# muelea/tuch

Measured on AMD Instinct MI355X. Metric: SMPLify-DC fit iters/sec at batch 64, higher is better.
Workload: dtype f32; 1 GPU; configs[1] extended to the full stage-2 step: batch=64/GPU SMPL forward + contact_fitting_loss (L_P/L_C push/pull, winding inside test, segment filter, r2r) + backward + Adam, V=6890 F=13776, float32; bodies_per_gpu=64, global_batch=64, launch=hipGraph replay of the whole step

## Files before the change

include/tuch_amd.h:

```cpp
#ifndef TUCH_AMD_H
#define TUCH_AMD_H

#include <stddef.h>
#include <stdint.h>

#ifdef __cplusplus
extern "C" {
#endif

const char* tuch_last_error(void);
int tuch_abi_version(void);


int tuch_batch_pairwise_dist(const float* x, const float* y, int B, int Nx, int Ny, int squared,
                             float* P, void* stream);

int tuch_batch_pairwise_dist_bwd(const float* x, const float* y, const float* grad_P, int B, int Nx, int Ny,
                                 int squared, float* grad_x, float* grad_y, void* stream);

int tuch_solid_angles_bwd(const float* points, const float* triangles, const float* grad_out, const float* grad_w,
                          int B, int Q, int F, float* grad_points, float* grad_triangles, void* stream);

int tuch_solid_angles(const float* points, const float* triangles, int B, int Q, int F, float* out,
                      void* stream);
// ... 70 lines not shown
int tuch_smplify_tail_bwd(const float* grad_out, const uint8_t* valid, const float* gj, const float* gc, const float* gp,
                          int B, int NJ, int P, float contact_scale, float r2r_scale, float* grad_contact, float* grad_r2r,
                          float* gj_out, float* gc_out, float* gp_out, void* stream);

size_t tuch_smplify_stage2_fused_scratch_floats(int B);
int tuch_smplify_stage2_fused(const float* points, const int32_t* partner, const uint8_t* exterior,
                              const uint8_t* body_valid, int B, int N, int mode, float euclthres,
                              const float* small_terms, const float* r2r, const int32_t* ij, int P, float contact_scale,
                              float r2r_scale, float* share, int* ticket, float* terms, float* out, float* grad_points,
                              const tuch_contact_model* model, const void* pair_keys, void* grad_fixed_zeroed, void* stream);
int tuch_fixed_to_float(const void* fixed, size_t n, float* out, void* stream);
void tuch_set_deterministic(int on);
int tuch_get_deterministic(void);

int tuch_region_pair_keys(const tuch_contact_model* model, const float* verts, int B, const uint8_t* select,
                          int use_geomask, void* keys_zeroed, void* stream);
int tuch_smplify_stage2_finish(const float* points, const int32_t* partner, const uint8_t* exterior,
                               const uint8_t* body_valid, int B, int N, int mode, float euclthres,
                               const float* small_terms, const float* r2r, int P, float contact_scale, float r2r_scale,
                               float* share, int* ticket, float* terms, float* out, void* stream);
int tuch_smplify_stage2_bwd(const float* grad_out, const uint8_t* body_valid, const float* points, const int32_t* partner,
                            const uint8_t* exterior, int B, int N, int mode, float euclthres, float contact_scale,
                            const int32_t* ij, int P, float r2r_scale, const float* gj, const float* gc, const float* gp,
                            int NJ, float* grad_points, float* gj_out, float* gc_out, float* gp_out, void* stream);

typedef struct tuch_contact_model tuch_contact_model;

int tuch_contact_model_create(tuch_contact_model** out, int V, int F, const int32_t* faces ,
                              const uint8_t* geomask ,
                              int num_segments, const int32_t* seg_q_off, const int32_t* seg_q_vidx,
                              const int32_t* seg_f_off, const int32_t* seg_faces,
                              int num_caps, const int32_t* cap_off, const int32_t* cap_vidx,
                              int num_regions, const int32_t* region_off, const int32_t* region_vidx,
                              int num_pairs, const int32_t* pairs);
void tuch_contact_model_destroy(tuch_contact_model* model);
int tuch_contact_model_set_option(tuch_contact_model* model, const char* name, int value);
int tuch_contact_model_get_option(const tuch_contact_model* model, const char* name, int* value);
int tuch_contact_model_canary_hits(const tuch_contact_model* model, int* hits_host, int reset);
int tuch_contact_model_canary_selftest(const tuch_contact_model* model, void* workspace, size_t workspace_bytes, void* stream);
const uint64_t* tuch_contact_model_mask_bits(const tuch_contact_model* model);
const int32_t* tuch_contact_model_faces(const tuch_contact_model* model);
int32_t* tuch_contact_model_tickets(const tuch_contact_model* model);
const uint64_t* tuch_contact_model_tree_mask_bits(const tuch_contact_model* model);
int tuch_contact_model_info(const tuch_contact_model* model, int* V, int* F, int* num_segments,
                            int* seg_q_total, int* num_pairs);
int tuch_contact_model_strips(const tuch_contact_model* model, int* stream_len, int* num_strips,
                              int32_t* vidx_host, float* sign_host);

int tuch_winding_tree_work(const tuch_contact_model* model, const float* verts, int B, void* workspace,
                           size_t workspace_bytes, unsigned long long* out_host, void* stream);

int tuch_ray_work(const tuch_contact_model* model, const float* verts, int B, void* workspace,
                  size_t workspace_bytes, unsigned long long* out_host, void* stream);
int tuch_contact_model_tree_order(const tuch_contact_model* model, int32_t* qperm_host, int32_t* face_leaf_host);

size_t tuch_v2v_model_workspace_bytes(const tuch_contact_model* model, int B);
size_t tuch_v2v_hint_bytes(const tuch_contact_model* model, int B);
int tuch_v2v_min_model(const tuch_contact_model* model, const float* verts, int B, float* min_d2,
                       int32_t* argmin, void* hint_inout, void* workspace, size_t workspace_bytes, void* stream);
int tuch_v2v_min_model_shared(const tuch_contact_model* model, const float* verts, int B, float* min_d2,
                              int32_t* argmin, void* hint_inout, void* workspace, size_t workspace_bytes, int leave_room,
                              void* stream);
int tuch_v2v_min_model_shared_zero(const tuch_contact_model* model, const float* verts, int B, float* min_d2, int32_t* argmin,
                                   void* hint_inout, void* workspace, size_t workspace_bytes, int leave_room, void* zero,
                                   size_t zero_bytes, void* stream);

int tuch_v2v_min_model_can_cap(const tuch_contact_model* model);
int tuch_v2v_min_model_capped(const tuch_contact_model* model, const float* verts, int B, float* min_d2, int32_t* argmin,
                              void* hint_inout, void* workspace, size_t workspace_bytes, int leave_room, void* zero,
                              size_t zero_bytes, const uint8_t* prev_exterior, float cap, void* stream);
int tuch_v2v_min_model_fix(const tuch_contact_model* model, int B, const uint8_t* exterior, uint8_t* prev_exterior, float cap,
                           float* min_d2, int32_t* argmin, void* hint_inout, void* workspace, size_t workspace_bytes,
                           void* stream);

typedef struct tuch_cluster_tree tuch_cluster_tree;
int tuch_cluster_tree_build(int V, int F, const int32_t* faces, int leaf_faces, tuch_cluster_tree** out);
void tuch_cluster_tree_free(tuch_cluster_tree* tree);
int tuch_cluster_tree_info(const tuch_cluster_tree* tree, int* num_nodes, int* exact_len, int* stream_len,
                           int* num_qblocks, int* num_frontiers, int* frontier_total);
int tuch_cluster_tree_export(const tuch_cluster_tree* tree, int32_t* nodes, int32_t* vidx, float* sign,
                             int32_t* qperm, int32_t* frontier_off, int32_t* frontier_nodes,
                             int32_t* launch_order, int32_t* rows, int32_t* face_leaf);

size_t tuch_exterior_workspace_bytes(const tuch_contact_model* model, int B);
int tuch_exterior_flags(const tuch_contact_model* model, const float* verts, int B, int apply_segments,
                        float thresh, float* w, uint8_t* exterior, float* seg_w, uint8_t* seg_exterior,
                        void* workspace, size_t workspace_bytes, void* stream);

size_t tuch_winding_points_workspace_bytes(const tuch_contact_model* model, int B, int Q);
int tuch_winding_points(const tuch_contact_model* model, const float* verts, const float* points,
                        const int32_t* counts, int B, int Q, float thresh, float* w, uint8_t* exterior,
                        void* workspace, size_t workspace_bytes, void* stream);

int tuch_region_pair_min(const tuch_contact_model* model, const float* verts, int B, const uint8_t* select,
                         int use_geomask, float* out_min, int32_t* out_ij, void* stream);
int tuch_region_pair_min_bwd(const tuch_contact_model* model, const float* verts, int B, const int32_t* ij,
                             const float* grad_out, float* grad_verts, void* stream);

int tuch_self_contact(const float* verts , const uint64_t* geomask_bits, int B, int V, float euclthres,
                      const int32_t* vreg_off , const int32_t* vreg , int R,
                      uint8_t* in_contact , int32_t* partner , float* min_d2 ,
                      float* sig_d2 , float* cnc_d2 , void* stream);

typedef struct tuch_smpl_model tuch_smpl_model;

int tuch_smpl_model_create(tuch_smpl_model** out, int V, const float* v_template, const float* shapedirs,
// ... 76 lines not shown
```

tuch_amd/_C.py:

```python
from __future__ import annotations

import ctypes
import os
from ctypes import POINTER, c_char_p, c_float, c_int, c_size_t, c_void_p

import torch

_HERE = os.path.dirname(os.path.abspath(__file__))
LIB_PATH = os.environ.get('TUCH_AMD_LIB') or os.path.join(_HERE, 'libtuch_amd.so')
_lib = None

_SIGNATURES = {
    'tuch_last_error': (c_char_p, []),
    'tuch_abi_version': (c_int, []),
    'tuch_batch_pairwise_dist': (c_int, [c_void_p, c_void_p, c_int, c_int, c_int, c_int, c_void_p, c_void_p]),
    'tuch_batch_pairwise_dist_bwd': (c_int, [c_void_p, c_void_p, c_void_p, c_int, c_int, c_int, c_int, c_void_p, c_void_p,
                                             c_void_p]),
    'tuch_solid_angles_bwd': (c_int, [c_void_p, c_void_p, c_void_p, c_void_p, c_int, c_int, c_int, c_void_p, c_void_p, c_void_p]),
    'tuch_solid_angles': (c_int, [c_void_p, c_void_p, c_int, c_int, c_int, c_void_p, c_void_p]),
    'tuch_gather_triangles': (c_int, [c_void_p, c_void_p, c_int, c_int, c_int, c_void_p, c_void_p]),
    'tuch_winding_workspace_bytes': (c_size_t, [c_int, c_int, c_int]),
    'tuch_winding_numbers': (c_int, [c_void_p, c_void_p, c_int, c_int, c_int, c_void_p, c_void_p, c_float,
                                     c_void_p, c_size_t, c_void_p]),
    'tuch_geomask_words': (c_int, [c_int]),
# ... 15 lines not shown
    'tuch_valid_mean_fwd': (c_int, [c_void_p, c_void_p, c_int, c_int, c_void_p, c_void_p]),
    'tuch_valid_mean_bwd': (c_int, [c_void_p, c_void_p, c_void_p, c_int, c_int, c_void_p, c_void_p]),
    'tuch_smpl_backward_split_adam': (c_int, [c_void_p, c_void_p, c_int, c_void_p, c_int, c_int, c_void_p, c_void_p, c_void_p,
                                              c_void_p, c_void_p, c_int, c_void_p, c_int, c_void_p, c_int,
                                              c_void_p, c_int, c_void_p, c_int, c_void_p, c_void_p, c_void_p, c_void_p, c_void_p,
                                              c_void_p, c_float, c_float, c_float, c_float, c_void_p, c_size_t, c_void_p, c_void_p]),
    'tuch_contact_terms_bwd_fixed': (c_int, [c_void_p, c_void_p, c_void_p, c_void_p, c_int, c_int, c_int, c_float,
                                             c_void_p, c_void_p, c_void_p]),
    'tuch_smplify_small_terms': (c_int, [c_void_p] * 9 + [c_int, c_int, c_int, c_float, c_float, c_float] + [c_void_p] * 5),
    'tuch_smplify_stage1_terms': (c_int, [c_void_p] * 7 + [c_int, c_int, c_int, c_float, c_float, c_float, c_float] + [c_void_p] * 7),
    'tuch_adam_step': (c_int, [c_int, c_void_p, c_void_p, c_void_p, c_void_p, c_void_p, c_void_p, c_void_p, c_float, c_float,
                                c_void_p]),
    'tuch_smplify_objective': (c_int, [c_void_p, c_void_p, c_void_p, c_int, c_int, c_float, c_float, c_void_p, c_void_p]),
    'tuch_smplify_objective_bwd': (c_int, [c_void_p, c_int, c_int, c_float, c_float, c_void_p, c_void_p, c_void_p,
                                           c_void_p]),
    'tuch_smplify_tail_bwd': (c_int, [c_void_p] * 5 + [c_int, c_int, c_int, c_float, c_float] + [c_void_p] * 6),
    'tuch_contact_model_create': (c_int, [POINTER(c_void_p), c_int, c_int, c_void_p, c_void_p,
                                          c_int, c_void_p, c_void_p, c_void_p, c_void_p,
                                          c_int, c_void_p, c_void_p,
                                          c_int, c_void_p, c_void_p, c_int, c_void_p]),
    'tuch_contact_model_destroy': (None, [c_void_p]),
    'tuch_contact_model_set_option': (c_int, [c_void_p, c_char_p, c_int]),
    'tuch_contact_model_get_option': (c_int, [c_void_p, c_char_p, POINTER(c_int)]),
    'tuch_contact_model_canary_hits': (c_int, [c_void_p, POINTER(c_int), c_int]),
    'tuch_contact_model_canary_selftest': (c_int, [c_void_p, c_void_p, c_size_t, c_void_p]),
    'tuch_contact_model_mask_bits': (c_void_p, [c_void_p]),
    'tuch_contact_model_faces': (c_void_p, [c_void_p]),
    'tuch_contact_model_tickets': (c_void_p, [c_void_p]),
    'tuch_contact_model_tree_mask_bits': (c_void_p, [c_void_p]),
    'tuch_contact_model_info': (c_int, [c_void_p, POINTER(c_int), POINTER(c_int), POINTER(c_int),
                                        POINTER(c_int), POINTER(c_int)]),
    'tuch_contact_model_strips': (c_int, [c_void_p, POINTER(c_int), POINTER(c_int), c_void_p, c_void_p]),
    'tuch_cluster_tree_build': (c_int, [c_int, c_int, c_void_p, c_int, POINTER(c_void_p)]),
    'tuch_cluster_tree_free': (None, [c_void_p]),
    'tuch_cluster_tree_info': (c_int, [c_void_p] + [POINTER(c_int)] * 6),
    'tuch_cluster_tree_export': (c_int, [c_void_p] * 10),
    'tuch_hd_points_fwd': (c_int, [c_void_p] * 5 + [c_int, c_int, c_void_p, c_void_p]),
    'tuch_hd_points_bwd': (c_int, [c_void_p] * 5 + [c_int, c_int, c_void_p, c_void_p]),
    'tuch_estimate_translation': (c_int, [c_void_p, c_void_p, c_void_p, c_int, c_int, c_float, c_float, c_void_p, c_void_p]),
    'tuch_rotmat_to_angle_axis': (c_int, [c_void_p, c_int, c_int, c_void_p, c_void_p]),
    'tuch_winding_tree_work': (c_int, [c_void_p, c_void_p, c_int, c_void_p, c_size_t, c_void_p, c_void_p]),
    'tuch_hd_model_create': (c_int, [POINTER(c_void_p), c_void_p, c_int, c_void_p, c_void_p, c_void_p]),
    'tuch_hd_model_create_k': (c_int, [POINTER(c_void_p), c_void_p, c_int, c_int, c_void_p, c_void_p, c_void_p]),
    'tuch_hd_model_destroy': (None, [c_void_p]),
    'tuch_hd_model_info': (c_int, [c_void_p, POINTER(c_int), c_void_p]),
    'tuch_hd_contact_saved_bytes': (c_size_t, [c_void_p, c_int]),
    'tuch_hd_contact_workspace_bytes': (c_size_t, [c_void_p, c_int]),
    'tuch_hd_contact_fwd': (c_int, [c_void_p] * 6 + [c_int, c_float, c_float, c_void_p, c_void_p, c_size_t, c_void_p, c_size_t,
                                    c_void_p]),
    'tuch_hd_contact_bwd': (c_int, [c_void_p, c_void_p, c_void_p, c_int, c_void_p, c_void_p, c_size_t, c_void_p]),
    'tuch_hd_contact_selection': (c_int, [c_void_p, c_void_p, c_int, c_void_p, c_void_p]),
    'tuch_hd_contact_details': (c_int, [c_void_p, c_void_p, c_int, c_void_p, c_void_p]),
    'tuch_ray_work': (c_int, [c_void_p, c_void_p, c_int, c_void_p, c_size_t, c_void_p, c_void_p]),
    'tuch_contact_model_tree_order': (c_int, [c_void_p, c_void_p, c_void_p]),
    'tuch_v2v_model_workspace_bytes': (c_size_t, [c_void_p, c_int]),
    'tuch_v2v_hint_bytes': (c_size_t, [c_void_p, c_int]),
    'tuch_v2v_min_model': (c_int, [c_void_p, c_void_p, c_int, c_void_p, c_void_p, c_void_p, c_void_p, c_size_t, c_void_p]),
    'tuch_v2v_min_model_shared': (c_int, [c_void_p, c_void_p, c_int, c_void_p, c_void_p, c_void_p, c_void_p, c_size_t, c_int,
                                          c_void_p]),
    'tuch_v2v_min_model_shared_zero': (c_int, [c_void_p, c_void_p, c_int, c_void_p, c_void_p, c_void_p, c_void_p, c_size_t, c_int,
                                               c_void_p, c_size_t, c_void_p]),
    'tuch_exterior_workspace_bytes': (c_size_t, [c_void_p, c_int]),
    'tuch_v2v_min_model_can_cap': (c_int, [c_void_p]),
    'tuch_v2v_min_model_capped': (c_int, [c_void_p, c_void_p, c_int, c_void_p, c_void_p, c_void_p, c_void_p, c_size_t, c_int,
                                          c_void_p, c_size_t, c_void_p, c_float, c_void_p]),
    'tuch_v2v_min_model_fix': (c_int, [c_void_p, c_int, c_void_p, c_void_p, c_float, c_void_p, c_void_p, c_void_p, c_void_p,
                                       c_size_t, c_void_p]),
    'tuch_exterior_flags': (c_int, [c_void_p, c_void_p, c_int, c_int, c_float, c_void_p, c_void_p, c_void_p,
                                    c_void_p, c_void_p, c_size_t, c_void_p]),
    'tuch_winding_points_workspace_bytes': (c_size_t, [c_void_p, c_int, c_int]),
    'tuch_winding_points': (c_int, [c_void_p, c_void_p, c_void_p, c_void_p, c_int, c_int, c_float, c_void_p, c_void_p,
                                    c_void_p, c_size_t, c_void_p]),
    'tuch_contact_terms_ragged_fwd': (c_int, [c_void_p, c_void_p, c_void_p, c_void_p, c_int, c_int, c_float, c_void_p,
                                              c_void_p]),
    'tuch_contact_terms_ragged_bwd': (c_int, [c_void_p, c_void_p, c_void_p, c_void_p, c_void_p, c_int, c_int, c_float,
                                              c_void_p, c_void_p]),
    'tuch_region_pair_min': (c_int, [c_void_p, c_void_p, c_int, c_void_p, c_int, c_void_p, c_void_p, c_void_p]),
    'tuch_smpl_model_create': (c_int, [POINTER(c_void_p), c_int] + [c_void_p] * 9),
    'tuch_smpl_model_destroy': (None, [c_void_p]),
    'tuch_smpl_model_info': (c_int, [c_void_p, POINTER(c_int)]),
    'tuch_smpl_forward_workspace_bytes': (c_size_t, [c_void_p, c_int]),
    'tuch_smpl_backward_workspace_bytes': (c_size_t, [c_void_p, c_int]),
    'tuch_smpl_forward': (c_int, [c_void_p, c_void_p, c_void_p, c_int, c_int, c_void_p, c_void_p, c_void_p,
                                  c_size_t, c_void_p]),
    'tuch_smpl_backward': (c_int, [c_void_p, c_void_p, c_int, c_int, c_void_p, c_void_p, c_void_p, c_void_p,
                                   c_void_p, c_void_p, c_size_t, c_void_p]),
    'tuch_smplify_stage2_fused_scratch_floats': (c_size_t, [c_int]),
    'tuch_smplify_stage2_fused': (c_int, [c_void_p, c_void_p, c_void_p, c_void_p, c_int, c_int, c_int, c_float, c_void_p, c_void_p,
                                           c_void_p, c_int, c_float, c_float, c_void_p, c_void_p, c_void_p, c_void_p, c_void_p,
                                           c_void_p, c_void_p, c_void_p, c_void_p]),
    'tuch_set_deterministic': (None, [c_int]),
    'tuch_get_deterministic': (c_int, []),
    'tuch_region_pair_keys': (c_int, [c_void_p, c_void_p, c_int, c_void_p, c_int, c_void_p, c_void_p]),
    'tuch_smplify_stage2_finish': (c_int, [c_void_p, c_void_p, c_void_p, c_void_p, c_int, c_int, c_int, c_float, c_void_p,
                                           c_void_p, c_int, c_float, c_float, c_void_p, c_void_p, c_void_p, c_void_p,
                                           c_void_p]),
    'tuch_smplify_stage2_bwd': (c_int, [c_void_p, c_void_p, c_void_p, c_void_p, c_void_p, c_int, c_int, c_int, c_float,
                                        c_float, c_void_p, c_int, c_float, c_void_p, c_void_p, c_void_p, c_int, c_void_p,
                                        c_void_p, c_void_p, c_void_p, c_void_p]),
    'tuch_smpl_forward_split': (c_int, [c_void_p, c_void_p, c_void_p, c_int, c_void_p, c_int, c_int, c_int, c_void_p,
                                        c_void_p, c_void_p, c_size_t, c_void_p]),
    'tuch_smpl_backward_split': (c_int, [c_void_p, c_void_p, c_int, c_void_p, c_int, c_int, c_int, c_void_p, c_void_p,
                                         c_void_p, c_void_p, c_void_p, c_int, c_void_p, c_int, c_void_p, c_size_t,
                                         c_void_p]),
    'tuch_smpl_backward_split_add': (c_int, [c_void_p, c_void_p, c_int, c_void_p, c_int, c_int, c_int, c_void_p, c_void_p,
                                             c_void_p, c_void_p, c_void_p, c_int, c_void_p, c_int, c_void_p, c_int, c_void_p,
# ... 65 lines not shown
```

tuch_amd/csrc/api.hip:

```cpp
#include "common.h"
#include <stdarg.h>
#include <stdio.h>

static thread_local char g_error[512] = "";

void tuch_set_error(const char* fmt, ...)
{
    va_list ap;
    va_start(ap, fmt);
    vsnprintf(g_error, sizeof(g_error), fmt, ap);
    va_end(ap);
}

int tuch_check_launch(const char* what)
{
    const hipError_t e = hipGetLastError();
    if (e != hipSuccess) {
        tuch_set_error("%s: %s", what, hipGetErrorString(e));
        return TUCH_ERR_HIP;
    }
    return TUCH_OK;
}

extern "C" const char* tuch_last_error(void) { return g_error; }
extern "C" int tuch_abi_version(void) { return 1; }

#include <stdlib.h>
static int g_deterministic = [] { const char* e = getenv("TUCH_DETERMINISTIC"); return e && atoi(e) == 0 ? 0 : 1; }();
int tuch_deterministic() { return g_deterministic; }
extern "C" void tuch_set_deterministic(int on) { g_deterministic = on ? 1 : 0; }
extern "C" int tuch_get_deterministic(void) { return g_deterministic; }

static int g_host_tables = [] { const char* e = getenv("TUCH_HOST_TABLES"); return e && atoi(e) != 0 ? 1 : 0; }();
int tuch_host_tables() { return g_host_tables; }
#include <string.h>
int tuch_table_upload(void** dst, const void* src, size_t bytes)
{
    *dst = nullptr;
    if (bytes == 0) return TUCH_OK;
    if (g_host_tables) {
        *dst = malloc(bytes);
        if (!*dst) { tuch_set_error("model table: malloc(%zu) failed", bytes); return TUCH_ERR_HIP; }
        memcpy(*dst, src, bytes);
        return TUCH_OK;
    }
    if (hipMalloc(dst, bytes) != hipSuccess) {
        *dst = nullptr;
        tuch_set_error("model table: hipMalloc(%zu) failed", bytes);
        return TUCH_ERR_HIP;
    }
    if (hipMemcpy(*dst, src, bytes, hipMemcpyHostToDevice) != hipSuccess) {
        tuch_set_error("model table: hipMemcpy of %zu bytes failed", bytes);
        return TUCH_ERR_HIP;
    }
    return TUCH_OK;
}
int tuch_table_download(void* dst_host, const void* src, size_t bytes)
{
    if (g_host_tables) { memcpy(dst_host, src, bytes); return TUCH_OK; }
    return hipMemcpy(dst_host, src, bytes, hipMemcpyDeviceToHost) == hipSuccess ? TUCH_OK : TUCH_ERR_HIP;
}
void tuch_table_free(void* p)
{
    if (!p) return;
    if (g_host_tables) free(p); else (void)hipFree(p);
}
```

tuch_amd/csrc/model.h:

```cpp
#pragma once
#include "common.h"
#include <vector>

struct tuch_cluster_tree {
    int V = 0, F = 0, num_nodes = 0, exact_len = 0, stream_len = 0, num_qblocks = 0, num_heights = 0;
    std::vector<int32_t> nodes;
    std::vector<int32_t> vidx;
    std::vector<float> sign;
    std::vector<int32_t> qperm;
    std::vector<int32_t> height_off, height_nodes;
    std::vector<int32_t> frontier_off, frontier_nodes;
    std::vector<int32_t> launch_order;
    std::vector<int32_t> ancestors;
    std::vector<int32_t> rows;
    std::vector<int32_t> face_leaf;
};

bool tuch_cluster_tree_build_impl(int V, int F, const int32_t* faces, int leaf_faces, tuch_cluster_tree& t);
void tuch_build_strips(const int32_t* faces, int F, std::vector<int32_t>& vidx, std::vector<float>& sign,
                       int* num_strips);

struct tuch_contact_model;

struct tuch_options {
    int winding_ray = 1;
    int winding_tree = 1;
    int winding_strips = 1;
    int tree_waves = 32768;
    int ray_pair_cap = 16;
    int ray_waves = 32768;
    int ray_fans = 0;
    int ray_cross = 0;
    int ray_cross_split = 0;
    int v2v_tree = 1;
    int v2v_waves = 0;
    int v2v_cap = 0;
    int v2v_flat = 2;
    int v2v_pairs = 24;
    int v2v_lds = -1;
    int seg_splits = 16;
    int seg_assist = 1;
    int seg_fused = 1;
    int canary = 0;
    int hd_search = 1;
    int hd_search_waves = 4;
    int hd_overlap = 1;
};
void tuch_options_from_env(tuch_options* o);

bool tuch_ray_available(const tuch_contact_model* m);
struct RayEntry { int32_t leaf, node; uint32_t mask_lo, mask_hi; };
struct RayTile { int32_t ex_off, ex_len, first, n; };
struct RayBody { int32_t tiles, overflow; };
struct TreeNode;
void tuch_ray_layout_touch(const tuch_contact_model* m, int B, int Q);
size_t tuch_ray_workspace_bytes(const tuch_contact_model* m, int B, int Q);
int tuch_ray_exterior_verts(const tuch_contact_model* m, const float* verts, int B, float thresh, uint8_t* exterior,
                            float* w, void* workspace, hipStream_t s, unsigned long long* stats_host,
                            uint8_t* exterior_copy = nullptr);
const int32_t* tuch_ray_segment_counts(const tuch_contact_model* m, int B, const void* workspace);
void tuch_ray_segment_prepare(const tuch_contact_model* m, const float* verts, const float* caps, int assisted, int B,
                              float* seg_entries, hipStream_t s);
bool tuch_ray_segment_fused_available(const tuch_contact_model* m);
int tuch_ray_segment_flags_one(const tuch_contact_model* m, const float* verts, const uint8_t* body_flags,
                               const int32_t* leaf_counts, int B, float thresh, uint8_t* exterior, hipStream_t s);
int tuch_ray_segment_flags(const tuch_contact_model* m, const float* verts, const float* caps, const int32_t* seg_count,
                           const int32_t* seg_list, const int32_t* leaf_counts, int B, int nsplit, float thresh, float* seg_tris,
                           int32_t* seg_partial, float* seg_w, uint8_t* seg_ext, uint8_t* exterior, hipStream_t s);
int tuch_ray_exterior_points(const tuch_contact_model* m, const float* verts, const float* points, const int32_t* counts,
                             int B, int Q, float thresh, uint8_t* exterior, float* w, void* workspace, hipStream_t s);

int tuch_v2v_min_indexed_seeded(const float* points, const int32_t* vertex_ids, const int32_t* offsets,
                                const int32_t* counts, const float* seed_best, const int32_t* seed_arg,
                                const int32_t* all_masked_arg, const uint64_t* geomask_bits, int B, int V,
                                int max_points_per_body, float* min_d2, int32_t* argmin, void* workspace, hipStream_t s);
extern "C" size_t tuch_v2v_min_indexed_workspace_bytes(int B, int max_points_per_body);
size_t tuch_hd_search_workspace_bytes(int B, int max_points_per_body);
int tuch_hd_search(const float* points, const int32_t* vertex_ids, const int32_t* offsets, const int32_t* counts,
                   const int32_t* all_masked_arg, const uint64_t* geomask_bits, int B, int V, int max_points_per_body,
                   float* min_d2, int32_t* argmin, void* workspace, hipStream_t s, int waves);
extern "C" size_t tuch_winding_points_workspace_bytes(const tuch_contact_model* m, int B, int Q);
extern "C" int tuch_winding_points(const tuch_contact_model* m, const float* verts, const float* points,
                                   const int32_t* counts, int B, int Q, float thresh, float* w,
                                   uint8_t* exterior, void* workspace, size_t workspace_bytes, void* stream);

struct tuch_contact_model {
    int device;
    tuch_options opt;
    int V, F;
    int32_t* faces;
    int32_t* tickets;
    int32_t* canary_hits;
    uint64_t* mask_bits;
    int strip_len, num_strips;
    int32_t* strip_vidx;
    float* strip_sign;
    int tree_nodes, tree_stream_len, tree_exact_len, tree_qblocks, tree_heights, tree_leaves;
    int32_t* tree_node;
    int32_t* tree_vidx;
    float* tree_sign;
    int32_t* tree_sign_word;
    int32_t* tree_qperm;
    int32_t* tree_height_off;
    int32_t* tree_height_nodes;
    int32_t* tree_frontier_nodes;
    int32_t* tree_launch_order;
    int32_t* tree_ancestors;
    int32_t* tree_rows;
    int32_t* tree_v2v_info;
    uint64_t* tree_mask_bits;
    uint64_t* tree_masked;
    int32_t* tree_sub_leaf;
// ... 49 lines not shown
```

tuch_amd/csrc/model.hip:

```cpp
#include "model.h"
#include <stdio.h>
#include <stdlib.h>
#include <string.h>
#include <algorithm>
#include <vector>
#include <unordered_map>

extern "C" int tuch_geomask_words(int V);

namespace {

template <typename T>
int upload(T** dst, const T* src, size_t count)
{
    return tuch_table_upload((void**)dst, src, count * sizeof(T));
}

int* host_copy(const int32_t* src, size_t n)
{
    int* p = (int*)malloc(sizeof(int) * (n ? n : 1));
    if (n) memcpy(p, src, sizeof(int) * n);
    return p;
}

// ... 375 lines not shown
        for (int r = 0; r < num_regions; ++r) {
            const int n = region_off[r + 1] - region_off[r];
            if (n > m->region_max) m->region_max = n;
        }
        rc = upload(&m->region_off, region_off, (size_t)num_regions + 1);
        if (rc == TUCH_OK) rc = upload(&m->region_vidx, region_vidx, (size_t)region_off[num_regions]);
        if (rc == TUCH_OK && num_pairs > 0) rc = upload(&m->pairs, pairs, (size_t)num_pairs * 2);
        if (rc == TUCH_OK && num_pairs > 0 && geomask) {
            std::vector<int64_t> off(num_pairs + 1, 0);
            for (int p = 0; p < num_pairs; ++p) {
                const int n1 = region_off[pairs[2 * p] + 1] - region_off[pairs[2 * p]];
                const int n2 = region_off[pairs[2 * p + 1] + 1] - region_off[pairs[2 * p + 1]];
                off[p + 1] = off[p] + (int64_t)n1 * ((n2 + 31) / 32);
            }
            std::vector<uint32_t> words((size_t)off[num_pairs], 0u);
            for (int p = 0; p < num_pairs; ++p) {
                const int32_t* r1 = region_vidx + region_off[pairs[2 * p]];
                const int32_t* r2 = region_vidx + region_off[pairs[2 * p + 1]];
                const int n1 = region_off[pairs[2 * p] + 1] - region_off[pairs[2 * p]];
                const int n2 = region_off[pairs[2 * p + 1] + 1] - region_off[pairs[2 * p + 1]];
                const int wpr = (n2 + 31) / 32;
                for (int a = 0; a < n1; ++a)
                    for (int k = 0; k < n2; ++k)
                        if (geomask[(size_t)r1[a] * V + r2[k]])
                            words[(size_t)off[p] + (size_t)a * wpr + (k >> 5)] |= 1u << (k & 31);
            }
            rc = upload(&m->pair_mask, words.data(), words.size());
            if (rc == TUCH_OK) rc = upload(&m->pair_mask_off, off.data(), off.size());
        }
    }
    if (rc == TUCH_OK && !tree_sign_host.empty()) {
        std::vector<int32_t> word(tree_sign_host.size(), 0);
        for (size_t p = 0; p < word.size(); ++p) {
            const int32_t sg = tree_sign_host[p] > 0.0f ? 1 : tree_sign_host[p] < 0.0f ? -1 : 0;
            const int32_t em = p < elem_mask_host.size() ? elem_mask_host[p] : 0;
            word[p] = (int32_t)(((uint32_t)em << 24) | ((uint32_t)sg & 0xffffffu));
        }
        rc = upload(&m->tree_sign_word, word.data(), word.size());
    }
    if (rc != TUCH_OK) {
        tuch_contact_model_destroy(m);
        *out = nullptr;
        return rc;
    }
    *out = m;
    return TUCH_OK;
}

namespace {
struct OptionName { const char* name; int tuch_options::*field; };
const OptionName kOptions[] = {
    {"winding_ray", &tuch_options::winding_ray}, {"winding_tree", &tuch_options::winding_tree},
    {"winding_strips", &tuch_options::winding_strips}, {"tree_waves", &tuch_options::tree_waves},
    {"ray_pair_cap", &tuch_options::ray_pair_cap}, {"ray_waves", &tuch_options::ray_waves}, {"ray_fans", &tuch_options::ray_fans}, {"ray_cross", &tuch_options::ray_cross}, {"v2v_cap", &tuch_options::v2v_cap}, {"ray_cross_split", &tuch_options::ray_cross_split},
    {"v2v_tree", &tuch_options::v2v_tree}, {"v2v_flat", &tuch_options::v2v_flat}, {"v2v_pairs", &tuch_options::v2v_pairs}, {"v2v_waves", &tuch_options::v2v_waves}, {"v2v_lds", &tuch_options::v2v_lds},
    {"seg_splits", &tuch_options::seg_splits}, {"seg_assist", &tuch_options::seg_assist}, {"seg_fused", &tuch_options::seg_fused},
    {"canary", &tuch_options::canary}, {"hd_search", &tuch_options::hd_search}, {"hd_search_waves", &tuch_options::hd_search_waves}, {"hd_overlap", &tuch_options::hd_overlap},
};
}

void tuch_options_from_env(tuch_options* o)
{
    for (const OptionName& k : kOptions) {
        char env[64] = "TUCH_";
        size_t n = strlen(env);
        for (const char* c = k.name; *c && n + 1 < sizeof(env); ++c) env[n++] = (char)toupper((unsigned char)*c);
        env[n] = 0;
        const char* e = getenv(env);
        if (e && *e) o->*(k.field) = atoi(e);
    }
}

extern "C" int tuch_contact_model_set_option(tuch_contact_model* m, const char* name, int value)
{
    TUCH_REQUIRE(m && name, "tuch_contact_model_set_option: null argument");
    for (const OptionName& k : kOptions)
        if (!strcmp(k.name, name)) {
            TUCH_REQUIRE(strcmp(name, "seg_assist") != 0, "tuch_contact_model_set_option: seg_assist is fixed when the model "
                         "is created (TUCH_SEG_ASSIST)");
            m->opt.*(k.field) = value;
            return TUCH_OK;
        }
    tuch_set_error("tuch_contact_model_set_option: unknown option '%s'", name);
    return TUCH_ERR_ARG;
}

extern "C" int tuch_contact_model_canary_hits(const tuch_contact_model* m, int* hits_host, int reset)
{
    TUCH_REQUIRE(m && hits_host, "tuch_contact_model_canary_hits: null argument");
    if (hipDeviceSynchronize() != hipSuccess ||
        hipMemcpy(hits_host, m->canary_hits, sizeof(int32_t), hipMemcpyDeviceToHost) != hipSuccess ||
        (reset && hipMemset(m->canary_hits, 0, sizeof(int32_t)) != hipSuccess)) {
        tuch_set_error("tuch_contact_model_canary_hits: %s", hipGetErrorString(hipGetLastError()));
        return TUCH_ERR_HIP;
    }
    return TUCH_OK;
}

extern "C" int tuch_contact_model_get_option(const tuch_contact_model* m, const char* name, int* value)
{
    TUCH_REQUIRE(m && name && value, "tuch_contact_model_get_option: null argument");
    if (!strcmp(name, "seg_fused_active")) {
        *value = tuch_ray_segment_fused_available(m) ? 1 : 0;
        return TUCH_OK;
    }
    for (const OptionName& k : kOptions)
        if (!strcmp(k.name, name)) {
            *value = m->opt.*(k.field);
            return TUCH_OK;
        }
    tuch_set_error("tuch_contact_model_get_option: unknown option '%s'", name);
    return TUCH_ERR_ARG;
}

extern "C" const uint64_t* tuch_contact_model_mask_bits(const tuch_contact_model* m)
{
    return m ? m->mask_bits : nullptr;
}

extern "C" const uint64_t* tuch_contact_model_tree_mask_bits(const tuch_contact_model* m)
{
    return m ? m->tree_mask_bits : nullptr;
}

extern "C" int32_t* tuch_contact_model_tickets(const tuch_contact_model* m)
{
    return m ? m->tickets : nullptr;
}

extern "C" const int32_t* tuch_contact_model_faces(const tuch_contact_model* m)
{
    return m ? m->faces : nullptr;
}

extern "C" int tuch_contact_model_tree_order(const tuch_contact_model* m, int32_t* qperm_host, int32_t* face_leaf_host)
{
    TUCH_REQUIRE(m, "tuch_contact_model_tree_order: null model");
    TUCH_REQUIRE(m->tree_nodes > 0 && m->tree_qperm_host && m->tree_face_leaf_host,
                 "tuch_contact_model_tree_order: the model has no cluster tree");
    if (qperm_host) memcpy(qperm_host, m->tree_qperm_host, sizeof(int32_t) * m->V);
    if (face_leaf_host) memcpy(face_leaf_host, m->tree_face_leaf_host, sizeof(int32_t) * m->F);
    return TUCH_OK;
}

extern "C" int tuch_contact_model_strips(const tuch_contact_model* m, int* stream_len, int* num_strips,
                                         int32_t* vidx_host, float* sign_host)
{
    TUCH_REQUIRE(m, "tuch_contact_model_strips: null model");
    if (stream_len) *stream_len = m->strip_len;
    if (num_strips) *num_strips = m->num_strips;
    if (vidx_host && tuch_table_download(vidx_host, m->strip_vidx, sizeof(int32_t) * m->strip_len) != TUCH_OK)
        return TUCH_ERR_HIP;
    if (sign_host && tuch_table_download(sign_host, m->strip_sign, sizeof(float) * m->strip_len) != TUCH_OK)
        return TUCH_ERR_HIP;
    return TUCH_OK;
}
// ... 13 lines not shown
```

tuch_amd/csrc/ray_winding.hip:

```cpp
#include "common.h"
#include "model.h"
#include "workspace.h"
#include "tree_device.h"
#include <stdlib.h>

#pragma clang fp contract(off)

namespace {

constexpr float kPi = 3.14159265358979323846f;
constexpr int kBlock = 256;
constexpr int kRayQueries = 64;
constexpr float kShearX = 0.3217f, kShearY = 0.4331f;
constexpr float kFanX = 0.8191f, kFanY = 0.3467f, kFanZ = 0.4571f;
constexpr int kSlabs = 9;
constexpr int kSlabStride = 10;
constexpr int kNearSlabs = 13;

struct RayElem { float x, y, z, sign; };

__device__ __forceinline__ float shear_x(float x, float z) { return __builtin_fmaf(-kShearX, z, x); }
__device__ __forceinline__ float shear_y(float y, float z) { return __builtin_fmaf(-kShearY, z, y); }

__global__ __launch_bounds__(kBlock) void ray_stream_kernel(
// ... 32 lines not shown
    v = fminf(v, dpp_move<0x141>(v));
    v = fminf(v, dpp_move<0x140>(v));
    return v;
}

__device__ __forceinline__ uint32_t half_below(float x)
{
    const _Float16 h = (_Float16)x;
    uint32_t u = __builtin_bit_cast(uint16_t, h);
    if ((float)h > x) u = (u & 0x8000u) ? u + 1 : (u == 0 ? 0x8001u : u - 1);
    return u;
}
__device__ __forceinline__ uint32_t half_above(float x)
{
    const _Float16 h = (_Float16)x;
    uint32_t u = __builtin_bit_cast(uint16_t, h);
    if ((float)h < x) u = (u & 0x8000u) ? (u == 0x8000u ? 0x0001u : u - 1) : u + 1;
    return u;
}
__device__ __host__ __forceinline__ size_t near_records_at(int B, int L) { return (size_t)B * kNearSlabs * L; }
__device__ __host__ __forceinline__ size_t near_centres_at(int B, int L) { return near_records_at(B, L) + (size_t)B * L * 8; }

struct QRec { float x, y, z; int32_t tag; };
constexpr int kNoSlot = 0xffffff;
struct RayPre { int blocks, qblocks; QRec* qrec; float4* ranges; const int32_t* vmask; };

__device__ __forceinline__ void ray_block_prepass(const float* __restrict__ vb, int first_vertex,
                                                  const int32_t* __restrict__ qperm, const int32_t* __restrict__ vmask,
                                                  int Q, int qb, int lane, QRec* __restrict__ qrec, float4* __restrict__ ranges)
{
    const int slot = qb * kRayQueries + lane;
    const float* q3 = vb + 3 * (size_t)qperm[slot];
    const float* c0 = vb + 3 * (size_t)first_vertex;
    const float qz = q3[2], qx = shear_x(q3[0], qz), qy = shear_y(q3[1], qz);
    const float cz = c0[2], cx = shear_x(c0[0], cz), cy = shear_y(c0[1], cz);
    QRec r;
    r.x = qx; r.y = qy; r.z = qz;
    r.tag = slot < Q ? (slot | (vmask ? vmask[slot] << 24 : 0)) : kNoSlot;
    qrec[slot] = r;
    const float rx = qx - cx, ry = qy - cy, rz = qz - cz;
    const float r4 = rx + ry, r5 = rx - ry, r6 = rx + rz, r7 = rx - rz, r8 = ry + rz, r9 = ry - rz;
    const float bx0 = wave_min_uniform(rx), bx1 = wave_max_uniform(rx), by0 = wave_min_uniform(ry), by1 = wave_max_uniform(ry);
    const float b40 = wave_min_uniform(r4), b41 = wave_max_uniform(r4), b50 = wave_min_uniform(r5), b51 = wave_max_uniform(r5);
    const float bz0 = wave_min_uniform(rz), b60 = wave_min_uniform(r6), b71 = wave_max_uniform(r7);
    const float b80 = wave_min_uniform(r8), b91 = wave_max_uniform(r9);
    if (lane == 0) {
        ranges[0] = make_float4(bx0, bx1, by0, by1);
        ranges[1] = make_float4(b40, b41, b50, b51);
        ranges[2] = make_float4(bz0, b60, b71, b80);
        ranges[3] = make_float4(b91, 0.f, 0.f, 0.f);
    }
}

__device__ __forceinline__ float fan_terms(const float* __restrict__ vb, int v, bool real, int& n,
                                           const int32_t* __restrict__ ring_off, const int32_t* __restrict__ ring_vidx);
template <bool kPose>
__global__ __launch_bounds__(kBoundsBlock) void ray_leaf_bounds_kernel(
    const RayElem* __restrict__ stream, int T, const TreeNode* __restrict__ nodes, int N,
    const int32_t* __restrict__ height_off, const int32_t* __restrict__ height_nodes, float* __restrict__ bounds,
    const float* __restrict__ verts, const int32_t* __restrict__ vidx, const float* __restrict__ sign, int V, int Lexact,
    RayElem* __restrict__ stream_out, uint4* __restrict__ zeroed, size_t zeroed_n,
    int leaf_blocks = 0, const int32_t* __restrict__ qperm = nullptr, const int32_t* __restrict__ ring_off = nullptr,
    const int32_t* __restrict__ ring_vidx = nullptr, float2* __restrict__ fans = nullptr, int fan_stride = 0,
    RayPre pre = RayPre{0, 0, nullptr, nullptr, nullptr})
{
    if (kPose && pre.blocks > 0 && (int)blockIdx.x >= (int)gridDim.x - pre.blocks) {
        for (size_t g = ((size_t)blockIdx.y * gridDim.x + blockIdx.x) * kBoundsBlock + threadIdx.x; g < zeroed_n;
             g += (size_t)gridDim.x * gridDim.y * kBoundsBlock)
            zeroed[g] = make_uint4(0u, 0u, 0u, 0u);
        const int qb = ((int)blockIdx.x - ((int)gridDim.x - pre.blocks)) * (kBoundsBlock / 64) + (int)(threadIdx.x >> 6);
        if (qb < pre.qblocks)
            ray_block_prepass(verts + (size_t)blockIdx.y * V * 3, vidx[0], qperm, pre.vmask, V, qb, threadIdx.x & 63,
                              pre.qrec + (size_t)blockIdx.y * pre.qblocks * kRayQueries,
                              pre.ranges + ((size_t)blockIdx.y * pre.qblocks + qb) * 4);
        return;
    }
    if (kPose && leaf_blocks > 0 && (int)blockIdx.x >= leaf_blocks) {
        for (size_t g = ((size_t)blockIdx.y * gridDim.x + blockIdx.x) * kBoundsBlock + threadIdx.x; g < zeroed_n;
             g += (size_t)gridDim.x * gridDim.y * kBoundsBlock)
            zeroed[g] = make_uint4(0u, 0u, 0u, 0u);
        const int i = ((int)blockIdx.x - leaf_blocks) * kBoundsBlock + (int)threadIdx.x;
        const bool real = i < V;
        const int v = qperm[real ? i : V - 1];
        int cr = 0;
        const float half = fan_terms(verts + (size_t)blockIdx.y * V * 3, v, real, cr, ring_off, ring_vidx);
        if (i < fan_stride) fans[(size_t)blockIdx.y * fan_stride + i] = make_float2(__int_as_float(cr), half);
        return;
    }
    const int b = blockIdx.y;
    const RayElem* st = stream + (size_t)b * T;
    const int group = threadIdx.x >> 4, sub = threadIdx.x & 15;
    const int i = height_off[0] + blockIdx.x * (kBoundsBlock / 16) + group;
    const bool real = i < height_off[1];
    const int node = height_nodes[real ? i : height_off[0]];
    const int off = nodes[node].ex_off, len = real ? nodes[node].ex_len : 0;
    if (kPose) {
        for (size_t g = ((size_t)b * gridDim.x + blockIdx.x) * kBoundsBlock + threadIdx.x; g < zeroed_n;
             g += (size_t)gridDim.x * gridDim.y * kBoundsBlock)
            zeroed[g] = make_uint4(0u, 0u, 0u, 0u);
        if (blockIdx.x == 0)
            for (int p = Lexact + (int)threadIdx.x; p < T; p += kBoundsBlock) stream_out[(size_t)b * T + p] = RayElem{0.f, 0.f, 0.f, 0.f};
    }
    float lo[kSlabs], nhi[kSlabs];
#pragma unroll
    for (int k = 0; k < kSlabs; ++k) { lo[k] = 3.0e38f; nhi[k] = 3.0e38f; }
    for (int p = sub; p < len; p += 16) {
        RayElem e;
        if (kPose) {
            const float* c = verts + ((size_t)b * V + vidx[off + p]) * 3;
            e.x = shear_x(c[0], c[2]); e.y = shear_y(c[1], c[2]); e.z = c[2]; e.sign = sign[off + p];
            stream_out[(size_t)b * T + off + p] = e;
        } else {
            e = st[off + p];
        }
        float pr[kSlabs];
        slab_project(e.x, e.y, e.z, pr);
#pragma unroll
        for (int k = 0; k < kSlabs; ++k) { lo[k] = fminf(lo[k], pr[k]); nhi[k] = fminf(nhi[k], -pr[k]); }
    }
#pragma unroll
    for (int k = 0; k < kSlabs; ++k) { lo[k] = row_min(lo[k]); nhi[k] = row_min(nhi[k]); }
    if (real && sub == 0) {
        const int L = height_off[1] - height_off[0], leaf = i - height_off[0];
        float lo_p[kSlabs], hi_p[kSlabs];
#pragma unroll
        for (int k = 0; k < kSlabs; ++k) {
            const float hi = -nhi[k];
            const float pad = 4e-7f * fmaxf(fabsf(lo[k]), fabsf(hi)) + 1e-9f;
            lo_p[k] = lo[k] - pad;
            hi_p[k] = hi + pad;
        }
        float c[3];
        if (kPose) {
            const float* c0 = verts + ((size_t)b * V + vidx[0]) * 3;
            c[0] = shear_x(c0[0], c0[2]); c[1] = shear_y(c0[1], c0[2]); c[2] = c0[2];
        } else {
            const RayElem e0 = st[0];
            c[0] = e0.x; c[1] = e0.y; c[2] = e0.z;
        }
        float pc[kSlabs];
        slab_project(c[0], c[1], c[2], pc);
        uint32_t lo_h[kSlabs], hi_h[kSlabs];
#pragma unroll
        for (int k = 0; k < kSlabs; ++k) {
            const float pad = 4e-6f * (fabsf(lo_p[k]) + fabsf(hi_p[k]) + fabsf(pc[k])) + 1e-7f;
            lo_h[k] = half_below(lo_p[k] - pc[k] - pad);
            hi_h[k] = half_above(hi_p[k] - pc[k] + pad);
        }
        uint4* r = reinterpret_cast<uint4*>(bounds + near_records_at(gridDim.y, L)) + ((size_t)b * L + leaf) * 2;
        r[0] = make_uint4(lo_h[0] | lo_h[1] << 16, lo_h[3] | lo_h[4] << 16, lo_h[6] | lo_h[8] << 16, hi_h[0] | hi_h[1] << 16);
        r[1] = make_uint4(hi_h[2] | hi_h[3] << 16, hi_h[4] | hi_h[5] << 16, hi_h[7] | (uint32_t)leaf << 16, (uint32_t)node);
        if (leaf == 0) *reinterpret_cast<float4*>(bounds + near_centres_at(gridDim.y, L) + (size_t)b * 4) = make_float4(c[0], c[1], c[2], 0.f);
    }
}

__global__ __launch_bounds__(kBoundsBlock) void ray_prepass_kernel(
    const float* __restrict__ verts, const int32_t* __restrict__ vidx, const int32_t* __restrict__ qperm, int V, RayPre pre)
{
    const int qb = (int)blockIdx.x * (kBoundsBlock / 64) + (int)(threadIdx.x >> 6);
    if (qb < pre.qblocks)
        ray_block_prepass(verts + (size_t)blockIdx.y * V * 3, vidx[0], qperm, pre.vmask, V, qb, threadIdx.x & 63,
                          pre.qrec + (size_t)blockIdx.y * pre.qblocks * kRayQueries,
                          pre.ranges + ((size_t)blockIdx.y * pre.qblocks + qb) * 4);
}

struct P3 { float x, y, z; };

__device__ __forceinline__ float edge_fn(const P3& p, const P3& q) { return p.x * q.y - p.y * q.x; }

__device__ __forceinline__ bool left_of(float e, const P3& p, const P3& q)
{
    return e > 0.0f || (e == 0.0f && (p.x < q.x || (p.x == q.x && p.y < q.y)));
}

__device__ __forceinline__ int crossing(const P3& a, const P3& b, const P3& c, float ea, float eb, float ec)
{
    const bool la = left_of(ea, b, c), lb = left_of(eb, c, a), lc = left_of(ec, a, b);
    const bool pos = la && lb && lc, neg = !la && !lb && !lc;
    if (!(pos || neg)) return 0;
    const float numz = ea * a.z + eb * b.z + ec * c.z;
    if (pos) return numz > 0.0f ? 1 : 0;
    return numz < 0.0f ? -1 : 0;
}

__device__ __forceinline__ int crossing_mostly_generic(const P3& a, const P3& b, const P3& c, float ea, float eb, float ec)
{
    const float numz = ea * a.z + eb * b.z + ec * c.z;
    const float mn = __builtin_fminf(__builtin_fminf(ea, eb), ec), mx = __builtin_fmaxf(__builtin_fmaxf(ea, eb), ec);
    int n = (int)(__builtin_fminf(mn, numz) > 0.0f) - (int)(__builtin_fmaxf(mx, numz) < 0.0f);
    const bool tie = (mn * mx == 0.0f) & (numz != 0.0f);
    if (__builtin_amdgcn_ballot_w64(tie)) {
        if (tie) n = crossing(a, b, c, ea, eb, ec);
    }
    return n;
}

template <bool kSkipIncident>
__device__ __forceinline__ int crossing_with_ties(const P3 a, const P3 b, const P3 c, float ea, float eb, float ec)
{
    if (kSkipIncident) {
        const bool za = (a.x == 0.0f) & (a.y == 0.0f) & (a.z == 0.0f);
        const bool zb = (b.x == 0.0f) & (b.y == 0.0f) & (b.z == 0.0f);
        const bool zc = (c.x == 0.0f) & (c.y == 0.0f) & (c.z == 0.0f);
        if (za | zb | zc) return 0;
    }
    return crossing(a, b, c, ea, eb, ec);
}

constexpr uint32_t kSegBias = 0x80808080u;
struct S3 { v2f xy; float z; };
__device__ __forceinline__ float edge_fn(const S3& p, const S3& q)
{
    v2f r;
    asm("v_pk_mul_f32 %0, %1, %2 op_sel:[0,1] op_sel_hi:[1,0]" : "=v"(r) : "v"(p.xy), "v"(q.xy));
    float d;
    asm("v_sub_f32 %0, %1, %2" : "=v"(d) : "v"(r.x), "v"(r.y));
    return d;
}
__device__ __forceinline__ P3 p3(const S3& a) { return P3{a.xy.x, a.xy.y, a.z}; }

template <int A, bool kSkipIncident, bool kSeg>
__device__ __forceinline__ void ray_step(const RayElem el, S3 (&s)[3], float (&e)[3], v2f qxy, float qz, int& count,
                                         int qmask, uint32_t& pa, uint32_t& pb)
{
    constexpr int Bq = (A + 1) % 3, Cq = (A + 2) % 3;
    s[A].xy = (v2f){el.x, el.y} - qxy;
    s[A].z = el.z - qz;
    e[Bq] = edge_fn(s[Cq], s[A]);
    e[Cq] = edge_fn(s[A], s[Bq]);
    const int word = __float_as_int(el.sign);
    if ((word & 0xffffff) != 0) {
        const float numz = __builtin_fmaf(e[A], s[A].z, __builtin_fmaf(e[Cq], s[Cq].z, e[Bq] * s[Bq].z));
        const float mn = __builtin_fminf(__builtin_fminf(e[0], e[1]), e[2]);
        const float mx = __builtin_fmaxf(__builtin_fmaxf(e[0], e[1]), e[2]);
        int c = (int)(__builtin_fminf(mn, numz) > 0.0f) - (int)(__builtin_fmaxf(mx, numz) < 0.0f);
        const bool edge_zero = mn * mx == 0.0f;
        if (__builtin_amdgcn_ballot_w64(edge_zero)) {
            const bool tie = edge_zero & (numz != 0.0f);
            if (__builtin_amdgcn_ballot_w64(tie)) {
                if (tie) c = crossing_with_ties<kSkipIncident>(p3(s[Bq]), p3(s[Cq]), p3(s[A]), e[Bq], e[Cq], e[A]);
            }
        }
        asm("v_mad_i32_i24 %0, %1, %2, %0" : "+v"(count) : "v"(c), "s"(word));
        if (kSeg && ((uint32_t)word >> 24) != 0) {
            const uint32_t t = ((uint32_t)word >> 24) & (uint32_t)qmask;
            if (__builtin_amdgcn_ballot_w64((t != 0) & (c != 0))) {
                uint32_t cs;
                asm("v_mul_i32_i24 %0, %1, %2" : "=v"(cs) : "v"(c), "s"(word));
                pa += cs * (((t & 15u) * 0x00204081u) & 0x01010101u);
                pb += cs * ((((t >> 4) & 15u) * 0x00204081u) & 0x01010101u);
            }
        }
    }
}

template <bool kSkipIncident, bool kSeg>
__device__ __forceinline__ void ray_run(const RayElem* __restrict__ st, int off, int len,
                                        S3 (&s)[3], float (&e)[3], v2f qxy, float qz, int& count,
                                        int qmask, uint32_t& pa, uint32_t& pb)
{
    const RayElem* p = st + off;
    RayElem n0 = p[0], n1 = p[1], n2 = p[2];
    for (int left = len; left > 0; left -= 3, p += 3) {
        asm("" : "+s"(left));
        const RayElem e0 = n0, e1 = n1, e2 = n2;
        n0 = p[3]; n1 = p[4]; n2 = p[5];
        ray_step<0, kSkipIncident, kSeg>(e0, s, e, qxy, qz, count, qmask, pa, pb);
        ray_step<1, kSkipIncident, kSeg>(e1, s, e, qxy, qz, count, qmask, pa, pb);
        ray_step<2, kSkipIncident, kSeg>(e2, s, e, qxy, qz, count, qmask, pa, pb);
    }
}

constexpr int kFallbackChunks = 8;

__device__ __forceinline__ float wave_min(float v) { return wave_min_uniform(v); }
__device__ __forceinline__ float wave_max(float v) { return wave_max_uniform(v); }


__device__ __forceinline__ float lo_minus(uint32_t s, float q)
{
    float d;
    asm("v_fma_mix_f32 %0, %1, 1.0, -%2 op_sel_hi:[1,0,0]" : "=v"(d) : "v"(s), "v"(q));
    return d;
}
__device__ __forceinline__ float hi_minus(uint32_t s, float q)
{
    float d;
    asm("v_fma_mix_f32 %0, %1, 1.0, -%2 op_sel:[1,0,0] op_sel_hi:[1,0,0]" : "=v"(d) : "v"(s), "v"(q));
    return d;
}
__device__ __forceinline__ float minus_lo(float q, uint32_t s)
{
    float d;
    asm("v_fma_mix_f32 %0, -%1, 1.0, %2 op_sel_hi:[1,0,0]" : "=v"(d) : "v"(s), "v"(q));
    return d;
}
__device__ __forceinline__ float minus_hi(float q, uint32_t s)
{
    float d;
    asm("v_fma_mix_f32 %0, -%1, 1.0, %2 op_sel:[1,0,0] op_sel_hi:[1,0,0]" : "=v"(d) : "v"(s), "v"(q));
    return d;
}
__device__ __forceinline__ float max3(float a, float b, float c)
{
    float d;
    asm("v_max3_f32 %0, %1, %2, %3" : "=v"(d) : "v"(a), "v"(b), "v"(c));
    return d;
}

template <bool kVerts, int kWaves>
__global__ __launch_bounds__(64 * kWaves) void ray_near_kernel(
    const float* __restrict__ pts, const TreeNode* __restrict__ nodes, const float* __restrict__ bounds, int N,
    int num_leaves, const int32_t* __restrict__ qperm,
    const int32_t* __restrict__ counts, int Q, int qblocks, RayEntry* __restrict__ lists, int32_t* __restrict__ list_len,
    int32_t* __restrict__ leaf_cnt,
    unsigned long long* __restrict__ stats,
    const int32_t* __restrict__ ring_off = nullptr, const int32_t* __restrict__ ring_vidx = nullptr,
    float2* __restrict__ fans = nullptr)
{
    if (kVerts && (int)blockIdx.x >= qblocks) {
        const int i = ((int)blockIdx.x - qblocks) * (64 * kWaves) + (int)threadIdx.x;
        const bool real = i < Q;
        const int v = qperm[real ? i : Q - 1];
        int cr = 0;
        const float half = fan_terms(pts + (size_t)blockIdx.y * Q * 3, v, real, cr, ring_off, ring_vidx);
        if (i < qblocks * kRayQueries) fans[(size_t)blockIdx.y * qblocks * kRayQueries + i] = make_float2(__int_as_float(cr), half);
        return;
    }
    __builtin_amdgcn_s_setprio(3);
    const int qb = blockIdx.x, b = blockIdx.y, lane = threadIdx.x & 63;
    const int wave = kWaves > 1 ? __builtin_amdgcn_readfirstlane(threadIdx.x >> 6) : 0;
    __shared__ uint4 queue[64 * kWaves][2];
    __shared__ float range[16];
    __shared__ int queued[2], slots;
    int i0;
    bool real;
    if (kVerts) {
        i0 = qperm[qb * kRayQueries + lane];
        real = qb * kRayQueries + lane < Q;
    } else {
        const int n = counts ? counts[b] : Q;
        if (qb * kRayQueries >= n) {
            if (threadIdx.x == 0) list_len[(size_t)b * qblocks + qb] = 0;
            return;
        }
        i0 = min(qb * kRayQueries + lane, n - 1);
        real = qb * kRayQueries + lane < n;
    }
    if (threadIdx.x == 0) { queued[0] = 0; queued[1] = 0; slots = 0; }
    const float4 ctr = *reinterpret_cast<const float4*>(bounds + near_centres_at(gridDim.y, num_leaves) + (size_t)b * 4);
    const uint4* recs = reinterpret_cast<const uint4*>(bounds + near_records_at(gridDim.y, num_leaves)) + (size_t)b * num_leaves * 2;
    struct Chunk { uint4 r0, r1; };
    auto load_chunk = [&](int base) {
        Chunk c;
        const int lc = min(base + lane, num_leaves - 1);
        c.r0 = recs[lc * 2];
        c.r1 = recs[lc * 2 + 1];
        return c;
    };
    Chunk nxt = load_chunk(wave * 64);
    const float* q3 = pts + ((size_t)b * Q + i0) * 3;
    const float qz = q3[2];
    const float qx = shear_x(q3[0], qz), qy = shear_y(q3[1], qz);
    const float rx = qx - ctr.x, ry = qy - ctr.y, rz = qz - ctr.z;
    const float r4 = rx + ry, r5 = rx - ry, r6 = rx + rz, r7 = rx - rz, r8 = ry + rz, r9 = ry - rz;
    float bx0, bx1, by0, by1, b40, b41, b50, b51, bz0, b60, b71, b80, b91;
    if (kWaves == 4) {
        if (wave == 0) {
            const float a = wave_min(rx), c = wave_max(rx), d = wave_min(ry), e = wave_max(ry);
            if (lane == 0) { range[0] = a; range[1] = c; range[2] = d; range[3] = e; }
        } else if (wave == 1) {
            const float a = wave_min(r4), c = wave_max(r4), d = wave_min(r5), e = wave_max(r5);
            if (lane == 0) { range[4] = a; range[5] = c; range[6] = d; range[7] = e; }
        } else if (wave == 2) {
            const float a = wave_min(rz), c = wave_min(r6), d = wave_max(r7);
            if (lane == 0) { range[8] = a; range[9] = c; range[10] = d; }
        } else {
            const float a = wave_min(r8), c = wave_max(r9);
            if (lane == 0) { range[11] = a; range[12] = c; }
        }
        __syncthreads();
        bx0 = range[0]; bx1 = range[1]; by0 = range[2]; by1 = range[3]; b40 = range[4]; b41 = range[5]; b50 = range[6];
        b51 = range[7]; bz0 = range[8]; b60 = range[9]; b71 = range[10]; b80 = range[11]; b91 = range[12];
    } else {
        bx0 = wave_min(rx); bx1 = wave_max(rx); by0 = wave_min(ry); by1 = wave_max(ry);
        b40 = wave_min(r4); b41 = wave_max(r4); b50 = wave_min(r5); b51 = wave_max(r5);
        bz0 = wave_min(rz); b60 = wave_min(r6); b71 = wave_max(r7); b80 = wave_min(r8); b91 = wave_max(r9);
    }
    RayEntry* list = lists + ((size_t)b * qblocks + qb) * num_leaves;
    unsigned long long useful = 0, listed = 0;
    auto outside13 = [&](const uint4& s0, const uint4& s1, float x1, float x0, float y1, float y0, float p1, float p0,
                         float m1, float m0, float z0, float xz0, float xz1, float yz0, float yz1) {
        float out = max3(lo_minus(s0.x, x1), minus_lo(x0, s0.w), hi_minus(s0.x, y1));
        out = max3(out, minus_hi(y0, s0.w), lo_minus(s0.y, p1));
        out = max3(out, minus_hi(p0, s1.x), hi_minus(s0.y, m1));
        out = max3(out, minus_lo(m0, s1.y), minus_lo(z0, s1.x));
        out = max3(out, minus_hi(xz0, s1.y), lo_minus(s0.z, xz1));
        return max3(out, minus_lo(yz0, s1.z), hi_minus(s0.z, yz1));
    };
    auto outside = [&](const uint4& s0, const uint4& s1) {
        return outside13(s0, s1, rx, rx, ry, ry, r4, r4, r5, r5, rz, r6, r7, r8, r9);
    };
    int nslots = 0;
    auto emit = [&](const uint4& s1, unsigned long long hit) {
        if (!hit) return;
        const int leaf = (int)(s1.z >> 16), nd = (int)s1.w;
        if (kWaves == 1) ++nslots;
        if (lane == 0) {
            const int slot = kWaves == 1 ? nslots - 1 : atomicAdd(&slots, 1);
            list[slot] = RayEntry{leaf, nd, (uint32_t)hit, (uint32_t)(hit >> 32)};
            atomicAdd(&leaf_cnt[(size_t)b * num_leaves + leaf], __builtin_popcountll(hit));
        }
        if (stats) {
            const int len = nodes[nd].ex_len;
            useful += (unsigned long long)__builtin_popcountll(hit) * len;
            listed += 64ull * len;
        }
    };
    auto sync = [&] { if (kWaves > 1) __syncthreads(); else __builtin_amdgcn_wave_barrier(); };
    for (int round = 0; round * 64 * kWaves < num_leaves; ++round) {
        const int base = (round * kWaves + wave) * 64;
        const Chunk c = nxt;
        if (base + 64 * kWaves < num_leaves) nxt = load_chunk(base + 64 * kWaves);
        const bool pass = (base + lane < num_leaves) &
                          !(outside13(c.r0, c.r1, bx1, bx0, by1, by0, b41, b40, b51, b50, bz0, b60, b71, b80, b91) > 0.0f);
        const unsigned long long mask = __builtin_amdgcn_ballot_w64(pass);
        if (mask) {
            int at = 0;
            if (kWaves > 1) {
                if (lane == 0) at = atomicAdd(&queued[round & 1], __builtin_popcountll(mask));
                at = __builtin_amdgcn_readfirstlane(at);
            }
            at += __builtin_amdgcn_mbcnt_hi((uint32_t)(mask >> 32), __builtin_amdgcn_mbcnt_lo((uint32_t)mask, 0));
            if (pass) { queue[at][0] = c.r0; queue[at][1] = c.r1; }
        }
        sync();
        const int n = kWaves > 1 ? queued[round & 1] : __builtin_popcountll(mask);
        if (kWaves > 1 && threadIdx.x == 0) queued[(round + 1) & 1] = 0;
        if (kWaves == 1) {
            for (int i = 0; i < n; i += 4) {
                const int k1 = min(i + 1, n - 1), k2 = min(i + 2, n - 1), k3 = min(i + 3, n - 1);
                const uint4 a0 = queue[i][0], a1 = queue[i][1], c0 = queue[k1][0], c1 = queue[k1][1];
                const uint4 d0 = queue[k2][0], d1 = queue[k2][1], f0 = queue[k3][0], f1 = queue[k3][1];
                const float out_a = outside(a0, a1), out_c = outside(c0, c1), out_d = outside(d0, d1), out_f = outside(f0, f1);
                const unsigned long long hit_a = __builtin_amdgcn_ballot_w64(real && !(out_a > 0.0f));
                const unsigned long long hit_c = __builtin_amdgcn_ballot_w64(real && !(out_c > 0.0f) && i + 1 < n);
                const unsigned long long hit_d = __builtin_amdgcn_ballot_w64(real && !(out_d > 0.0f) && i + 2 < n);
                const unsigned long long hit_f = __builtin_amdgcn_ballot_w64(real && !(out_f > 0.0f) && i + 3 < n);
                emit(a1, hit_a);
                emit(c1, hit_c);
                emit(d1, hit_d);
                emit(f1, hit_f);
// ... 123 lines not shown
        for (int l = l0; l < l1; ++l) {
            const int c = cnt[l];
            off_s[l] = off;
            tile_s[l] = tile;
            off += c;
            tile += (c + 63) >> 6;
        }
        int ent = sq - nent;
        for (int q = q0; q < q1; ++q) { blk[q] = ent; ent += len[q]; }
        if (lane == 0) blk[qblocks] = total;
    }
    __syncthreads();
    for (int l = (int)blockIdx.y + (int)gridDim.y * lane; l < num_leaves; l += (int)gridDim.y * 64) {
        const TreeNode nd = nodes[leaf_nodes[l]];
        const int ex_off = nd.ex_off, ex_len = nd.ex_len;
        const int c = cnt[l], off = off_s[l];
        RayTile* out = tiles + (size_t)b * max_tiles + tile_s[l];
        for (int k = 0; k < c; k += 64) *out++ = RayTile{ex_off, ex_len, off + k, min(64, c - k)};
    }
    int32_t* fill = leaf_fill + (size_t)b * num_leaves;
    int32_t* out = pairs + (size_t)b * cap;
    for (int base = (int)blockIdx.y * 64; base < total; base += (int)gridDim.y * 64) {
        const int g = base + lane;
        RayEntry e = RayEntry{0, 0, 0u, 0u};
        int dst = 0, qb = 0;
        if (g < total) {
            int lo = 0, hi = qblocks;
            while (hi - lo > 1) {
                const int mid = (lo + hi) >> 1;
                if (blk[mid] <= g) lo = mid; else hi = mid;
            }
            qb = lo;
            e = lists[((size_t)b * qblocks + qb) * list_stride + (g - blk[qb])];
            dst = off_s[e.leaf] + atomicAdd(&fill[e.leaf], __builtin_popcount(e.mask_lo) + __builtin_popcount(e.mask_hi));
        }
        const int m = min(64, total - base);
        for (int k = 0; k < m; ++k) {
            const uint32_t lo = __builtin_amdgcn_readlane(e.mask_lo, k), hi = __builtin_amdgcn_readlane(e.mask_hi, k);
            const int d = __builtin_amdgcn_readlane(dst, k), q = __builtin_amdgcn_readlane(qb, k);
            const unsigned long long mask = ((unsigned long long)hi << 32) | lo;
            if ((mask >> lane) & 1ull)
                out[d + __builtin_popcountll(mask & ((1ull << lane) - 1ull))] = q * kRayQueries + lane;
        }
    }
}

template <bool kVerts, bool kCount, bool kSeg>
__global__ __launch_bounds__(64) void ray_leaf_kernel(
    const float* __restrict__ pts, const RayElem* __restrict__ stream, const RayTile* __restrict__ tiles,
    const RayBody* __restrict__ body, const int32_t* __restrict__ pairs, const RayEntry* __restrict__ lists,
    const int32_t* __restrict__ list_len, const TreeNode* __restrict__ nodes, int num_leaves,
    const int32_t* __restrict__ qperm, const int32_t* __restrict__ counts, int Q, int T, int qblocks, int num_bodies,
    int cap, int max_tiles, int32_t* __restrict__ count, unsigned long long* __restrict__ stats,
    const int32_t* __restrict__ vmask, int32_t* __restrict__ seg_count)
{
    const int lane = threadIdx.x;
    struct Work { int b, off, len, slot, qmask; bool active; float qx, qy, qz; };
    int b_cur = blockIdx.x, base = 0, g = blockIdx.y;
    auto fetch = [&]() {
        Work w;
        w.b = -1; w.off = w.len = w.slot = 0; w.qmask = 0; w.active = false; w.qx = w.qy = w.qz = 0.0f;
        while (b_cur < num_bodies) {
            const int b = b_cur;
            const int nt = __builtin_amdgcn_readfirstlane(body[b].tiles);
            if (g >= base + nt) { base += nt; b_cur += gridDim.x; continue; }
            const int t = g - base;
            g += gridDim.y;
            const float* pb = pts + (size_t)b * Q * 3;
            w.b = b;
            int i0;
            if (!__builtin_amdgcn_readfirstlane(body[b].overflow)) {
                const RayTile tile = tiles[(size_t)b * max_tiles + t];
                const int n = __builtin_amdgcn_readfirstlane(tile.n), first = __builtin_amdgcn_readfirstlane(tile.first);
                w.active = lane < n;
                w.slot = pairs[(size_t)b * cap + first + (w.active ? lane : 0)];
                i0 = kVerts ? qperm[w.slot] : w.slot;
                w.off = __builtin_amdgcn_readfirstlane(tile.ex_off);
                w.len = __builtin_amdgcn_readfirstlane(tile.ex_len);
            } else {
                const int nq = kVerts ? Q : (counts ? counts[b] : Q);
                w.slot = (t / kFallbackChunks) * kRayQueries + lane;
                w.active = w.slot < nq;
                i0 = kVerts ? qperm[w.slot] : min(w.slot, nq - 1);
                w.off = t;
                w.len = -1;
            }
            w.qz = pb[3 * i0 + 2];
            w.qx = shear_x(pb[3 * i0], w.qz);
            w.qy = shear_y(pb[3 * i0 + 1], w.qz);
            if (kSeg) w.qmask = vmask[w.slot];
            break;
        }
        return w;
    };
    int walked = 0;
    Work next = fetch();
    while (next.b >= 0) {
        const Work w = next;
        next = fetch();
        S3 s[3];
        float e[3];
#pragma unroll
        for (int k = 0; k < 3; ++k) { s[k].xy = (v2f){0.0f, 0.0f}; s[k].z = 0.0f; e[k] = 0.0f; }
        const v2f qxy = {w.qx, w.qy};
        int crossings = 0;
        uint32_t pa = kSegBias, pb = kSegBias;
        const RayElem* st = stream + (size_t)w.b * T;
        if (w.len >= 0) {
            ray_run<kVerts, kSeg>(st, w.off, w.len, s, e, qxy, w.qz, crossings, w.qmask, pa, pb);
            if (kCount) walked += w.len;
        } else {
            const int qb = w.off / kFallbackChunks, c = w.off % kFallbackChunks;
            const int cnt = __builtin_amdgcn_readfirstlane(list_len[(size_t)w.b * qblocks + qb]);
            const RayEntry* list = lists + ((size_t)w.b * qblocks + qb) * num_leaves;
            for (int j = c; j < cnt; j += kFallbackChunks) {
                const TreeNode nd = nodes[__builtin_amdgcn_readfirstlane(list[j].node)];
                ray_run<kVerts, kSeg>(st, nd.ex_off, nd.ex_len, s, e, qxy, w.qz, crossings, w.qmask, pa, pb);
                if (kCount) walked += nd.ex_len;
            }
        }
        if (w.active && crossings != 0) atomicAdd(&count[((size_t)w.b * qblocks) * kRayQueries + w.slot], crossings);
        if (kSeg && w.active && (pa != kSegBias || pb != kSegBias)) {
            int32_t* sc = seg_count + 2 * (((size_t)w.b * qblocks) * kRayQueries + w.slot);
            if (pa != kSegBias) atomicAdd(sc, (int32_t)(pa - kSegBias));
            if (pb != kSegBias) atomicAdd(sc + 1, (int32_t)(pb - kSegBias));
        }
    }
    if (kCount && lane == 0) atomicAdd(stats, (unsigned long long)walked);
}

constexpr int kCrossRing = 256, kCrossTrip = 3;
template <bool kSeg>
__global__ __launch_bounds__(64) void ray_cross_kernel(
    const RayElem* __restrict__ stream, const TreeNode* __restrict__ nodes, const float* __restrict__ bounds, int num_leaves,
    int nsplit,
    const QRec* __restrict__ qrec, const float4* __restrict__ ranges, int T, int qblocks, int num_bodies,
    int32_t* __restrict__ count, int32_t* __restrict__ seg_count)
{
    __shared__ QRec ring[kCrossRing];
    const int lane = threadIdx.x;
    const int unit = blockIdx.y / nsplit, z = blockIdx.y % nsplit;
    const int b = blockIdx.x + gridDim.x * (unit / num_leaves);
    if (b >= num_bodies) return;
    const int leaf = unit % num_leaves;
    const uint4* recs = reinterpret_cast<const uint4*>(bounds + near_records_at(num_bodies, num_leaves)) + ((size_t)b * num_leaves + leaf) * 2;
    const uint4 s0 = recs[0], s1 = recs[1];
    const float4 ctr = *reinterpret_cast<const float4*>(bounds + near_centres_at(num_bodies, num_leaves) + (size_t)b * 4);
    const TreeNode nd = nodes[(int)s1.w];
    const int ex_off = __builtin_amdgcn_readfirstlane(nd.ex_off), ex_len = __builtin_amdgcn_readfirstlane(nd.ex_len);
    const RayElem* st = stream + (size_t)b * T;
    const QRec* qb_base = qrec + (size_t)b * qblocks * kRayQueries;
    const float4* rg = ranges + (size_t)b * qblocks * 4;
    const int mine = qblocks > z ? (qblocks - z + nsplit - 1) / nsplit : 0;
    auto outside13 = [&](float x1, float x0, float y1, float y0, float p1, float p0, float m1, float m0, float z0, float xz0,
                         float xz1, float yz0, float yz1) {
        float out = max3(lo_minus(s0.x, x1), minus_lo(x0, s0.w), hi_minus(s0.x, y1));
        out = max3(out, minus_hi(y0, s0.w), lo_minus(s0.y, p1));
        out = max3(out, minus_hi(p0, s1.x), hi_minus(s0.y, m1));
        out = max3(out, minus_lo(m0, s1.y), minus_lo(z0, s1.x));
        out = max3(out, minus_hi(xz0, s1.y), lo_minus(s0.z, xz1));
        return max3(out, minus_lo(yz0, s1.z), hi_minus(s0.z, yz1));
    };
    auto ray_outside = [&](const QRec& q) {
        const float rx = q.x - ctr.x, ry = q.y - ctr.y, rz = q.z - ctr.z;
        return outside13(rx, rx, ry, ry, rx + ry, rx + ry, rx - ry, rx - ry, rz, rx + rz, rx - rz, ry + rz, ry - rz);
    };
    int head = 0, tail = 0;
    int base = -64;
    unsigned long long todo = 0;
    bool more = true, loaded = false;
    QRec q[kCrossTrip];
    bool have[kCrossTrip];
#pragma unroll
    for (int j = 0; j < kCrossTrip; ++j) { q[j] = QRec{0.f, 0.f, 0.f, kNoSlot}; have[j] = false; }
    auto fetch = [&]() {
        int k[kCrossTrip];
#pragma unroll
        for (int j = 0; j < kCrossTrip; ++j) {
// ... 9 lines not shown
        loaded = true;
    };
    for (;;) {
        if (tail - head < 64 && (more || loaded)) {
            if (loaded) {
                QRec qc[kCrossTrip];
                bool hc[kCrossTrip];
#pragma unroll
                for (int j = 0; j < kCrossTrip; ++j) { qc[j] = q[j]; hc[j] = have[j]; }
                loaded = false;
                if (todo) fetch();
                unsigned long long hit[kCrossTrip];
#pragma unroll
                for (int j = 0; j < kCrossTrip; ++j)
                    hit[j] = __builtin_amdgcn_ballot_w64(hc[j] && (qc[j].tag & kNoSlot) != kNoSlot && !(ray_outside(qc[j]) > 0.0f));
#pragma unroll
                for (int j = 0; j < kCrossTrip; ++j) {
                    if (hit[j]) {
                        const int pos = tail + __builtin_amdgcn_mbcnt_hi((uint32_t)(hit[j] >> 32), __builtin_amdgcn_mbcnt_lo((uint32_t)hit[j], 0));
                        if ((hit[j] >> lane) & 1ull) ring[pos & (kCrossRing - 1)] = qc[j];
                        tail += __builtin_popcountll(hit[j]);
                    }
                }
                continue;
            }
            if (!todo) {
                base += 64;
                if (base >= mine) { more = false; continue; }
                const int j = base + lane;
                const float4* g = rg + (size_t)(z + nsplit * min(j, mine - 1)) * 4;
                const float4 g0 = g[0], g1 = g[1], g2 = g[2], g3 = g[3];
                const bool pass = (j < mine) &
                                  !(outside13(g0.y, g0.x, g0.w, g0.z, g1.y, g1.x, g1.w, g1.z, g2.x, g2.y, g2.z, g2.w, g3.x) > 0.0f);
                todo = __builtin_amdgcn_ballot_w64(pass);
                continue;
            }
            fetch();
            continue;
        }
        const int n = min(64, tail - head);
        if (n <= 0) break;
        __builtin_amdgcn_wave_barrier();
        const bool active = lane < n;
        const QRec w = ring[(head + (active ? lane : 0)) & (kCrossRing - 1)];
        __builtin_amdgcn_wave_barrier();
        head += n;
        const int slot = w.tag & kNoSlot;
        S3 s[3];
        float e[3];
#pragma unroll
        for (int u = 0; u < 3; ++u) { s[u].xy = (v2f){0.0f, 0.0f}; s[u].z = 0.0f; e[u] = 0.0f; }
        int crossings = 0;
        uint32_t pa = kSegBias, pb = kSegBias;
        ray_run<true, kSeg>(st, ex_off, ex_len, s, e, (v2f){w.x, w.y}, w.z, crossings, (int)((uint32_t)w.tag >> 24), pa, pb);
        if (active && crossings != 0) atomicAdd(&count[((size_t)b * qblocks) * kRayQueries + slot], crossings);
        if (kSeg && active && (pa != kSegBias || pb != kSegBias)) {
            int32_t* sc = seg_count + 2 * (((size_t)b * qblocks) * kRayQueries + slot);
            if (pa != kSegBias) atomicAdd(sc, (int32_t)(pa - kSegBias));
            if (pb != kSegBias) atomicAdd(sc + 1, (int32_t)(pb - kSegBias));
        }
    }
}

__device__ __forceinline__ float fast_atan2(float y, float x)
{
    const float ax = __builtin_fabsf(x), ay = __builtin_fabsf(y);
    const float mx = __builtin_fmaxf(__builtin_fmaxf(ax, ay), 1e-37f);
    const float t = __builtin_fminf(ax, ay) / mx;
    const float s = t * t;
    float p = 0.0024567253421992064f;
    p = p * s + -0.014401361346244812f;
    p = p * s + 0.03978123143315315f;
    p = p * s + -0.07234857976436615f;
    p = p * s + 0.10498946160078049f;
    p = p * s + -0.14161229133605957f;
    p = p * s + 0.19985906779766083f;
    p = p * s + -0.33332598209381104f;
    p = p * s + 0.9999998807907104f;
    float v = p * t;
    v = ay > ax ? 1.57079632679489661923f - v : v;
    v = x < 0.0f ? kPi - v : v;
    return __builtin_copysignf(v, y);
}

__device__ __forceinline__ float half_solid_angle(const P3& a, const P3& b, const P3& c)
{
    const float na = __builtin_sqrtf(a.x * a.x + a.y * a.y + a.z * a.z);
    const float nb = __builtin_sqrtf(b.x * b.x + b.y * b.y + b.z * b.z);
    const float nc = __builtin_sqrtf(c.x * c.x + c.y * c.y + c.z * c.z);
    const float cx = b.y * c.z - b.z * c.y, cy = b.z * c.x - b.x * c.z, cz = b.x * c.y - b.y * c.x;
    const float num = a.x * cx + a.y * cy + a.z * cz;
    const float dab = a.x * b.x + a.y * b.y + a.z * b.z;
    const float dbc = b.x * c.x + b.y * c.y + b.z * c.z;
    const float dac = a.x * c.x + a.y * c.y + a.z * c.z;
    const float den = na * nb * nc + dab * nc + dac * nb + dbc * na;
    return fast_atan2(num, den);
}

__device__ __forceinline__ void cone_term(const P3& us, const P3& sb, const P3& sc, const P3& u, const P3& pb, const P3& pc,
                                          int& crossings, float& half)
{
    const float ea = edge_fn(sb, sc), eb = edge_fn(sc, us), ec = edge_fn(us, sb);
    const float d = ea * us.z + eb * sb.z + ec * sc.z;
    const bool la = left_of(ea, sb, sc), lb = left_of(eb, sc, us), lc = left_of(ec, us, sb);
    const bool front = d >= 0.0f;
    crossings = (la & lb & lc) ? (int)front : ((!la & !lb & !lc) ? -(int)!front : 0);
    const float nu = __builtin_sqrtf(u.x * u.x + u.y * u.y + u.z * u.z);
    const float nb = __builtin_sqrtf(pb.x * pb.x + pb.y * pb.y + pb.z * pb.z);
    const float nc = __builtin_sqrtf(pc.x * pc.x + pc.y * pc.y + pc.z * pc.z);
    const float cx = pb.y * pc.z - pb.z * pc.y, cy = pb.z * pc.x - pb.x * pc.z, cz = pb.x * pc.y - pb.y * pc.x;
    const float num = __builtin_fabsf(u.x * cx + u.y * cy + u.z * cz);
    const float dub = u.x * pb.x + u.y * pb.y + u.z * pb.z;
    const float dbc = pb.x * pc.x + pb.y * pc.y + pb.z * pc.z;
    const float duc = u.x * pc.x + u.y * pc.y + u.z * pc.z;
    const float den = nu * nb * nc + dub * nc + duc * nb + dbc * nu;
    half = fast_atan2(front ? num : -num, den);
}

__device__ __forceinline__ float fan_terms(const float* __restrict__ vb, int v, bool real, int& n,
                                           const int32_t* __restrict__ ring_off, const int32_t* __restrict__ ring_vidx)
{
    const float vx = vb[3 * v], vy = vb[3 * v + 1], vz = vb[3 * v + 2];
    const float qx = shear_x(vx, vz), qy = shear_y(vy, vz);
    const P3 u_dir = {kFanX, kFanY, kFanZ};
    const P3 us = {shear_x(kFanX, kFanZ), shear_y(kFanY, kFanZ), kFanZ};
    const int lo = ring_off[v], cnt = real ? ring_off[v + 1] - lo : 0;
    float half_sum = 0.0f;
    constexpr int kLongRing = 16;
    constexpr int kShortRing = 8;
    if (cnt > 0 && cnt <= kShortRing) {
        int rr[kShortRing];
        float cc[kShortRing][3];
#pragma unroll
        for (int u = 0; u < kShortRing; ++u) rr[u] = ring_vidx[lo + min(u, cnt - 1)];
#pragma unroll
        for (int u = 0; u < kShortRing; ++u) { cc[u][0] = vb[3 * rr[u]]; cc[u][1] = vb[3 * rr[u] + 1]; cc[u][2] = vb[3 * rr[u] + 2]; }
        P3 pb = {cc[kShortRing - 1][0] - vx, cc[kShortRing - 1][1] - vy, cc[kShortRing - 1][2] - vz};
        P3 sb = {shear_x(cc[kShortRing - 1][0], cc[kShortRing - 1][2]) - qx, shear_y(cc[kShortRing - 1][1], cc[kShortRing - 1][2]) - qy,
                 cc[kShortRing - 1][2] - vz};
#pragma unroll
        for (int u = 0; u < kShortRing; ++u) {
            if (u < cnt) {
                const P3 pc = {cc[u][0] - vx, cc[u][1] - vy, cc[u][2] - vz};
                const P3 sc = {shear_x(cc[u][0], cc[u][2]) - qx, shear_y(cc[u][1], cc[u][2]) - qy, cc[u][2] - vz};
                int cr;
                float hf;
                cone_term(us, sb, sc, u_dir, pb, pc, cr, hf);
                half_sum += hf;
                n += cr;
                pb = pc;
                sb = sc;
            }
        }
    } else if (cnt > 0 && cnt <= kLongRing) {
        int r = ring_vidx[lo + cnt - 1];
        P3 pb = {vb[3 * r] - vx, vb[3 * r + 1] - vy, vb[3 * r + 2] - vz};
        P3 sb = {shear_x(vb[3 * r], vb[3 * r + 2]) - qx, shear_y(vb[3 * r + 1], vb[3 * r + 2]) - qy, vb[3 * r + 2] - vz};
        for (int j0 = 0; j0 < cnt; j0 += 4) {
            int rr[4];
            float cc[4][3];
#pragma unroll
            for (int u = 0; u < 4; ++u) rr[u] = ring_vidx[lo + min(j0 + u, cnt - 1)];
#pragma unroll
            for (int u = 0; u < 4; ++u) { cc[u][0] = vb[3 * rr[u]]; cc[u][1] = vb[3 * rr[u] + 1]; cc[u][2] = vb[3 * rr[u] + 2]; }
#pragma unroll
            for (int u = 0; u < 4; ++u) {
                if (j0 + u < cnt) {
                    const P3 pc = {cc[u][0] - vx, cc[u][1] - vy, cc[u][2] - vz};
                    const P3 sc = {shear_x(cc[u][0], cc[u][2]) - qx, shear_y(cc[u][1], cc[u][2]) - qy, cc[u][2] - vz};
                    int cr;
                    float hf;
                    cone_term(us, sb, sc, u_dir, pb, pc, cr, hf);
                    half_sum += hf;
                    n += cr;
                    pb = pc;
                    sb = sc;
                }
            }
        }
    }
    unsigned long long todo = __builtin_amdgcn_ballot_w64(cnt > kLongRing);
    const int lane = threadIdx.x & 63;
    while (todo) {
        const int src = __builtin_ctzll(todo);
        todo &= todo - 1;
        const int llo = __builtin_amdgcn_readlane(lo, src), lcnt = __builtin_amdgcn_readlane(cnt, src);
        const float lvx = __shfl(vx, src), lvy = __shfl(vy, src), lvz = __shfl(vz, src);
        float h = 0.0f;
        int cr = 0;
        for (int j = lane; j < lcnt; j += 64) {
            const int r_prev = ring_vidx[llo + (j == 0 ? lcnt - 1 : j - 1)], r_cur = ring_vidx[llo + j];
            const float bx = vb[3 * r_prev], by = vb[3 * r_prev + 1], bz = vb[3 * r_prev + 2];
            const float cx = vb[3 * r_cur], cy = vb[3 * r_cur + 1], cz = vb[3 * r_cur + 2];
            const float lqx = shear_x(lvx, lvz), lqy = shear_y(lvy, lvz);
            const P3 pb = {bx - lvx, by - lvy, bz - lvz}, pc = {cx - lvx, cy - lvy, cz - lvz};
            const P3 sb = {shear_x(bx, bz) - lqx, shear_y(by, bz) - lqy, bz - lvz}, sc = {shear_x(cx, cz) - lqx, shear_y(cy, cz) - lqy, cz - lvz};
            int c1;
            float h1;
            cone_term(us, sb, sc, u_dir, pb, pc, c1, h1);
            h += h1;
            cr += c1;
        }
#pragma unroll
        for (int m = 32; m >= 1; m >>= 1) { h += __shfl_xor(h, m); cr += __shfl_xor(cr, m); }
        if (lane == src) { half_sum = h; n += cr; }
    }
    return half_sum;
}
__device__ __forceinline__ float fan_winding(const float* __restrict__ vb, int v, bool real, int n,
                                             const int32_t* __restrict__ ring_off, const int32_t* __restrict__ ring_vidx)
{
    const float half_sum = fan_terms(vb, v, real, n, ring_off, ring_vidx);
    return (float)n - half_sum * (0.5f / kPi);
}

__global__ __launch_bounds__(kBlock) void ray_finalize_verts_kernel(
    const float* __restrict__ verts, const int32_t* __restrict__ count, const int32_t* __restrict__ qperm,
    const int32_t* __restrict__ ring_off, const int32_t* __restrict__ ring_vidx,
    int V, int stride, float thresh, float* __restrict__ w_out, uint8_t* __restrict__ exterior,
    uint8_t* __restrict__ exterior_copy,
    const float2* __restrict__ fans)
{
    const int b = blockIdx.y;
    const int i = blockIdx.x * kBlock + threadIdx.x;
    const bool real = i < V;
    const int v = qperm[real ? i : V - 1];
    const int n = count[(size_t)b * stride + (real ? i : V - 1)];
    float w;
    if (fans) {
        const float2 f = fans[(size_t)b * stride + (real ? i : V - 1)];
        w = (float)(n + __float_as_int(f.x)) - f.y * (0.5f / kPi);
    } else
        w = fan_winding(verts + (size_t)b * V * 3, v, real, n, ring_off, ring_vidx);
    const size_t o = (size_t)b * V + v;
    if (real) {
        if (w_out) w_out[o] = w;
        if (exterior) exterior[o] = w <= thresh;
        if (exterior_copy) exterior_copy[o] = w <= thresh;
    }
}

__global__ __launch_bounds__(kBlock) void ray_finalize_points_kernel(
    const int32_t* __restrict__ count, const int32_t* __restrict__ counts,
    int Q, int stride, float thresh, float* __restrict__ w_out, uint8_t* __restrict__ exterior)
{
    const int b = blockIdx.y;
    const int i = blockIdx.x * kBlock + threadIdx.x;
    if (i >= Q) return;
    const int n = (!counts || i < counts[b]) ? count[(size_t)b * stride + i] : 0;
    const float w = (float)n;
    const size_t o = (size_t)b * Q + i;
    if (w_out) w_out[o] = w;
    if (exterior) exterior[o] = w <= thresh;
}

constexpr int kSegRayChunk = 128;

constexpr float kConeMarker = 3.0e38f;
__global__ __launch_bounds__(kBlock) void segment_shear_entries_kernel(
    const float* __restrict__ verts, const float* __restrict__ caps,
    const int32_t* __restrict__ ent, int V, int K, int E, float* __restrict__ out)
{
    const int b = blockIdx.y;
    const int i = blockIdx.x * kBlock + threadIdx.x;
    if (i >= E) return;
    const int id[3] = {ent[3 * i], ent[3 * i + 1], ent[3 * i + 2]};
    float* dst = out + ((size_t)b * E + i) * 9;
    const int corners = id[2] < 0 ? 2 : 3;
    for (int k = 0; k < corners; ++k) {
        const float* src = id[k] < V ? verts + ((size_t)b * V + id[k]) * 3 : caps + ((size_t)b * K + (id[k] - V)) * 3;
        dst[3 * k] = shear_x(src[0], src[2]); dst[3 * k + 1] = shear_y(src[1], src[2]); dst[3 * k + 2] = src[2];
    }
    if (corners == 2) { dst[6] = (float)id[2]; dst[7] = kConeMarker; dst[8] = 0.0f; }
}

constexpr int kItemsBlock = 256;
__global__ __launch_bounds__(kItemsBlock) void segment_items_kernel(
    const int32_t* __restrict__ count, int BS, int2* __restrict__ items, int32_t* __restrict__ items_total,
    int max_split, int grid)
{
    __shared__ int sc[kItemsBlock];
    __shared__ int base;
    const int t = threadIdx.x;
    if (t == 0) base = 0;
    __syncthreads();
    for (int c0 = 0; c0 < BS; c0 += kItemsBlock) {
        const int e = c0 + t;
        const int nb = e < BS ? (count[e] + 63) >> 6 : 0;
        sc[t] = nb;
        __syncthreads();
        for (int d = 1; d < kItemsBlock; d <<= 1) {
// ... 26 lines not shown
    const P3 u_dir = {kFanX, kFanY, kFanZ};
    const P3 us = {shear_x(kFanX, kFanZ), shear_y(kFanY, kFanZ), kFanZ};
    __shared__ float sT[kSegRayChunk * 9];
    const int ns = items_total[1];
    const int units = items_total[0] * ns;
    for (int unit = blockIdx.x; unit < units; unit += gridDim.x) {
        const int2 item = items[unit / ns];
        const int split = unit % ns;
        const int b = item.x / S, s = item.x % S, k_start = item.y;
        const int n = count[item.x];
        const int q_beg = seg_q_off[s];
        const int32_t* mine = list + (size_t)b * Qs_total + q_beg;
        const int k0 = k_start + threadIdx.x;
        const int v0 = seg_q_vidx[q_beg + mine[min(k0, n - 1)]];
        const float* vb = verts + (size_t)b * V * 3;
        const float qz = vb[3 * v0 + 2];
        const float qx = shear_x(vb[3 * v0], qz), qy = shear_y(vb[3 * v0 + 1], qz);
        const int f_seg = ent_off[s], f_cnt = ent_off[s + 1] - f_seg;
        const int per = (f_cnt + ns - 1) / ns;
        const int f_beg = f_seg + split * per, f_end = min(f_seg + f_cnt, f_beg + per);
        int crossings = 0;
        float half_sum = 0.0f;
        for (int chunk = f_beg; chunk < f_end; chunk += kSegRayChunk) {
            const int cn = min(kSegRayChunk, f_end - chunk);
            const float* src = entries + ((size_t)b * E + chunk) * 9;
            __syncthreads();
            for (int i = threadIdx.x; i < cn * 9; i += 64) sT[i] = src[i];
            __syncthreads();
            for (int f = 0; f < cn; ++f) {
                const float* t = sT + f * 9;
                if (t[7] != kConeMarker) {
                    const P3 a = {t[0] - qx, t[1] - qy, t[2] - qz}, bb = {t[3] - qx, t[4] - qy, t[5] - qz}, c = {t[6] - qx, t[7] - qy, t[8] - qz};
                    const float ea = edge_fn(bb, c), eb = edge_fn(c, a), ec = edge_fn(a, bb);
                    const float numz = ea * a.z + eb * bb.z + ec * c.z;
                    const float mn = __builtin_fminf(__builtin_fminf(ea, eb), ec), mx = __builtin_fmaxf(__builtin_fmaxf(ea, eb), ec);
                    int n1 = (int)(__builtin_fminf(mn, numz) > 0.0f) - (int)(__builtin_fmaxf(mx, numz) < 0.0f);
                    const bool edge_zero = mn * mx == 0.0f;
                    if (__builtin_amdgcn_ballot_w64(edge_zero)) {
                        const bool tie = edge_zero & (numz != 0.0f);
                        if (__builtin_amdgcn_ballot_w64(tie)) {
                            if (tie) n1 = crossing_with_ties<true>(a, bb, c, ea, eb, ec);
                        }
                    }
                    crossings += n1;
                } else {
                    const P3 bb = {t[0] - qx, t[1] - qy, t[2] - qz}, c = {t[3] - qx, t[4] - qy, t[5] - qz};
                    const bool at_query = ((bb.x == 0.0f) & (bb.y == 0.0f) & (bb.z == 0.0f)) | ((c.x == 0.0f) & (c.y == 0.0f) & (c.z == 0.0f));
                    if (!at_query) {
                        const int mult = (int)t[6];
                        const P3 pb = {__builtin_fmaf(kShearX, bb.z, bb.x), __builtin_fmaf(kShearY, bb.z, bb.y), bb.z};
                        const P3 pc = {__builtin_fmaf(kShearX, c.z, c.x), __builtin_fmaf(kShearY, c.z, c.y), c.z};
                        int c1;
                        float h1;
                        cone_term(us, bb, c, u_dir, pb, pc, c1, h1);
                        crossings += mult * c1;
                        half_sum += (float)mult * h1;
                    }
                }
            }
        }
        const size_t o = ((size_t)b * nsplit + split) * Qs_total + q_beg;
        if (k0 < n) { partial[o + k0] = crossings; partial_half[o + k0] = half_sum; }
    }
}

__device__ __forceinline__ int seg_leaf_count(const int32_t* words, int s)
{
    int32_t x = words[s >> 2];
    int c = 0;
    for (int k = 0; k <= (s & 3); ++k) {
        c = (int)(int8_t)(x & 255);
        x = (x - c) >> 8;
    }
    return c;
}

__global__ __launch_bounds__(kBlock) void segment_ray_finalize_kernel(
    const float* __restrict__ verts, const float* __restrict__ caps, const int32_t* __restrict__ partial,
    const float* __restrict__ partial_half,
    const int32_t* __restrict__ seg_of_q, const int32_t* __restrict__ seg_q_off, const int32_t* __restrict__ seg_q_vidx,
    const int32_t* __restrict__ link_off, const int32_t* __restrict__ link,
    const int32_t* __restrict__ count, const int32_t* __restrict__ list,
    const int32_t* __restrict__ leaf_counts,
    const int32_t* __restrict__ vpos, int slots, int V, int K,
    int Qs_total, int S, int nsplit, const int32_t* __restrict__ items_total, float thresh, float* __restrict__ seg_w,
    uint8_t* __restrict__ seg_ext, uint8_t* __restrict__ exterior)
{
    const int b = blockIdx.y;
    const int q = blockIdx.x * kBlock + threadIdx.x;
    const int ns = items_total[1];
    bool active = q < Qs_total;
    const int s = active ? seg_of_q[q] : 0;
    const int k = q - seg_q_off[s];
    active = active && k < count[b * S + s];
    int n = 0;
    float half_sum = 0.0f;
    int qq = 0, v = 0;
    if (active) {
        for (int sp = 0; sp < ns; ++sp) {
            n += partial[((size_t)b * nsplit + sp) * Qs_total + q];
            half_sum += partial_half[((size_t)b * nsplit + sp) * Qs_total + q];
        }
        qq = seg_q_off[s] + list[(size_t)b * Qs_total + q];
        v = seg_q_vidx[qq];
        if (leaf_counts) n += seg_leaf_count(leaf_counts + 2 * ((size_t)b * slots + vpos[v]), s);
    }
    const float* vb = verts + (size_t)b * V * 3;
    const float* cb = caps + (size_t)b * K * 3;
    const float vx = vb[3 * v], vy = vb[3 * v + 1], vz = vb[3 * v + 2];
    const float qx = shear_x(vx, vz), qy = shear_y(vy, vz);
    const P3 u_dir = {kFanX, kFanY, kFanZ};
    const P3 us = {shear_x(kFanX, kFanZ), shear_y(kFanY, kFanZ), kFanZ};
    auto cone = [&](const float* p0, const float* p1, float ax, float ay, float az, float sx, float sy, float& h, int& c) {
        const P3 pb = {p0[0] - ax, p0[1] - ay, p0[2] - az}, pc = {p1[0] - ax, p1[1] - ay, p1[2] - az};
        const P3 sb = {shear_x(p0[0], p0[2]) - sx, shear_y(p0[1], p0[2]) - sy, p0[2] - az};
        const P3 sc = {shear_x(p1[0], p1[2]) - sx, shear_y(p1[1], p1[2]) - sy, p1[2] - az};
        int c1;
        float h1;
        cone_term(us, sb, sc, u_dir, pb, pc, c1, h1);
        h += h1;
        c += c1;
    };
    const int e0 = active ? link_off[qq] : 0, e1 = active ? link_off[qq + 1] : 0;
    constexpr int kLongLinks = 16;
    if (e1 - e0 <= kLongLinks) {
        for (int e = e0; e < e1; e += 2) {
            int id[4];
            float pp[4][3];
#pragma unroll
            for (int u = 0; u < 4; ++u) id[u] = link[2 * min(e + (u >> 1), e1 - 1) + (u & 1)];
#pragma unroll
            for (int u = 0; u < 4; ++u) {
                const float* p = id[u] < V ? vb + 3 * (size_t)id[u] : cb + 3 * (size_t)(id[u] - V);
                pp[u][0] = p[0]; pp[u][1] = p[1]; pp[u][2] = p[2];
            }
#pragma unroll
            for (int h = 0; h < 2; ++h)
                if (e + h < e1) cone(pp[2 * h], pp[2 * h + 1], vx, vy, vz, qx, qy, half_sum, n);
        }
    }
    unsigned long long todo = __builtin_amdgcn_ballot_w64(e1 - e0 > kLongLinks);
    const int lane = threadIdx.x & 63;
    while (todo) {
        const int src = __builtin_ctzll(todo);
        todo &= todo - 1;
        const int le0 = __builtin_amdgcn_readlane(e0, src), le1 = __builtin_amdgcn_readlane(e1, src);
        const float lvx = __shfl(vx, src), lvy = __shfl(vy, src), lvz = __shfl(vz, src);
        const float lqx = __shfl(qx, src), lqy = __shfl(qy, src);
        float h = 0.0f;
        int cr = 0;
        for (int e = le0 + lane; e < le1; e += 64) {
            const int i0 = link[2 * e], i1 = link[2 * e + 1];
            const float* p0 = i0 < V ? vb + 3 * (size_t)i0 : cb + 3 * (size_t)(i0 - V);
            const float* p1 = i1 < V ? vb + 3 * (size_t)i1 : cb + 3 * (size_t)(i1 - V);
            const float a0[3] = {p0[0], p0[1], p0[2]}, a1[3] = {p1[0], p1[1], p1[2]};
            cone(a0, a1, lvx, lvy, lvz, lqx, lqy, h, cr);
        }
#pragma unroll
        for (int m = 32; m >= 1; m >>= 1) { h += __shfl_xor(h, m); cr += __shfl_xor(cr, m); }
        if (lane == src) { half_sum += h; n += cr; }
    }
    if (!active) return;
    const float w = (float)n - half_sum * (0.5f / kPi);
    const size_t o = (size_t)b * Qs_total + qq;
    if (seg_w) seg_w[o] = w;
    if (seg_ext) seg_ext[o] = w <= thresh;
    if (exterior && !(w <= thresh)) exterior[(size_t)b * V + v] = 1;
}

inline size_t align256(size_t x) { return (x + 255) & ~(size_t)255; }

struct RayLayout {
    size_t stream, bounds, lists, list_len, zeroed, zeroed_bytes, leaf_cnt, leaf_fill, count, leaf_off, tiles, body, pairs,
        stats, fans, qrec, ranges, total;
    int T, qblocks, cap, max_tiles, workers, columns;
    size_t seg_count;
};

constexpr int kSegFusedMaxQ = 4096;
constexpr int kSegFusedMaxCaps = 8;

template <int kWaves>
__device__ __forceinline__ void seg_fused_caps(const float* __restrict__ vb, const int32_t* __restrict__ cap_off,
                                               const int32_t* __restrict__ cap_vidx, int c_lo, int c_hi, float* s_caps)
{
    const int lane = threadIdx.x & 63, wave = threadIdx.x >> 6;
    for (int c = c_lo + wave; c < c_hi; c += kWaves) {
        float sx = 0.f, sy = 0.f, sz = 0.f;
        const int beg = cap_off[c], end = cap_off[c + 1];
        for (int k = beg + lane; k < end; k += 64) {
            const float* p = vb + 3 * cap_vidx[k];
            sx += p[0]; sy += p[1]; sz += p[2];
        }
#pragma unroll
        for (int o = 32; o > 0; o >>= 1) { sx += __shfl_down(sx, o, 64); sy += __shfl_down(sy, o, 64); sz += __shfl_down(sz, o, 64); }
        if (lane == 0) {
            const float inv = 1.0f / (float)(end - beg);
            s_caps[3 * (c - c_lo)] = sx * inv; s_caps[3 * (c - c_lo) + 1] = sy * inv; s_caps[3 * (c - c_lo) + 2] = sz * inv;
        }
    }
}

constexpr int kSegOneBlock = 512, kSegOneWaves = kSegOneBlock / 64, kSegOneChunk = 256, kSegOneZ = 8;
constexpr int kSegOneOwn = kSegFusedMaxQ / kSegOneZ;
#ifdef TUCH_SEG_CLOCKS
__device__ unsigned long long g_seg_clocks[8192][8];
#define SEG_CLOCK(i) do { if (threadIdx.x == 0) { const int blk = (blockIdx.z * gridDim.y + blockIdx.y) * gridDim.x + blockIdx.x; if (blk < 8192) g_seg_clocks[blk][i] = __builtin_amdgcn_s_memrealtime(); } } while (0)
extern "C" int tuch_debug_seg_clocks(unsigned long long* out)
{
    return hipMemcpyFromSymbol(out, HIP_SYMBOL(g_seg_clocks), sizeof(unsigned long long) * 8192 * 8) == hipSuccess ? TUCH_OK : TUCH_ERR_HIP;
}
#else
#define SEG_CLOCK(i) do { } while (0)
#endif

__global__ __launch_bounds__(kSegOneBlock) void segment_one_kernel(
    const float* __restrict__ verts, const uint8_t* __restrict__ body_flags, uint8_t* __restrict__ exterior,
    const int32_t* __restrict__ seg_q_off, const int32_t* __restrict__ seg_q_vidx,
    const int32_t* __restrict__ cap_range, const int32_t* __restrict__ cap_off, const int32_t* __restrict__ cap_vidx,
    const int32_t* __restrict__ ent_off, const int32_t* __restrict__ ent,
    const int32_t* __restrict__ link_off, const int32_t* __restrict__ link, const int32_t* __restrict__ leaf_counts,
    const int32_t* __restrict__ vpos, int slots, int V, float thresh)
{
    __shared__ int32_t s_list[kSegFusedMaxQ];
    __shared__ int32_t s_cnt[kSegOneOwn];
    __shared__ float s_half[kSegOneOwn];
    __shared__ float sT[kSegOneChunk * 9];
    __shared__ float s_caps[kSegFusedMaxCaps * 3];
    __shared__ int32_t s_wave[kSegOneWaves];
    __shared__ int32_t s_n;
    const int sg = blockIdx.x, b = blockIdx.y, z = blockIdx.z, t = threadIdx.x, lane = t & 63, wave = t >> 6;
    const float* vb = verts + (size_t)b * V * 3;
    uint8_t* eb = exterior + (size_t)b * V;
    const int q_beg = seg_q_off[sg], nq = seg_q_off[sg + 1] - q_beg;
    SEG_CLOCK(0);
    {
        const uint8_t* fb = body_flags + (size_t)b * V;
        constexpr int kRounds = kSegFusedMaxQ / kSegOneBlock;
        uint32_t interior = 0;
#pragma unroll
        for (int r = 0; r < kRounds; ++r) {
            const int q = r * kSegOneBlock + t;
            if (q < nq && fb[seg_q_vidx[q_beg + q]] == 0) interior |= 1u << r;
        }
        if (t == 0) s_n = 0;
        __syncthreads();
        for (int r = 0; r * kSegOneBlock < nq; ++r) {
            const bool in = (interior >> r) & 1u;
            const unsigned long long bal = __builtin_amdgcn_ballot_w64(in);
            if (lane == 0) s_wave[wave] = __builtin_popcountll(bal);
            __syncthreads();
            int base = s_n;
            for (int w2 = 0; w2 < wave; ++w2) base += s_wave[w2];
            if (in) s_list[base + __builtin_popcountll(bal & ((1ull << lane) - 1ull))] = r * kSegOneBlock + t;
            __syncthreads();
            if (t == 0) { int add = 0; for (int w2 = 0; w2 < kSegOneWaves; ++w2) add += s_wave[w2]; s_n += add; }
            __syncthreads();
        }
    }
    const int n = s_n;
    const int groups = (n + 63) >> 6;
    const int mine = groups > z ? (groups - z + kSegOneZ - 1) / kSegOneZ : 0;
    SEG_CLOCK(1);
    if (mine == 0) return;
    const int c_lo = cap_range[sg];
    seg_fused_caps<kSegOneWaves>(vb, cap_off, cap_vidx, c_lo, cap_range[sg + 1], s_caps);
    SEG_CLOCK(2);
    const P3 u_dir = {kFanX, kFanY, kFanZ};
    const P3 us = {shear_x(kFanX, kFanZ), shear_y(kFanY, kFanZ), kFanZ};
    const int e_beg = ent_off[sg], e_end = ent_off[sg + 1];
    const int slices = mine >= kSegOneWaves ? 1 : kSegOneWaves / mine;
    for (int j0 = 0; j0 < mine; j0 += kSegOneWaves) {
        const int j = slices > 1 ? wave / slices : j0 + wave;
        const int sl = slices > 1 ? wave % slices : 0;
        const bool have = j < mine && (slices == 1 || wave < mine * slices);
        const int k = (z + (have ? j : 0) * kSegOneZ) * 64 + lane;
        const int v0 = seg_q_vidx[q_beg + s_list[min(k, n - 1)]];
        const float qz = vb[3 * (size_t)v0 + 2];
        const float qx = shear_x(vb[3 * (size_t)v0], qz), qy = shear_y(vb[3 * (size_t)v0 + 1], qz);
        int crossings = 0;
        float half_sum = 0.0f;
        for (int chunk = e_beg; chunk < e_end; chunk += kSegOneChunk) {
            const int cn = min(kSegOneChunk, e_end - chunk);
            __syncthreads();
            for (int i = t; i < cn; i += kSegOneBlock) {
                const int id[3] = {ent[3 * (size_t)(chunk + i)], ent[3 * (size_t)(chunk + i) + 1], ent[3 * (size_t)(chunk + i) + 2]};
                float* dst = sT + i * 9;
                const int corners = id[2] < 0 ? 2 : 3;
                for (int c = 0; c < corners; ++c) {
                    const float* p = id[c] < V ? vb + 3 * (size_t)id[c] : s_caps + 3 * (id[c] - V - c_lo);
                    dst[3 * c] = shear_x(p[0], p[2]); dst[3 * c + 1] = shear_y(p[1], p[2]); dst[3 * c + 2] = p[2];
                }
                if (corners == 2) { dst[6] = (float)id[2]; dst[7] = kConeMarker; dst[8] = 0.0f; }
            }
            __syncthreads();
            if (!have) continue;
            for (int f = sl; f < cn; f += slices) {
                const float* e = sT + f * 9;
                if (e[7] != kConeMarker) {
                    const P3 a = {e[0] - qx, e[1] - qy, e[2] - qz}, bb = {e[3] - qx, e[4] - qy, e[5] - qz}, c = {e[6] - qx, e[7] - qy, e[8] - qz};
                    const float ea = edge_fn(bb, c), eb2 = edge_fn(c, a), ec = edge_fn(a, bb);
                    const float numz = ea * a.z + eb2 * bb.z + ec * c.z;
                    const float mn = __builtin_fminf(__builtin_fminf(ea, eb2), ec), mx = __builtin_fmaxf(__builtin_fmaxf(ea, eb2), ec);
                    int n1 = (int)(__builtin_fminf(mn, numz) > 0.0f) - (int)(__builtin_fmaxf(mx, numz) < 0.0f);
                    const bool edge_zero = mn * mx == 0.0f;
                    if (__builtin_amdgcn_ballot_w64(edge_zero)) {
                        const bool tie = edge_zero & (numz != 0.0f);
                        if (__builtin_amdgcn_ballot_w64(tie)) {
                            if (tie) n1 = crossing_with_ties<true>(a, bb, c, ea, eb2, ec);
                        }
                    }
                    crossings += n1;
                } else {
                    const P3 bb = {e[0] - qx, e[1] - qy, e[2] - qz}, c = {e[3] - qx, e[4] - qy, e[5] - qz};
                    const bool at_query = ((bb.x == 0.0f) & (bb.y == 0.0f) & (bb.z == 0.0f)) | ((c.x == 0.0f) & (c.y == 0.0f) & (c.z == 0.0f));
                    if (!at_query) {
                        const int mult = (int)e[6];
                        const P3 pb = {__builtin_fmaf(kShearX, bb.z, bb.x), __builtin_fmaf(kShearY, bb.z, bb.y), bb.z};
                        const P3 pc = {__builtin_fmaf(kShearX, c.z, c.x), __builtin_fmaf(kShearY, c.z, c.y), c.z};
                        int c1;
                        float h1;
                        cone_term(us, bb, c, u_dir, pb, pc, c1, h1);
                        crossings += mult * c1;
                        half_sum += (float)mult * h1;
                    }
                }
            }
        }
        if (have) {
            const int at = slices > 1 ? (sl * mine + j) * 64 + lane : j * 64 + lane;
            s_cnt[at] = crossings;
            s_half[at] = half_sum;
        }
        if (slices > 1) break;
    }
    __syncthreads();
    SEG_CLOCK(3);
    auto pos = [&](int id, float (&o)[3]) {
        const float* p = id < V ? vb + 3 * (size_t)id : s_caps + 3 * (id - V - c_lo);
        o[0] = p[0]; o[1] = p[1]; o[2] = p[2];
    };
    for (int j = wave; j < mine; j += kSegOneWaves) {
        const int k = (z + j * kSegOneZ) * 64 + lane;
        const bool active = k < n;
        const int qq = q_beg + s_list[active ? k : 0];
        const int v = seg_q_vidx[qq];
        int cnt = 0;
        float half_sum = 0.0f;
        if (active) {
            if (slices > 1) {
                for (int s2 = 0; s2 < slices; ++s2) { cnt += s_cnt[(s2 * mine + j) * 64 + lane]; half_sum += s_half[(s2 * mine + j) * 64 + lane]; }
            } else {
                cnt = s_cnt[j * 64 + lane];
                half_sum = s_half[j * 64 + lane];
            }
            cnt += seg_leaf_count(leaf_counts + 2 * ((size_t)b * slots + vpos[v]), sg);
        }
        const float vx = vb[3 * (size_t)v], vy = vb[3 * (size_t)v + 1], vz = vb[3 * (size_t)v + 2];
        const float qx = shear_x(vx, vz), qy = shear_y(vy, vz);
        auto cone = [&](const float (&p0)[3], const float (&p1)[3], float ax, float ay, float az, float sx, float sy, float& h, int& c) {
            const P3 pb = {p0[0] - ax, p0[1] - ay, p0[2] - az}, pc = {p1[0] - ax, p1[1] - ay, p1[2] - az};
            const P3 sb = {shear_x(p0[0], p0[2]) - sx, shear_y(p0[1], p0[2]) - sy, p0[2] - az};
            const P3 sc = {shear_x(p1[0], p1[2]) - sx, shear_y(p1[1], p1[2]) - sy, p1[2] - az};
            int c1;
            float h1;
            cone_term(us, sb, sc, u_dir, pb, pc, c1, h1);
            h += h1;
            c += c1;
        };
        const int e0 = active ? link_off[qq] : 0, e1 = active ? link_off[qq + 1] : 0;
        constexpr int kLongLinks = 16;
        if (e1 - e0 <= kLongLinks) {
            for (int e = e0; e < e1; e += 2) {
                int id[4];
                float pp[4][3];
#pragma unroll
                for (int u = 0; u < 4; ++u) id[u] = link[2 * min(e + (u >> 1), e1 - 1) + (u & 1)];
#pragma unroll
                for (int u = 0; u < 4; ++u) pos(id[u], pp[u]);
#pragma unroll
                for (int h = 0; h < 2; ++h)
                    if (e + h < e1) cone(pp[2 * h], pp[2 * h + 1], vx, vy, vz, qx, qy, half_sum, cnt);
            }
        }
        unsigned long long todo = __builtin_amdgcn_ballot_w64(e1 - e0 > kLongLinks);
        while (todo) {
            const int src = __builtin_ctzll(todo);
            todo &= todo - 1;
            const int le0 = __builtin_amdgcn_readlane(e0, src), le1 = __builtin_amdgcn_readlane(e1, src);
            const float lvx = __shfl(vx, src), lvy = __shfl(vy, src), lvz = __shfl(vz, src);
            const float lqx = __shfl(qx, src), lqy = __shfl(qy, src);
            float h = 0.0f;
            int cr = 0;
            for (int e = le0 + lane; e < le1; e += 64) {
                float a0[3], a1[3];
                pos(link[2 * e], a0);
                pos(link[2 * e + 1], a1);
                cone(a0, a1, lvx, lvy, lvz, lqx, lqy, h, cr);
            }
#pragma unroll
            for (int m2 = 32; m2 >= 1; m2 >>= 1) { h += __shfl_xor(h, m2); cr += __shfl_xor(cr, m2); }
            if (lane == src) { half_sum += h; cnt += cr; }
        }
        if (active) {
            const float w = (float)cnt - half_sum * (0.5f / kPi);
            if (!(w <= thresh)) eb[v] = 1;
        }
    }
    SEG_CLOCK(4);
}

}

bool tuch_ray_segment_fused_available(const tuch_contact_model* m)
{
    return m && m->seg_cap_off && m->seg_cap_range && m->seg_elem_mask && m->seg_q_max <= kSegFusedMaxQ && m->opt.seg_fused != 0;
}

int tuch_ray_segment_flags_one(const tuch_contact_model* m, const float* verts, const uint8_t* body_flags,
                               const int32_t* leaf_counts, int B, float thresh, uint8_t* exterior, hipStream_t s)
{
    hipLaunchKernelGGL(segment_one_kernel, dim3(m->num_segments, B, kSegOneZ), dim3(kSegOneBlock), 0, s, verts, body_flags, exterior,
                       (const int32_t*)m->seg_q_off, (const int32_t*)m->seg_q_vidx, (const int32_t*)m->seg_cap_range,
                       (const int32_t*)m->cap_off, (const int32_t*)m->cap_vidx, (const int32_t*)m->seg_cap_off,
                       (const int32_t*)m->seg_cap_ent, (const int32_t*)m->seg_link_off, (const int32_t*)m->seg_link, leaf_counts,
                       (const int32_t*)m->seg_vpos, 2 * m->tree_qblocks * kRayQueries, m->V, thresh);
    return tuch_check_launch("tuch_ray_segment_flags_one");
}

bool tuch_ray_available(const tuch_contact_model* m)
{
    if (!m || m->tree_nodes <= 0 || !m->ring_off || m->tree_exact_len <= 0) return false;
    if (m->tree_leaves > 65535) return false;
    return m->opt.winding_ray != 0;
}

static int ray_pair_cap(const tuch_contact_model* m) { return m->opt.ray_pair_cap < 1 ? 1 : m->opt.ray_pair_cap; }

static RayLayout full_layout(const tuch_contact_model* m, int B, int Q, bool verts)
{
    RayLayout l;
    l.qblocks = verts ? 2 * m->tree_qblocks : ceil_div(Q, kRayQueries);
    l.T = ceil_div(m->tree_exact_len, 3) * 3 + 6;
    const int L = m->tree_leaves;
    const long cap = (long)ray_pair_cap(m) * Q;
    l.cap = (int)(cap < 0x3fffffffL ? cap : 0x3fffffffL);
    l.max_tiles = l.cap / 64 + L;
    if (l.max_tiles < l.qblocks * kFallbackChunks) l.max_tiles = l.qblocks * kFallbackChunks;
    l.columns = B < 8 ? B : 8;
    const int waves = m->opt.ray_waves > 0 ? m->opt.ray_waves : 32768;
    l.workers = waves / l.columns > 0 ? waves / l.columns : 1;
    size_t o = 0;
    l.stream = tuch_ws_take(o, (size_t)B * l.T * sizeof(RayElem));
    l.bounds = tuch_ws_take(o, (size_t)B * m->tree_nodes * 2 * kSlabStride * sizeof(float));
    l.lists = tuch_ws_take(o, (size_t)B * l.qblocks * L * sizeof(RayEntry));
    l.list_len = tuch_ws_take(o, (size_t)B * l.qblocks * sizeof(int32_t));
    l.zeroed = o;
    l.leaf_cnt = tuch_ws_take(o, (size_t)B * L * sizeof(int32_t), false);
    l.leaf_fill = tuch_ws_take(o, (size_t)B * L * sizeof(int32_t), false);
    l.count = tuch_ws_take(o, (size_t)B * l.qblocks * kRayQueries * sizeof(int32_t), false);
    l.seg_count = o;
    if (verts && m->seg_elem_mask) o += align256(2 * (size_t)B * l.qblocks * kRayQueries * sizeof(int32_t));
    l.zeroed_bytes = o - l.zeroed;
    (void)tuch_ws_take(o, 0);
    l.leaf_off = tuch_ws_take(o, (size_t)B * L * sizeof(int32_t));
    l.tiles = tuch_ws_take(o, (size_t)B * l.max_tiles * sizeof(RayTile));
    l.body = tuch_ws_take(o, (size_t)B * sizeof(RayBody));
    l.pairs = tuch_ws_take(o, (size_t)B * l.cap * sizeof(int32_t));
    l.stats = tuch_ws_take(o, 256);
    l.fans = verts ? tuch_ws_take(o, (size_t)B * l.qblocks * kRayQueries * sizeof(float2)) : 0;
    l.qrec = verts ? tuch_ws_take(o, (size_t)B * l.qblocks * kRayQueries * sizeof(QRec)) : 0;
    l.ranges = verts ? tuch_ws_take(o, (size_t)B * l.qblocks * 4 * sizeof(float4)) : 0;
    l.total = o;
    return l;
}

void tuch_ray_layout_touch(const tuch_contact_model* m, int B, int Q)
{
    (void)full_layout(m, B, Q > 0 ? Q : m->V, Q <= 0);
}

size_t tuch_ray_workspace_bytes(const tuch_contact_model* m, int B, int Q)
{
    if (!m || m->tree_nodes <= 0 || B <= 0) return 0;
    const size_t a = full_layout(m, B, m->V, true).total;
    const size_t b = Q > 0 ? full_layout(m, B, Q, false).total : 0;
    return a > b ? a : b;
}

static bool fans_in_bounds_launch(const tuch_contact_model* m) { return m->ring_off && m->opt.ray_fans == 1 && m->tree_leaf_runs_tile; }
static bool cross_in_one_launch(const tuch_contact_model* m);
static bool fans_in_near_launch(const tuch_contact_model* m) { return m->ring_off && m->opt.ray_fans == 2 && !cross_in_one_launch(m); }

static bool cross_in_one_launch(const tuch_contact_model* m)
{
    return m->opt.ray_cross != 0 && 2L * m->tree_qblocks * kRayQueries < kNoSlot;
}

static void launch_ray_boxes(const tuch_contact_model* m, const RayLayout& l, const float* verts, int B, char* ws, hipStream_t s,
                             bool one_launch, bool query_side = false)
{
    RayElem* st = (RayElem*)(ws + l.stream);
    float* bounds = (float*)(ws + l.bounds);
    const RayPre pre{query_side ? ceil_div(l.qblocks, kBoundsBlock / 64) : 0, l.qblocks, (QRec*)(ws + l.qrec), (float4*)(ws + l.ranges),
                     (const int32_t*)m->seg_vmask};
    if (one_launch && m->tree_leaf_runs_tile) {
        const int leaf_blocks = ceil_div(m->tree_leaves, kBoundsBlock / 16);
        const bool fans = fans_in_bounds_launch(m);
        hipLaunchKernelGGL(ray_leaf_bounds_kernel<true>, dim3(leaf_blocks + (fans ? ceil_div(m->V, kBoundsBlock) : 0) + pre.blocks, B),
                           dim3(kBoundsBlock), 0,
                           s, (const RayElem*)st, l.T, (const TreeNode*)m->tree_node, m->tree_nodes,
                           (const int32_t*)m->tree_height_off, (const int32_t*)m->tree_height_nodes, bounds, verts,
                           (const int32_t*)m->tree_vidx, (const float*)m->tree_sign_word, m->V, m->tree_exact_len, st,
                           (uint4*)(ws + l.zeroed), l.zeroed_bytes / sizeof(uint4), fans ? leaf_blocks : 0,
                           (const int32_t*)m->tree_qperm, (const int32_t*)m->ring_off, (const int32_t*)m->ring_vidx,
                           (float2*)(ws + l.fans), l.qblocks * kRayQueries, pre);
        return;
    }
    if (query_side)
        hipLaunchKernelGGL(ray_prepass_kernel, dim3(pre.blocks, B), dim3(kBoundsBlock), 0, s, verts, (const int32_t*)m->tree_vidx,
                           (const int32_t*)m->tree_qperm, m->V, pre);
    hipLaunchKernelGGL(ray_stream_kernel, dim3(ceil_div(l.T, kBlock), B), dim3(kBlock), 0, s, verts,
                       (const int32_t*)m->tree_vidx, (const float*)m->tree_sign_word, m->V, m->tree_exact_len, l.T, st,
                       (uint4*)(ws + l.zeroed), l.zeroed_bytes / sizeof(uint4));
    hipLaunchKernelGGL(ray_leaf_bounds_kernel<false>, dim3(ceil_div(m->tree_leaves, kBoundsBlock / 16), B), dim3(kBoundsBlock), 0, s,
                       (const RayElem*)st, l.T, (const TreeNode*)m->tree_node, m->tree_nodes,
                       (const int32_t*)m->tree_height_off, (const int32_t*)m->tree_height_nodes, bounds,
                       (const float*)nullptr, (const int32_t*)nullptr, (const float*)nullptr, 0, 0, (RayElem*)nullptr,
                       (uint4*)nullptr, (size_t)0);
}

template <bool kVerts>
static int launch_ray_counts(const tuch_contact_model* m, const RayLayout& l, const float* verts, const float* queries,
                             const int32_t* counts, int B, int Q, char* ws, hipStream_t s, unsigned long long* stats)
{
    const bool one = kVerts && !stats && cross_in_one_launch(m);
    launch_ray_boxes(m, l, verts, B, ws, s, kVerts, one);
    const int L = m->tree_leaves;
    const TreeNode* nodes = (const TreeNode*)m->tree_node;
    if (one) {
        const int columns = B < 8 ? B : 8;
        int nsplit = m->opt.ray_cross_split > 0 ? m->opt.ray_cross_split : (B <= 8 ? 4 : B <= 32 ? 2 : 1);
        if (nsplit > l.qblocks) nsplit = l.qblocks;
        const dim3 grid(columns, ceil_div(B, columns) * L * nsplit);
        int32_t* seg_cnt = (int32_t*)(ws + l.seg_count);
        if (m->seg_elem_mask)
            hipLaunchKernelGGL(ray_cross_kernel<true>, grid, dim3(64), 0, s, (const RayElem*)(ws + l.stream), nodes, (const float*)(ws + l.bounds), L,
                               nsplit, (const QRec*)(ws + l.qrec), (const float4*)(ws + l.ranges), l.T, l.qblocks, B,
                               (int32_t*)(ws + l.count), seg_cnt);
        else
            hipLaunchKernelGGL(ray_cross_kernel<false>, grid, dim3(64), 0, s, (const RayElem*)(ws + l.stream), nodes, (const float*)(ws + l.bounds), L,
                               nsplit, (const QRec*)(ws + l.qrec), (const float4*)(ws + l.ranges), l.T, l.qblocks, B,
                               (int32_t*)(ws + l.count), seg_cnt);
        return TUCH_OK;
    }
    const int32_t* leaf_nodes = (const int32_t*)m->tree_height_nodes;
    const int32_t* qperm = kVerts ? (const int32_t*)m->tree_qperm : nullptr;
    RayEntry* lists = (RayEntry*)(ws + l.lists);
    int32_t* list_len = (int32_t*)(ws + l.list_len);
    int32_t* leaf_cnt = (int32_t*)(ws + l.leaf_cnt);
    int32_t* leaf_off = (int32_t*)(ws + l.leaf_off);
    RayTile* tiles = (RayTile*)(ws + l.tiles);
    RayBody* body = (RayBody*)(ws + l.body);
    int32_t* pairs = (int32_t*)(ws + l.pairs);
    const bool fans = kVerts && fans_in_near_launch(m);
    float2* fan_out = fans ? (float2*)(ws + l.fans) : nullptr;
    if ((long)l.qblocks * B <= 2048)
        hipLaunchKernelGGL((ray_near_kernel<kVerts, 4>), dim3(l.qblocks + (fans ? ceil_div(Q, 256) : 0), B), dim3(256), 0, s, queries, nodes,
                           (const float*)(ws + l.bounds), m->tree_nodes, L, qperm, counts, Q, l.qblocks, lists, list_len,
                           leaf_cnt, stats, (const int32_t*)m->ring_off, (const int32_t*)m->ring_vidx, fan_out);
    else
        hipLaunchKernelGGL((ray_near_kernel<kVerts, 1>), dim3(l.qblocks + (fans ? ceil_div(Q, 64) : 0), B), dim3(64), 0, s, queries, nodes,
                           (const float*)(ws + l.bounds), m->tree_nodes, L, qperm, counts, Q, l.qblocks, lists, list_len,
                           leaf_cnt, stats, (const int32_t*)m->ring_off, (const int32_t*)m->ring_vidx, fan_out);
    const size_t tf_lds = (2 * (size_t)L + l.qblocks + 1) * sizeof(int32_t);
    if (l.qblocks <= kFillMaxBlocks && tf_lds <= 48u * 1024)
        hipLaunchKernelGGL(ray_tiles_fill_kernel, dim3(B, std::min(256, std::max(kFillSplit, 2048 / B))), dim3(kTilesFillBlock), tf_lds, s, (const int32_t*)leaf_cnt,
                           nodes, leaf_nodes, L, l.cap, l.max_tiles, l.qblocks * kFallbackChunks, tiles, body,
                           (const RayEntry*)lists, (const int32_t*)list_len, l.qblocks, (int32_t*)(ws + l.leaf_fill), pairs, L);
    else {
    hipLaunchKernelGGL(ray_tiles_kernel, dim3(B), dim3(kTilesBlock), 0, s, (const int32_t*)leaf_cnt, nodes, leaf_nodes, L, l.cap,
                       l.max_tiles, l.qblocks * kFallbackChunks, leaf_off, tiles, body);
    hipLaunchKernelGGL(ray_fill_kernel, dim3(l.qblocks, B), dim3(64), 0, s, (const RayEntry*)lists, (const int32_t*)list_len,
                       (const RayBody*)body, (const int32_t*)leaf_off, L, l.qblocks, l.cap, (int32_t*)(ws + l.leaf_fill), pairs);
    }
    const dim3 grid(l.columns, l.workers);
    const bool seg = kVerts && m->seg_elem_mask;
    const int32_t* vmask = (const int32_t*)m->seg_vmask;
    int32_t* seg_count = (int32_t*)(ws + l.seg_count);
#define TUCH_LAUNCH_RAY_LEAF(COUNT, SEG)                                                                                      \
    hipLaunchKernelGGL((ray_leaf_kernel<kVerts, COUNT, SEG>), grid, dim3(64), 0, s, queries, (const RayElem*)(ws + l.stream),  \
                       (const RayTile*)tiles, (const RayBody*)body, (const int32_t*)pairs, (const RayEntry*)lists,            \
                       (const int32_t*)list_len, nodes, L, qperm, counts, Q, l.T, l.qblocks, B, l.cap, l.max_tiles,           \
                       (int32_t*)(ws + l.count), stats, vmask, seg_count)
    if (stats) {
        if (seg) TUCH_LAUNCH_RAY_LEAF(true, kVerts); else TUCH_LAUNCH_RAY_LEAF(true, false);
    } else {
        if (seg) TUCH_LAUNCH_RAY_LEAF(false, kVerts); else TUCH_LAUNCH_RAY_LEAF(false, false);
    }
#undef TUCH_LAUNCH_RAY_LEAF
    return TUCH_OK;
}

int tuch_ray_exterior_verts(const tuch_contact_model* m, const float* verts, int B, float thresh, uint8_t* exterior,
                            float* w, void* workspace, hipStream_t s, unsigned long long* stats_host, uint8_t* exterior_copy)
{
    const RayLayout l = full_layout(m, B, m->V, true);
    char* ws = (char*)workspace;
    unsigned long long* stats = stats_host ? (unsigned long long*)(ws + l.stats) : nullptr;
    if (stats && hipMemsetAsync(stats, 0, 4 * sizeof(unsigned long long), s) != hipSuccess) return TUCH_ERR_HIP;
    const int rc = launch_ray_counts<true>(m, l, verts, verts, nullptr, B, m->V, ws, s, stats);
    if (rc != TUCH_OK) return rc;
    if (w || exterior)
        hipLaunchKernelGGL(ray_finalize_verts_kernel, dim3(ceil_div(m->V, kBlock), B), dim3(kBlock), 0, s, verts,
                           (const int32_t*)(ws + l.count), (const int32_t*)m->tree_qperm, (const int32_t*)m->ring_off,
                           (const int32_t*)m->ring_vidx, m->V, l.qblocks * kRayQueries, thresh, w, exterior, exterior_copy,
                           (const float2*)(fans_in_bounds_launch(m) || fans_in_near_launch(m) ? ws + l.fans : nullptr));
    if (stats_host) {
        RayBody bodies[8];
        const int nb = B < 8 ? B : 8;
        if (hipMemcpyAsync(stats_host, stats, 3 * sizeof(unsigned long long), hipMemcpyDeviceToHost, s) != hipSuccess ||
            hipMemcpyAsync(bodies, ws + l.body, nb * sizeof(RayBody), hipMemcpyDeviceToHost, s) != hipSuccess ||
            hipStreamSynchronize(s) != hipSuccess)
            return TUCH_ERR_HIP;
        unsigned long long tiles = 0;
        for (int b = 0; b < nb; ++b) tiles += bodies[b].tiles;
        stats_host[3] = tiles * B / nb;
    }
    return tuch_check_launch("tuch_ray_exterior_verts");
}

const int32_t* tuch_ray_segment_counts(const tuch_contact_model* m, int B, const void* workspace)
{
    if (!m->seg_elem_mask) return nullptr;
    return (const int32_t*)((const char*)workspace + full_layout(m, B, m->V, true).seg_count);
}

int tuch_ray_exterior_points(const tuch_contact_model* m, const float* verts, const float* points, const int32_t* counts,
                             int B, int Q, float thresh, uint8_t* exterior, float* w, void* workspace, hipStream_t s)
{
    const RayLayout l = full_layout(m, B, Q, false);
    char* ws = (char*)workspace;
    const int rc = launch_ray_counts<false>(m, l, verts, points, counts, B, Q, ws, s, nullptr);
    if (rc != TUCH_OK) return rc;
    hipLaunchKernelGGL(ray_finalize_points_kernel, dim3(ceil_div(Q, kBlock), B), dim3(kBlock), 0, s,
                       (const int32_t*)(ws + l.count), counts, Q, l.qblocks * kRayQueries, thresh, w, exterior);
    return tuch_check_launch("tuch_ray_exterior_points");
}

void tuch_ray_segment_prepare(const tuch_contact_model* m, const float* verts, const float* caps, int assisted, int B,
                              float* seg_entries, hipStream_t s)
{
    const bool as = assisted && m->seg_cap_off;
    const int E = as ? m->seg_cap_total : m->seg_ray_total;
    hipLaunchKernelGGL(segment_shear_entries_kernel, dim3(ceil_div(E > 0 ? E : 1, kBlock), B), dim3(kBlock), 0, s,
                       verts, caps, (const int32_t*)(as ? m->seg_cap_ent : m->seg_ray_ent), m->V, m->num_caps, E, seg_entries);
}

int tuch_ray_segment_flags(const tuch_contact_model* m, const float* verts, const float* caps, const int32_t* seg_count,
                           const int32_t* seg_list, const int32_t* leaf_counts, int B, int nsplit, float thresh,
                           float* seg_entries, int32_t* seg_partial, float* seg_w, uint8_t* seg_ext, uint8_t* exterior,
                           hipStream_t s)
{
    const bool assisted = leaf_counts && m->seg_cap_off;
    const int E = assisted ? m->seg_cap_total : m->seg_ray_total;
    const int32_t* ent_off = (const int32_t*)(assisted ? m->seg_cap_off : m->seg_ray_off);
    float* partial_half = (float*)(seg_partial + (size_t)B * nsplit * m->seg_q_total);
    int2* items = (int2*)(partial_half + (size_t)B * nsplit * m->seg_q_total);
    int32_t* items_total = (int32_t*)(items + (size_t)B * m->num_seg_blocks);
    const long worst = (long)B * m->num_seg_blocks * nsplit;
    const int grid = (int)(worst < 8192 ? worst : 8192);
    hipLaunchKernelGGL(segment_items_kernel, dim3(1), dim3(kItemsBlock), 0, s, seg_count, B * m->num_segments, items, items_total,
                       nsplit, grid);
    hipLaunchKernelGGL(segment_ray_kernel, dim3((unsigned)grid), dim3(64), 0, s, verts,
                       (const float*)seg_entries, (const int2*)items, (const int32_t*)items_total, (const int32_t*)m->seg_q_off,
                       (const int32_t*)m->seg_q_vidx, ent_off, seg_count, seg_list, m->V, E,
                       m->seg_q_total, m->num_segments, nsplit, seg_partial, partial_half);
    hipLaunchKernelGGL(segment_ray_finalize_kernel, dim3(ceil_div(m->seg_q_total, kBlock), B), dim3(kBlock), 0, s, verts, caps,
                       (const int32_t*)seg_partial, (const float*)partial_half, (const int32_t*)m->seg_of_q,
                       (const int32_t*)m->seg_q_off, (const int32_t*)m->seg_q_vidx, (const int32_t*)m->seg_link_off,
                       (const int32_t*)m->seg_link, seg_count, seg_list, assisted ? leaf_counts : nullptr,
                       (const int32_t*)m->seg_vpos, 2 * m->tree_qblocks * kRayQueries, m->V,
                       m->num_caps, m->seg_q_total, m->num_segments, nsplit, (const int32_t*)items_total, thresh, seg_w, seg_ext,
                       exterior);
    return tuch_check_launch("tuch_ray_segment_flags");
}
```

tuch_amd/csrc/winding.hip:

```cpp
#include "common.h"
#include "model.h"
#include "workspace.h"
#include "tree_device.h"
#include <stdlib.h>

namespace {

constexpr float kPi = 3.14159265358979323846f;
constexpr float kHalfPi = 1.57079632679489661923f;
constexpr int kBlock = 256;
constexpr int kQueriesPerLane = 2;
constexpr int kQueriesPerBlock = kBlock * kQueriesPerLane;
constexpr int kStripBlock = 128;
constexpr int kStripQueries = kStripBlock * kQueriesPerLane;

__device__ __forceinline__ v2f atan_poly(v2f t)
{
    const v2f s = t * t;
    v2f p = splat2(0.0024567253421992064f);
    p = fma2(p, s, splat2(-0.014401361346244812f));
    p = fma2(p, s, splat2(0.03978123143315315f));
    p = fma2(p, s, splat2(-0.07234857976436615f));
    p = fma2(p, s, splat2(0.10498946160078049f));
    p = fma2(p, s, splat2(-0.14161229133605957f));
// ... 815 lines not shown
    TUCH_REQUIRE(B > 0 && V > 0 && F > 0, "tuch_gather_triangles: bad sizes");
    hipLaunchKernelGGL(gather_triangles_kernel, dim3(ceil_div(F * 3, kBlock), B), dim3(kBlock), 0,
                       (hipStream_t)stream, verts, faces, V, F, triangles);
    return tuch_check_launch("tuch_gather_triangles");
}

extern "C" size_t tuch_exterior_workspace_bytes(const tuch_contact_model* m, int B)
{
    if (!m || B <= 0) return 0;
    tuch_ws_scope scope(m->opt.canary != 0);
    return exterior_layout(m, B).total;
}

extern "C" int tuch_exterior_flags(const tuch_contact_model* m, const float* verts, int B,
                                   int apply_segments, float thresh, float* w, uint8_t* exterior,
                                   float* seg_w, uint8_t* seg_exterior,
                                   void* workspace, size_t workspace_bytes, void* stream)
{
    TUCH_REQUIRE(m && verts && exterior, "tuch_exterior_flags: null pointer");
    TUCH_REQUIRE(B > 0 && B <= 65535, "tuch_exterior_flags: bad batch %d", B);
    tuch_ws_scope scope(m->opt.canary != 0);
    const ExteriorLayout l = scope.record(0, [&] { return exterior_layout(m, B); });
    if (!workspace || workspace_bytes < l.total) {
        tuch_set_error("tuch_exterior_flags: workspace %zu < %zu bytes", workspace_bytes, l.total);
        return TUCH_ERR_WORKSPACE;
    }
    if (tuch_ray_available(m)) scope.record(l.ray, [&] { tuch_ray_layout_touch(m, B, 0); return 0; });
    scope.arm(workspace, m->canary_hits, (hipStream_t)stream);
    char* ws = (char*)workspace;
    float* tris = (float*)(ws + l.tris);
    hipStream_t s = (hipStream_t)stream;
    int rc = TUCH_OK;
    const int ray = ray_mode(m);
    const bool segments = apply_segments && m->num_segments > 0;
    const bool body_by_rays = ray == 2 || (ray == 1 && !w);
    const bool segments_by_rays = segments && m->seg_link_off && (ray == 2 || (ray == 1 && !seg_w));
    const bool segments_fused = segments && segments_by_rays && body_by_rays && !seg_w && !seg_exterior &&
                                tuch_ray_segment_fused_available(m);
    if (segments && !segments_fused) {
        if (m->num_caps > 0) {
            hipLaunchKernelGGL(cap_centroid_kernel, dim3(m->num_caps, B), dim3(64), 0, s,
                               verts, (const int32_t*)m->cap_off, (const int32_t*)m->cap_vidx, m->V,
                               m->num_caps, (float*)(ws + l.caps), (int32_t*)(ws + l.seg_count), m->num_segments);
        } else if (hipMemsetAsync(ws + l.seg_count, 0, (size_t)B * m->num_segments * sizeof(int32_t), s) != hipSuccess) {
            tuch_set_error("tuch_exterior_flags: hipMemsetAsync failed");
            return TUCH_ERR_HIP;
        }
        if (segments_by_rays)
            tuch_ray_segment_prepare(m, verts, (const float*)(ws + l.caps), body_by_rays && m->seg_elem_mask, B,
                                     (float*)(ws + l.seg_tris), s);
    }
    if (body_by_rays) {
        rc = tuch_ray_exterior_verts(m, verts, B, thresh, exterior, w, ws + l.ray, s, nullptr,
                                     segments_fused ? (uint8_t*)(ws + l.body_flags) : (uint8_t*)nullptr);
        if (rc != TUCH_OK) return rc;
    } else if (use_strips(m) && use_tree(m)) {
        launch_tree_walk(m, l, verts, B, ws, nullptr, s);
        hipLaunchKernelGGL(winding_finalize_tree_kernel, dim3(ceil_div(m->V, kBlock), B), dim3(kBlock), 0, s,
                           (const float*)(ws + l.partial), (const int32_t*)m->tree_qperm, m->V,
                           2 * m->tree_qblocks * kTreeQueries, l.tree_subs, thresh, w, exterior);
    } else if (use_strips(m) && m->strip_len > 0) {
        StreamElem* st = (StreamElem*)tris;
        hipLaunchKernelGGL(gather_stream_kernel, dim3(ceil_div(l.lpad, kBlock), B), dim3(kBlock), 0, s, verts,
                           (const int32_t*)m->strip_vidx, (const float*)m->strip_sign, m->V, m->strip_len,
                           l.lpad, st);
        const int nsplit = choose_strip_splits(B, m->V, l.lpad);
        const int per_split = ceil_div(ceil_div(l.lpad - 6, nsplit), 3) * 3;
        hipLaunchKernelGGL(winding_strip_kernel, dim3(B, nsplit, ceil_div(m->V, kStripQueries)), dim3(kStripBlock),
                           0, s, verts, (const StreamElem*)st, m->V, l.lpad, per_split, (const int32_t*)nullptr,
                           (float*)(ws + l.partial));
        hipLaunchKernelGGL(winding_finalize_kernel, dim3(ceil_div(m->V, kBlock), B), dim3(kBlock), 0, s,
                           (const float*)(ws + l.partial), m->V, m->V, nsplit, thresh, w, exterior);
    } else {
        hipLaunchKernelGGL(gather_triangles_kernel, dim3(ceil_div(m->F * 3, kBlock), B), dim3(kBlock), 0, s,
                           verts, (const int32_t*)m->faces, m->V, m->F, tris);
        rc = tuch_winding_numbers(verts, tris, B, m->V, m->F, w, exterior, thresh, ws + l.partial,
                                  l.bounds - l.partial, stream);
        if (rc != TUCH_OK) return rc;
    }
    if (segments_fused) {
        rc = tuch_ray_segment_flags_one(m, verts, (const uint8_t*)(ws + l.body_flags), tuch_ray_segment_counts(m, B, ws + l.ray), B, thresh,
                                        exterior, s);
        if (rc != TUCH_OK) return rc;
    } else if (segments) {
        float* caps = (float*)(ws + l.caps);
        float* seg_tris = (float*)(ws + l.seg_tris);
        float* seg_partial = (float*)(ws + l.seg_partial);
        int32_t* seg_count = (int32_t*)(ws + l.seg_count);
        int32_t* seg_list = (int32_t*)(ws + l.seg_list);
        const bool all = seg_w || seg_exterior;
        hipLaunchKernelGGL(segment_compact_kernel, dim3(ceil_div(m->seg_q_total, kBlock), B), dim3(kBlock), 0, s,
                           all ? (const uint8_t*)nullptr : (const uint8_t*)exterior, (const int32_t*)m->seg_of_q,
                           (const int32_t*)m->seg_q_off, (const int32_t*)m->seg_q_vidx, m->V, m->seg_q_total,
                           m->num_segments, seg_count, seg_list);
        if (segments_by_rays) {
            rc = tuch_ray_segment_flags(m, verts, caps, seg_count, seg_list,
                                        body_by_rays ? tuch_ray_segment_counts(m, B, ws + l.ray) : nullptr, B, seg_splits(m),
                                        thresh, seg_tris, (int32_t*)seg_partial, seg_w, seg_exterior, exterior, s);
            if (rc != TUCH_OK) return rc;
            return tuch_check_launch("tuch_exterior_flags");
        }
        hipLaunchKernelGGL(gather_segment_triangles_kernel, dim3(ceil_div(m->seg_f_total * 3, kBlock), B),
                           dim3(kBlock), 0, s, verts, (const float*)caps, (const int32_t*)m->seg_faces,
                           m->V, m->num_caps, m->seg_f_total, seg_tris);
        hipLaunchKernelGGL(segment_winding_kernel, dim3(B, seg_splits(m), m->num_seg_blocks), dim3(kSegBlock),
                           0, s, verts, (const float*)seg_tris, (const int32_t*)m->seg_blocks,
                           (const int32_t*)m->seg_q_off, (const int32_t*)m->seg_q_vidx,
                           (const int32_t*)m->seg_f_off, (const int32_t*)seg_count, (const int32_t*)seg_list,
                           m->V, m->seg_f_total, m->seg_q_total, m->num_segments, seg_partial);
        hipLaunchKernelGGL(segment_finalize_kernel, dim3(ceil_div(m->seg_q_total, kBlock), B), dim3(kBlock), 0, s,
                           (const float*)seg_partial, (const int32_t*)m->seg_of_q, (const int32_t*)m->seg_q_off,
                           (const int32_t*)m->seg_q_vidx, (const int32_t*)seg_count, (const int32_t*)seg_list,
                           m->V, m->seg_q_total, m->num_segments, seg_splits(m), thresh, seg_w, seg_exterior, exterior);
    }
    return tuch_check_launch("tuch_exterior_flags");
}

extern "C" int tuch_winding_tree_work(const tuch_contact_model* m, const float* verts, int B,
                                      void* workspace, size_t workspace_bytes, unsigned long long* out_host, void* stream)
{
    TUCH_REQUIRE(m && verts && out_host, "tuch_winding_tree_work: null pointer");
    TUCH_REQUIRE(m->tree_nodes > 0, "tuch_winding_tree_work: the model has no cluster tree");
    TUCH_REQUIRE(B > 0 && B <= 65535, "tuch_winding_tree_work: bad batch %d", B);
    const ExteriorLayout l = exterior_layout(m, B);
    if (!workspace || workspace_bytes < l.total) {
        tuch_set_error("tuch_winding_tree_work: workspace %zu < %zu bytes", workspace_bytes, l.total);
        return TUCH_ERR_WORKSPACE;
    }
    char* ws = (char*)workspace;
    hipStream_t s = (hipStream_t)stream;
    unsigned long long* stats = (unsigned long long*)(ws + l.stats);
    if (hipMemsetAsync(stats, 0, 2 * sizeof(unsigned long long), s) != hipSuccess) return TUCH_ERR_HIP;
    launch_tree_walk(m, l, verts, B, ws, stats, s);
    if (hipMemcpyAsync(out_host, stats, 2 * sizeof(unsigned long long), hipMemcpyDeviceToHost, s) != hipSuccess ||
        hipStreamSynchronize(s) != hipSuccess) {
        tuch_set_error("tuch_winding_tree_work: copy back failed");
        return TUCH_ERR_HIP;
    }
    out_host[2] = (unsigned long long)B * l.tree_subs * m->tree_qblocks * 2;
    out_host[3] = (unsigned long long)m->strip_len;
    return tuch_check_launch("tuch_winding_tree_work");
}

extern "C" int tuch_ray_work(const tuch_contact_model* m, const float* verts, int B, void* workspace,
                             size_t workspace_bytes, unsigned long long* out_host, void* stream)
{
    TUCH_REQUIRE(m && verts && out_host, "tuch_ray_work: null pointer");
    TUCH_REQUIRE(tuch_ray_available(m), "tuch_ray_work: the model has no cluster tree / vertex rings");
    TUCH_REQUIRE(B > 0 && B <= 65535, "tuch_ray_work: bad batch %d", B);
    const ExteriorLayout l = exterior_layout(m, B);
    if (!workspace || workspace_bytes < l.total) {
        tuch_set_error("tuch_ray_work: workspace %zu < %zu bytes", workspace_bytes, l.total);
        return TUCH_ERR_WORKSPACE;
    }
    return tuch_ray_exterior_verts(m, verts, B, 0.99f, nullptr, nullptr, (char*)workspace + l.ray, (hipStream_t)stream, out_host);
}

struct PointsLayout { size_t stream, bounds, partial, total; int frontier, nsub, qblocks; };

static PointsLayout points_layout(const tuch_contact_model* m, int B, int Q)
{
    PointsLayout l;
    l.qblocks = ceil_div(Q, kTreeQueries);
    int f = 0;
    while (f + 1 < m->tree_num_frontiers &&
           (long)B * l.qblocks * (m->tree_frontier_off_host[f + 1] - m->tree_frontier_off_host[f]) < 65536L) ++f;
    l.frontier = f;
    l.nsub = m->tree_frontier_off_host[f + 1] - m->tree_frontier_off_host[f];
    size_t o = 0;
    l.stream = tuch_ws_take(o, (size_t)B * (m->tree_stream_len + 3) * sizeof(StreamElem));
    l.bounds = tuch_ws_take(o, (size_t)B * m->tree_nodes * 2 * kSlabStride * sizeof(float));
    l.partial = tuch_ws_take(o, (size_t)B * l.nsub * l.qblocks * kTreeQueries * sizeof(float));
    l.total = o;
    return l;
}

extern "C" size_t tuch_winding_points_workspace_bytes(const tuch_contact_model* m, int B, int Q)
{
    if (!m || B <= 0 || Q <= 0) return 0;
    tuch_ws_scope scope(m->opt.canary != 0);
    const int lpad = strip_lpad(m->strip_len);
    const size_t flat = align256((size_t)B * lpad * sizeof(StreamElem)) +
                        align256((size_t)B * choose_strip_splits(B, Q, lpad) * Q * sizeof(float));
    if (m->tree_nodes <= 0) return flat;
    size_t tree = points_layout(m, B, Q).total;
    const size_t ray = tuch_ray_workspace_bytes(m, B, Q);
    if (ray > tree) tree = ray;
    return tree > flat ? tree : flat;
}

extern "C" int tuch_winding_points(const tuch_contact_model* m, const float* verts, const float* points,
                                   const int32_t* counts, int B, int Q, float thresh, float* w,
                                   uint8_t* exterior, void* workspace, size_t workspace_bytes, void* stream)
{
    TUCH_REQUIRE(m && verts && points && (w || exterior), "tuch_winding_points: null pointer");
    TUCH_REQUIRE(B > 0 && B <= 65535 && Q > 0, "tuch_winding_points: bad sizes B=%d Q=%d", B, Q);
    const size_t need = tuch_winding_points_workspace_bytes(m, B, Q);
    if (!workspace || workspace_bytes < need) {
        tuch_set_error("tuch_winding_points: workspace %zu < %zu bytes", workspace_bytes, need);
        return TUCH_ERR_WORKSPACE;
    }
    hipStream_t s = (hipStream_t)stream;
    const int ray = ray_mode(m);
    tuch_ws_scope scope(m->opt.canary != 0);
    if (ray == 2 || (ray == 1 && !w)) {
        scope.record(0, [&] { tuch_ray_layout_touch(m, B, Q); return 0; });
        scope.arm(workspace, m->canary_hits, s);
        return tuch_ray_exterior_points(m, verts, points, counts, B, Q, thresh, exterior, w, workspace, s);
    }
    if (use_strips(m) && use_tree(m)) {
// ... 40 lines not shown
```

tuch_amd/ops.py:

```python
from __future__ import annotations

import contextlib
import ctypes
import os
import weakref
from typing import Dict, List, Optional, Sequence, Tuple

import numpy as np
import torch
from torch.autograd.function import once_differentiable

from . import _C, backward_pass
from .backward_pass import backward_scalar

MODE_SMPLIFY = 0
MODE_TRAIN = 1


def _f32(t: torch.Tensor) -> torch.Tensor:
    if t.dtype is torch.float32 and t.is_contiguous():
        return t.detach()
    return t.detach().to(torch.float32).contiguous()


# ... 795 lines not shown
        sign = np.zeros(n.value, np.float32)
        _C.check(L.tuch_contact_model_strips(self._handle, None, None, vidx.ctypes.data_as(ctypes.c_void_p),
                                             sign.ctypes.data_as(ctypes.c_void_p)))
        return vidx, sign, k.value

    def exterior_and_partner(self, verts: torch.Tensor, apply_segments: bool = True, also=None, zero_floats: int = 0,
                             iterative: bool = False, cap: Optional[float] = None):
        zero = torch.empty((int(zero_floats) + 3) // 4 * 4, dtype=torch.float32, device=verts.device) if zero_floats > 0 else None
        call_also = (lambda: None) if also is None else also if zero is None else (lambda: also(zero))
        capped = cap is not None and verts.is_cuda and self.v2v_can_cap(verts.shape[0])
        overlap = bool(verts.is_cuda and self._py_options['overlap'])
        if overlap:
            cur, side = _current_stream(verts.device), _side_stream(verts.device)
            side.wait_stream(cur)
        first = not overlap or capped or self._py_options.get('inside_first', 0)
        exterior = self.exterior_flags(verts, apply_segments=apply_segments) if first else None
        with (torch.cuda.stream(side) if overlap else contextlib.nullcontext()):
            if overlap and zero is not None:
                zero.record_stream(side)
            mn, partner, *state = self.v2v_min(verts, leave_room=overlap, zero=zero, iterative=iterative,
                                               cap=cap if capped else None)
            if capped and not overlap:
                self.v2v_fix(exterior, mn, partner, state[0])
            extra = call_also()
        if not first:
            exterior = self.exterior_flags(verts, apply_segments=apply_segments)
        if overlap:
            cur.wait_stream(side)
            for t in (mn, partner, *(st[0] for st in state), *(extra if isinstance(extra, (tuple, list)) else (extra,))):
                if torch.is_tensor(t):
                    t.record_stream(cur)
            if capped:
                self.v2v_fix(exterior, mn, partner, state[0])
        return exterior, mn, partner, extra

    def winding_tree_work(self, verts: torch.Tensor) -> dict:
        verts = _f32(verts)
        b = verts.shape[0]
        L = _C.lib()
        nbytes = L.tuch_exterior_workspace_bytes(self._handle, b)
        ws = _workspace(nbytes, verts.device)
        out = (ctypes.c_ulonglong * 4)()
        _C.check(L.tuch_winding_tree_work(self._handle, _C.ptr(verts), b, _C.ptr(ws), nbytes, out, _C.stream()))
        return dict(leaf_elements=int(out[0]), cap_elements=int(out[1]), wavefronts=int(out[2]),
                    flat_stream_elements=int(out[3]), queries_per_step=64,
                    query_blocks=-(-self.num_verts // 128) * 2 * b)

    def ray_work(self, verts: torch.Tensor) -> dict:
        verts = _f32(verts)
        b = verts.shape[0]
        L = _C.lib()
        nbytes = L.tuch_exterior_workspace_bytes(self._handle, b)
        ws = _workspace(nbytes, verts.device)
        out = (ctypes.c_ulonglong * 4)()
        _C.check(L.tuch_ray_work(self._handle, _C.ptr(verts), b, _C.ptr(ws), nbytes, out, _C.stream()))
        return dict(elements=int(out[0]), wavefronts=int(out[3]), queries_per_step=64,
                    lanes_inside_leaf_slabs=int(out[1]) / max(int(out[2]), 1))

    def exterior_flags(self, verts: torch.Tensor, apply_segments: bool = True, thresh: float = 0.99,
                       return_details: bool = False):
        verts = _f32(verts)
        b = verts.shape[0]
        assert verts.shape[1] == self.num_verts
        L = _C.lib()
        ext = torch.empty(b, self.num_verts, dtype=torch.uint8, device=verts.device)
        w = torch.empty(b, self.num_verts, dtype=torch.float32, device=verts.device) if return_details else None
        seg_w = seg_e = None
        if return_details and self.num_segments:
            seg_w = torch.empty(b, self.seg_q_total, dtype=torch.float32, device=verts.device)
            seg_e = torch.empty(b, self.seg_q_total, dtype=torch.uint8, device=verts.device)
        nbytes = L.tuch_exterior_workspace_bytes(self._handle, b)
        ws = _workspace(nbytes, verts.device)
        _C.check(L.tuch_exterior_flags(self._handle, _C.ptr(verts), b, int(apply_segments), float(thresh),
                                       _C.ptr(w), _C.ptr(ext), _C.ptr(seg_w), _C.ptr(seg_e), _C.ptr(ws), nbytes,
                                       _C.stream()))
        return (ext, w, seg_w, seg_e) if return_details else ext

    def v2v_min(self, verts: torch.Tensor, leave_room: bool = False, zero: Optional[torch.Tensor] = None, iterative: bool = False,
                cap: Optional[float] = None):
        if not self.has_mask:
            raise _C.TuchError('ContactModel was created without a geodesic mask')
        verts = _f32(verts)
        b = verts.shape[0]
        assert verts.shape[1] == self.num_verts
        L = _C.lib()
        mn = torch.empty(b, self.num_verts, dtype=torch.float32, device=verts.device)
        arg = torch.empty(b, self.num_verts, dtype=torch.int32, device=verts.device)
        nbytes = L.tuch_v2v_model_workspace_bytes(self._handle, b)
        ws = _workspace(nbytes, verts.device)
        flags = int(bool(leave_room)) | (2 if iterative else 0)
        zbytes = zero.numel() * zero.element_size() if zero is not None else 0
        if cap is not None:
            prev = self._v2v_prev(b)
            _C.check(L.tuch_v2v_min_model_capped(self._handle, _C.ptr(verts), b, _C.ptr(mn), _C.ptr(arg), _C.ptr(self._v2v_hint(b)),
                                                 _C.ptr(ws), nbytes, flags, _C.ptr(zero), zbytes, _C.ptr(prev), float(cap), _C.stream()))
            return mn, arg, (ws, nbytes, prev, float(cap))
        _C.check(L.tuch_v2v_min_model_shared_zero(self._handle, _C.ptr(verts), b, _C.ptr(mn), _C.ptr(arg),
                                                  _C.ptr(self._v2v_hint(b)), _C.ptr(ws), nbytes, flags, _C.ptr(zero), zbytes, _C.stream()))
        return mn, arg

    def v2v_can_cap(self, batch: int) -> bool:
        return bool(self.has_mask and _C.lib().tuch_v2v_min_model_can_cap(self._handle)) and self._v2v_hint(batch) is not None

    def v2v_fix(self, exterior: torch.Tensor, mn: torch.Tensor, arg: torch.Tensor, state) -> None:
        ws, nbytes, prev, cap = state
        b = exterior.shape[0]
        _C.check(_C.lib().tuch_v2v_min_model_fix(self._handle, b, _C.ptr(exterior), _C.ptr(prev), cap, _C.ptr(mn), _C.ptr(arg),
                                                 _C.ptr(self._v2v_hint(b)), _C.ptr(ws), nbytes, _C.stream()))

    def _v2v_prev(self, batch: int) -> torch.Tensor:
# ... 181 lines not shown
```

Before: 151,500 body-fit iterations/s.

## Pick per-block ray direction (+z or -z) minimizing candidate leaf count

Adds a mirrored set of leaf bounding records (z negated) and, per query block, counts how many leaves pass the slab test for rays cast along +z versus -z, then traces the cheaper direction. The goal is to cut ray-triangle work in the inside/outside test by choosing the direction that crosses fewer leaf clusters. In exchange it adds an extra pass over all leaf records per block, extra workspace for the mirrored records and a direction array, plus a direction flag that the finalize kernels must respect. A debug API to read back the chosen directions is also added.

```diff
diff --git a/include/tuch_amd.h b/include/tuch_amd.h
--- a/include/tuch_amd.h
+++ b/include/tuch_amd.h
@@ -146,6 +146,8 @@
 
 int tuch_ray_work(const tuch_contact_model* model, const float* verts, int B, void* workspace,
                   size_t workspace_bytes, unsigned long long* out_host, void* stream);
+int tuch_ray_directions(const tuch_contact_model* model, const float* verts, int B, void* workspace,
+                        size_t workspace_bytes, int32_t* dir_out, void* stream);
 int tuch_contact_model_tree_order(const tuch_contact_model* model, int32_t* qperm_host, int32_t* face_leaf_host);
 
 size_t tuch_v2v_model_workspace_bytes(const tuch_contact_model* model, int B);
diff --git a/tuch_amd/_C.py b/tuch_amd/_C.py
--- a/tuch_amd/_C.py
+++ b/tuch_amd/_C.py
@@ -91,6 +91,7 @@
     'tuch_hd_contact_selection': (c_int, [c_void_p, c_void_p, c_int, c_void_p, c_void_p]),
     'tuch_hd_contact_details': (c_int, [c_void_p, c_void_p, c_int, c_void_p, c_void_p]),
     'tuch_ray_work': (c_int, [c_void_p, c_void_p, c_int, c_void_p, c_size_t, c_void_p, c_void_p]),
+    'tuch_ray_directions': (c_int, [c_void_p, c_void_p, c_int, c_void_p, c_size_t, c_void_p, c_void_p]),
     'tuch_contact_model_tree_order': (c_int, [c_void_p, c_void_p, c_void_p]),
     'tuch_v2v_model_workspace_bytes': (c_size_t, [c_void_p, c_int]),
     'tuch_v2v_hint_bytes': (c_size_t, [c_void_p, c_int]),
diff --git a/tuch_amd/csrc/api.hip b/tuch_amd/csrc/api.hip
--- a/tuch_amd/csrc/api.hip
+++ b/tuch_amd/csrc/api.hip
@@ -23,7 +23,7 @@
 }
 
 extern "C" const char* tuch_last_error(void) { return g_error; }
-extern "C" int tuch_abi_version(void) { return 1; }
+extern "C" int tuch_abi_version(void) { return 2; }
 
 #include <stdlib.h>
 static int g_deterministic = [] { const char* e = getenv("TUCH_DETERMINISTIC"); return e && atoi(e) == 0 ? 0 : 1; }();
diff --git a/tuch_amd/csrc/model.h b/tuch_amd/csrc/model.h
--- a/tuch_amd/csrc/model.h
+++ b/tuch_amd/csrc/model.h
@@ -31,6 +31,7 @@
     int ray_waves = 32768;
     int ray_fans = 0;
     int ray_cross = 0;
+    int ray_dir = 1;
     int ray_cross_split = 0;
     int v2v_tree = 1;
     int v2v_waves = 0;
@@ -57,7 +58,9 @@
 size_t tuch_ray_workspace_bytes(const tuch_contact_model* m, int B, int Q);
 int tuch_ray_exterior_verts(const tuch_contact_model* m, const float* verts, int B, float thresh, uint8_t* exterior,
                             float* w, void* workspace, hipStream_t s, unsigned long long* stats_host,
-                            uint8_t* exterior_copy = nullptr);
+                            uint8_t* exterior_copy = nullptr, bool plus_only = false);
+const int32_t* tuch_ray_dir(const tuch_contact_model* m, int B, const void* workspace);
+int tuch_ray_dir_active(const tuch_contact_model* m);
 const int32_t* tuch_ray_segment_counts(const tuch_contact_model* m, int B, const void* workspace);
 void tuch_ray_segment_prepare(const tuch_contact_model* m, const float* verts, const float* caps, int assisted, int B,
                               float* seg_entries, hipStream_t s);
diff --git a/tuch_amd/csrc/model.hip b/tuch_amd/csrc/model.hip
--- a/tuch_amd/csrc/model.hip
+++ b/tuch_amd/csrc/model.hip
@@ -451,7 +451,7 @@
 const OptionName kOptions[] = {
     {"winding_ray", &tuch_options::winding_ray}, {"winding_tree", &tuch_options::winding_tree},
     {"winding_strips", &tuch_options::winding_strips}, {"tree_waves", &tuch_options::tree_waves},
-    {"ray_pair_cap", &tuch_options::ray_pair_cap}, {"ray_waves", &tuch_options::ray_waves}, {"ray_fans", &tuch_options::ray_fans}, {"ray_cross", &tuch_options::ray_cross}, {"v2v_cap", &tuch_options::v2v_cap}, {"ray_cross_split", &tuch_options::ray_cross_split},
+    {"ray_pair_cap", &tuch_options::ray_pair_cap}, {"ray_waves", &tuch_options::ray_waves}, {"ray_fans", &tuch_options::ray_fans}, {"ray_cross", &tuch_options::ray_cross}, {"v2v_cap", &tuch_options::v2v_cap}, {"ray_cross_split", &tuch_options::ray_cross_split}, {"ray_dir", &tuch_options::ray_dir},
     {"v2v_tree", &tuch_options::v2v_tree}, {"v2v_flat", &tuch_options::v2v_flat}, {"v2v_pairs", &tuch_options::v2v_pairs}, {"v2v_waves", &tuch_options::v2v_waves}, {"v2v_lds", &tuch_options::v2v_lds},
     {"seg_splits", &tuch_options::seg_splits}, {"seg_assist", &tuch_options::seg_assist}, {"seg_fused", &tuch_options::seg_fused},
     {"canary", &tuch_options::canary}, {"hd_search", &tuch_options::hd_search}, {"hd_search_waves", &tuch_options::hd_search_waves}, {"hd_overlap", &tuch_options::hd_overlap},
@@ -501,6 +501,10 @@
     TUCH_REQUIRE(m && name && value, "tuch_contact_model_get_option: null argument");
     if (!strcmp(name, "seg_fused_active")) {
         *value = tuch_ray_segment_fused_available(m) ? 1 : 0;
+        return TUCH_OK;
+    }
+    if (!strcmp(name, "ray_dir_active")) {
+        *value = tuch_ray_dir_active(m);
         return TUCH_OK;
     }
     for (const OptionName& k : kOptions)
diff --git a/tuch_amd/csrc/ray_winding.hip b/tuch_amd/csrc/ray_winding.hip
--- a/tuch_amd/csrc/ray_winding.hip
+++ b/tuch_amd/csrc/ray_winding.hip
@@ -108,7 +108,7 @@
     }
 }
 
-__device__ __forceinline__ float fan_terms(const float* __restrict__ vb, int v, bool real, int& n,
+__device__ __forceinline__ float fan_terms(const float* __restrict__ vb, int v, bool real, bool mirror, int& n,
                                            const int32_t* __restrict__ ring_off, const int32_t* __restrict__ ring_vidx);
 template <bool kPose>
 __global__ __launch_bounds__(kBoundsBlock) void ray_leaf_bounds_kernel(
@@ -118,7 +118,8 @@
     RayElem* __restrict__ stream_out, uint4* __restrict__ zeroed, size_t zeroed_n,
     int leaf_blocks = 0, const int32_t* __restrict__ qperm = nullptr, const int32_t* __restrict__ ring_off = nullptr,
     const int32_t* __restrict__ ring_vidx = nullptr, float2* __restrict__ fans = nullptr, int fan_stride = 0,
-    RayPre pre = RayPre{0, 0, nullptr, nullptr, nullptr})
+    RayPre pre = RayPre{0, 0, nullptr, nullptr, nullptr},
+    uint4* __restrict__ records_m = nullptr)
 {
     if (kPose && pre.blocks > 0 && (int)blockIdx.x >= (int)gridDim.x - pre.blocks) {
         for (size_t g = ((size_t)blockIdx.y * gridDim.x + blockIdx.x) * kBoundsBlock + threadIdx.x; g < zeroed_n;
@@ -139,7 +140,7 @@
         const bool real = i < V;
         const int v = qperm[real ? i : V - 1];
         int cr = 0;
-        const float half = fan_terms(verts + (size_t)blockIdx.y * V * 3, v, real, cr, ring_off, ring_vidx);
+        const float half = fan_terms(verts + (size_t)blockIdx.y * V * 3, v, real, false, cr, ring_off, ring_vidx);
         if (i < fan_stride) fans[(size_t)blockIdx.y * fan_stride + i] = make_float2(__int_as_float(cr), half);
         return;
     }
@@ -207,6 +208,11 @@
         r[0] = make_uint4(lo_h[0] | lo_h[1] << 16, lo_h[3] | lo_h[4] << 16, lo_h[6] | lo_h[8] << 16, hi_h[0] | hi_h[1] << 16);
         r[1] = make_uint4(hi_h[2] | hi_h[3] << 16, hi_h[4] | hi_h[5] << 16, hi_h[7] | (uint32_t)leaf << 16, (uint32_t)node);
         if (leaf == 0) *reinterpret_cast<float4*>(bounds + near_centres_at(gridDim.y, L) + (size_t)b * 4) = make_float4(c[0], c[1], c[2], 0.f);
+        if (records_m) {
+            uint4* rm = records_m + ((size_t)b * L + leaf) * 2;
+            rm[0] = make_uint4(lo_h[0] | lo_h[1] << 16, lo_h[3] | lo_h[4] << 16, lo_h[5] | lo_h[7] << 16, hi_h[0] | hi_h[1] << 16);
+            rm[1] = make_uint4((lo_h[2] ^ 0x8000u) | hi_h[3] << 16, hi_h[4] | hi_h[6] << 16, hi_h[8] | (uint32_t)leaf << 16, (uint32_t)node);
+        }
     }
 }
 
@@ -276,12 +282,12 @@
 __device__ __forceinline__ P3 p3(const S3& a) { return P3{a.xy.x, a.xy.y, a.z}; }
 
 template <int A, bool kSkipIncident, bool kSeg>
-__device__ __forceinline__ void ray_step(const RayElem el, S3 (&s)[3], float (&e)[3], v2f qxy, float qz, int& count,
+__device__ __forceinline__ void ray_step(const RayElem el, S3 (&s)[3], float (&e)[3], v2f qxy, float sg, float nqz, int& count,
                                          int qmask, uint32_t& pa, uint32_t& pb)
 {
     constexpr int Bq = (A + 1) % 3, Cq = (A + 2) % 3;
     s[A].xy = (v2f){el.x, el.y} - qxy;
-    s[A].z = el.z - qz;
+    s[A].z = __builtin_fmaf(sg, el.z, nqz);
     e[Bq] = edge_fn(s[Cq], s[A]);
     e[Cq] = edge_fn(s[A], s[Bq]);
     const int word = __float_as_int(el.sign);
@@ -312,7 +318,7 @@
 
 template <bool kSkipIncident, bool kSeg>
 __device__ __forceinline__ void ray_run(const RayElem* __restrict__ st, int off, int len,
-                                        S3 (&s)[3], float (&e)[3], v2f qxy, float qz, int& count,
+                                        S3 (&s)[3], float (&e)[3], v2f qxy, float sg, float nqz, int& count,
                                         int qmask, uint32_t& pa, uint32_t& pb)
 {
     const RayElem* p = st + off;
@@ -321,9 +327,9 @@
         asm("" : "+s"(left));
         const RayElem e0 = n0, e1 = n1, e2 = n2;
         n0 = p[3]; n1 = p[4]; n2 = p[5];
-        ray_step<0, kSkipIncident, kSeg>(e0, s, e, qxy, qz, count, qmask, pa, pb);
-        ray_step<1, kSkipIncident, kSeg>(e1, s, e, qxy, qz, count, qmask, pa, pb);
-        ray_step<2, kSkipIncident, kSeg>(e2, s, e, qxy, qz, count, qmask, pa, pb);
+        ray_step<0, kSkipIncident, kSeg>(e0, s, e, qxy, sg, nqz, count, qmask, pa, pb);
+        ray_step<1, kSkipIncident, kSeg>(e1, s, e, qxy, sg, nqz, count, qmask, pa, pb);
+        ray_step<2, kSkipIncident, kSeg>(e2, s, e, qxy, sg, nqz, count, qmask, pa, pb);
     }
 }
 
@@ -372,14 +378,17 @@
     int32_t* __restrict__ leaf_cnt,
     unsigned long long* __restrict__ stats,
     const int32_t* __restrict__ ring_off = nullptr, const int32_t* __restrict__ ring_vidx = nullptr,
-    float2* __restrict__ fans = nullptr)
+    float2* __restrict__ fans = nullptr,
+    const uint4* __restrict__ records_m = nullptr,
+    int32_t* __restrict__ dir = nullptr,
+    int dir_mode = 0)
 {
     if (kVerts && (int)blockIdx.x >= qblocks) {
         const int i = ((int)blockIdx.x - qblocks) * (64 * kWaves) + (int)threadIdx.x;
         const bool real = i < Q;
         const int v = qperm[real ? i : Q - 1];
         int cr = 0;
-        const float half = fan_terms(pts + (size_t)blockIdx.y * Q * 3, v, real, cr, ring_off, ring_vidx);
+        const float half = fan_terms(pts + (size_t)blockIdx.y * Q * 3, v, real, false, cr, ring_off, ring_vidx);
         if (i < qblocks * kRayQueries) fans[(size_t)blockIdx.y * qblocks * kRayQueries + i] = make_float2(__int_as_float(cr), half);
         return;
     }
@@ -387,8 +396,9 @@
     const int qb = blockIdx.x, b = blockIdx.y, lane = threadIdx.x & 63;
     const int wave = kWaves > 1 ? __builtin_amdgcn_readfirstlane(threadIdx.x >> 6) : 0;
     __shared__ uint4 queue[64 * kWaves][2];
-    __shared__ float range[16];
+    __shared__ float range[20];
     __shared__ int queued[2], slots;
+    __shared__ int passing[2];
     int i0;
     bool real;
     if (kVerts) {
@@ -397,15 +407,16 @@
     } else {
         const int n = counts ? counts[b] : Q;
         if (qb * kRayQueries >= n) {
-            if (threadIdx.x == 0) list_len[(size_t)b * qblocks + qb] = 0;
+            if (threadIdx.x == 0) { list_len[(size_t)b * qblocks + qb] = 0; if (dir) dir[(size_t)b * qblocks + qb] = 1; }
             return;
         }
         i0 = min(qb * kRayQueries + lane, n - 1);
         real = qb * kRayQueries + lane < n;
     }
-    if (threadIdx.x == 0) { queued[0] = 0; queued[1] = 0; slots = 0; }
+    if (threadIdx.x == 0) { queued[0] = 0; queued[1] = 0; slots = 0; passing[0] = 0; passing[1] = 0; }
     const float4 ctr = *reinterpret_cast<const float4*>(bounds + near_centres_at(gridDim.y, num_leaves) + (size_t)b * 4);
     const uint4* recs = reinterpret_cast<const uint4*>(bounds + near_records_at(gridDim.y, num_leaves)) + (size_t)b * num_leaves * 2;
+    const uint4* recs_m = records_m + (size_t)b * num_leaves * 2;
     struct Chunk { uint4 r0, r1; };
     auto load_chunk = [&](int base) {
         Chunk c;
@@ -414,13 +425,17 @@
         c.r1 = recs[lc * 2 + 1];
         return c;
     };
-    Chunk nxt = load_chunk(wave * 64);
+    Chunk nxt = Chunk{make_uint4(0u, 0u, 0u, 0u), make_uint4(0u, 0u, 0u, 0u)};
+    if (!dir_mode) nxt = load_chunk(wave * 64);
     const float* q3 = pts + ((size_t)b * Q + i0) * 3;
     const float qz = q3[2];
     const float qx = shear_x(q3[0], qz), qy = shear_y(q3[1], qz);
-    const float rx = qx - ctr.x, ry = qy - ctr.y, rz = qz - ctr.z;
-    const float r4 = rx + ry, r5 = rx - ry, r6 = rx + rz, r7 = rx - rz, r8 = ry + rz, r9 = ry - rz;
+    const float rx = qx - ctr.x, ry = qy - ctr.y;
+    float rz = qz - ctr.z;
+    const float r4 = rx + ry, r5 = rx - ry;
+    float r6 = rx + rz, r7 = rx - rz, r8 = ry + rz, r9 = ry - rz;
     float bx0, bx1, by0, by1, b40, b41, b50, b51, bz0, b60, b71, b80, b91;
+    float mz0 = 0.f, m60 = 0.f, m71 = 0.f, m80 = 0.f, m91 = 0.f;
     if (kWaves == 4) {
         if (wave == 0) {
             const float a = wave_min(rx), c = wave_max(rx), d = wave_min(ry), e = wave_max(ry);
@@ -431,17 +446,27 @@
         } else if (wave == 2) {
             const float a = wave_min(rz), c = wave_min(r6), d = wave_max(r7);
             if (lane == 0) { range[8] = a; range[9] = c; range[10] = d; }
+            if (dir_mode) {
+                const float f = -wave_max(rz), g = wave_min(r7);
+                if (lane == 0) { range[13] = f; range[14] = g; }
+            }
         } else {
             const float a = wave_min(r8), c = wave_max(r9);
             if (lane == 0) { range[11] = a; range[12] = c; }
+            if (dir_mode) {
+                const float f = wave_max(r6), g = wave_min(r9), h = wave_max(r8);
+                if (lane == 0) { range[15] = f; range[16] = g; range[17] = h; }
+            }
         }
         __syncthreads();
         bx0 = range[0]; bx1 = range[1]; by0 = range[2]; by1 = range[3]; b40 = range[4]; b41 = range[5]; b50 = range[6];
         b51 = range[7]; bz0 = range[8]; b60 = range[9]; b71 = range[10]; b80 = range[11]; b91 = range[12];
+        if (dir_mode) { mz0 = range[13]; m60 = range[14]; m71 = range[15]; m80 = range[16]; m91 = range[17]; }
     } else {
         bx0 = wave_min(rx); bx1 = wave_max(rx); by0 = wave_min(ry); by1 = wave_max(ry);
         b40 = wave_min(r4); b41 = wave_max(r4); b50 = wave_min(r5); b51 = wave_max(r5);
         bz0 = wave_min(rz); b60 = wave_min(r6); b71 = wave_max(r7); b80 = wave_min(r8); b91 = wave_max(r9);
+        if (dir_mode) { mz0 = -wave_max(rz); m60 = wave_min(r7); m71 = wave_max(r6); m80 = wave_min(r9); m91 = wave_max(r8); }
     }
     RayEntry* list = lists + ((size_t)b * qblocks + qb) * num_leaves;
     unsigned long long useful = 0, listed = 0;
@@ -454,6 +479,48 @@
         out = max3(out, minus_hi(xz0, s1.y), lo_minus(s0.z, xz1));
         return max3(out, minus_lo(yz0, s1.z), hi_minus(s0.z, yz1));
     };
+    bool minus = dir_mode == 2;
+    if (dir_mode == 1) {
+        int np = 0, nm = 0;
+        struct Both { uint4 r0, r1, m1; uint32_t m0z; };
+        auto load_both = [&](int base) {
+            Both c;
+            const int lc = min(base + lane, num_leaves - 1);
+            c.r0 = recs[lc * 2];
+            c.r1 = recs[lc * 2 + 1];
+            c.m1 = recs_m[lc * 2 + 1];
+            c.m0z = reinterpret_cast<const uint32_t*>(recs_m + lc * 2)[2];
+            return c;
+        };
+        Both ahead = load_both(wave * 64);
+        for (int base = wave * 64; base < num_leaves; base += 64 * kWaves) {
+            const Both c = ahead;
+            if (base + 64 * kWaves < num_leaves) ahead = load_both(base + 64 * kWaves);
+            const uint4 m0 = make_uint4(c.r0.x, c.r0.y, c.m0z, c.r0.w);
+            const bool in = base + lane < num_leaves;
+            const float out_p = outside13(c.r0, c.r1, bx1, bx0, by1, by0, b41, b40, b51, b50, bz0, b60, b71, b80, b91);
+            const float out_m = outside13(m0, c.m1, bx1, bx0, by1, by0, b41, b40, b51, b50, mz0, m60, m71, m80, m91);
+            np += __builtin_popcountll(__builtin_amdgcn_ballot_w64(in & !(out_p > 0.0f)));
+            nm += __builtin_popcountll(__builtin_amdgcn_ballot_w64(in & !(out_m > 0.0f)));
+        }
+        if (kWaves > 1) {
+            if (lane == 0) { atomicAdd(&passing[0], np); atomicAdd(&passing[1], nm); }
+            __syncthreads();
+            np = passing[0];
+            nm = passing[1];
+        }
+        minus = __builtin_amdgcn_readfirstlane(nm < np);
+    }
+    if (minus) {
+        recs = recs_m;
+        rz = -rz;
+        const float t6 = r6, t8 = r8;
+        r6 = r7; r7 = t6; r8 = r9; r9 = t8;
+        bz0 = mz0; b60 = m60; b71 = m71; b80 = m80; b91 = m91;
+    }
+    if (dir && threadIdx.x == 0) dir[(size_t)b * qblocks + qb] = minus ? -1 : 1;
+    if (stats && minus && threadIdx.x == 0) atomicAdd(stats + 3, 1ull);
+    if (dir_mode) nxt = load_chunk(wave * 64);
     auto outside = [&](const uint4& s0, const uint4& s1) {
         return outside13(s0, s1, rx, rx, ry, ry, r4, r4, r5, r5, rz, r6, r7, r8, r9);
     };
@@ -683,14 +750,15 @@
     const int32_t* __restrict__ list_len, const TreeNode* __restrict__ nodes, int num_leaves,
     const int32_t* __restrict__ qperm, const int32_t* __restrict__ counts, int Q, int T, int qblocks, int num_bodies,
     int cap, int max_tiles, int32_t* __restrict__ count, unsigned long long* __restrict__ stats,
-    const int32_t* __restrict__ vmask, int32_t* __restrict__ seg_count)
+    const int32_t* __restrict__ vmask, int32_t* __restrict__ seg_count,
+    const int32_t* __restrict__ dir)
 {
     const int lane = threadIdx.x;
-    struct Work { int b, off, len, slot, qmask; bool active; float qx, qy, qz; };
+    struct Work { int b, off, len, slot, qmask; bool active; float qx, qy, sg, nqz; };
     int b_cur = blockIdx.x, base = 0, g = blockIdx.y;
     auto fetch = [&]() {
         Work w;
-        w.b = -1; w.off = w.len = w.slot = 0; w.qmask = 0; w.active = false; w.qx = w.qy = w.qz = 0.0f;
+        w.b = -1; w.off = w.len = w.slot = 0; w.qmask = 0; w.active = false; w.qx = w.qy = w.nqz = 0.0f; w.sg = 1.0f;
         while (b_cur < num_bodies) {
             const int b = b_cur;
             const int nt = __builtin_amdgcn_readfirstlane(body[b].tiles);
@@ -716,9 +784,11 @@
                 w.off = t;
                 w.len = -1;
             }
-            w.qz = pb[3 * i0 + 2];
-            w.qx = shear_x(pb[3 * i0], w.qz);
-            w.qy = shear_y(pb[3 * i0 + 1], w.qz);
+            if (dir) w.sg = (float)dir[(size_t)b * qblocks + (w.slot >> 6)];
+            const float qz = pb[3 * i0 + 2];
+            w.qx = shear_x(pb[3 * i0], qz);
+            w.qy = shear_y(pb[3 * i0 + 1], qz);
+            w.nqz = -w.sg * qz;
             if (kSeg) w.qmask = vmask[w.slot];
             break;
         }
@@ -738,7 +808,7 @@
         uint32_t pa = kSegBias, pb = kSegBias;
         const RayElem* st = stream + (size_t)w.b * T;
         if (w.len >= 0) {
-            ray_run<kVerts, kSeg>(st, w.off, w.len, s, e, qxy, w.qz, crossings, w.qmask, pa, pb);
+            ray_run<kVerts, kSeg>(st, w.off, w.len, s, e, qxy, w.sg, w.nqz, crossings, w.qmask, pa, pb);
             if (kCount) walked += w.len;
         } else {
             const int qb = w.off / kFallbackChunks, c = w.off % kFallbackChunks;
@@ -746,15 +816,17 @@
             const RayEntry* list = lists + ((size_t)w.b * qblocks + qb) * num_leaves;
             for (int j = c; j < cnt; j += kFallbackChunks) {
                 const TreeNode nd = nodes[__builtin_amdgcn_readfirstlane(list[j].node)];
-                ray_run<kVerts, kSeg>(st, nd.ex_off, nd.ex_len, s, e, qxy, w.qz, crossings, w.qmask, pa, pb);
+                ray_run<kVerts, kSeg>(st, nd.ex_off, nd.ex_len, s, e, qxy, w.sg, w.nqz, crossings, w.qmask, pa, pb);
                 if (kCount) walked += nd.ex_len;
             }
         }
-        if (w.active && crossings != 0) atomicAdd(&count[((size_t)w.b * qblocks) * kRayQueries + w.slot], crossings);
+        const bool neg = w.sg < 0.0f;
+        if (w.active && crossings != 0) atomicAdd(&count[((size_t)w.b * qblocks) * kRayQueries + w.slot], neg ? -crossings : crossings);
         if (kSeg && w.active && (pa != kSegBias || pb != kSegBias)) {
             int32_t* sc = seg_count + 2 * (((size_t)w.b * qblocks) * kRayQueries + w.slot);
-            if (pa != kSegBias) atomicAdd(sc, (int32_t)(pa - kSegBias));
-            if (pb != kSegBias) atomicAdd(sc + 1, (int32_t)(pb - kSegBias));
+            const int32_t da = (int32_t)(pa - kSegBias), db = (int32_t)(pb - kSegBias);
+            if (da != 0) atomicAdd(sc, neg ? -da : da);
+            if (db != 0) atomicAdd(sc + 1, neg ? -db : db);
         }
     }
     if (kCount && lane == 0) atomicAdd(stats, (unsigned long long)walked);
@@ -870,7 +942,7 @@
         for (int u = 0; u < 3; ++u) { s[u].xy = (v2f){0.0f, 0.0f}; s[u].z = 0.0f; e[u] = 0.0f; }
         int crossings = 0;
         uint32_t pa = kSegBias, pb = kSegBias;
-        ray_run<true, kSeg>(st, ex_off, ex_len, s, e, (v2f){w.x, w.y}, w.z, crossings, (int)((uint32_t)w.tag >> 24), pa, pb);
+        ray_run<true, kSeg>(st, ex_off, ex_len, s, e, (v2f){w.x, w.y}, 1.0f, -w.z, crossings, (int)((uint32_t)w.tag >> 24), pa, pb);
         if (active && crossings != 0) atomicAdd(&count[((size_t)b * qblocks) * kRayQueries + slot], crossings);
         if (kSeg && active && (pa != kSegBias || pb != kSegBias)) {
             int32_t* sc = seg_count + 2 * (((size_t)b * qblocks) * kRayQueries + slot);
@@ -916,13 +988,14 @@
 }
 
 __device__ __forceinline__ void cone_term(const P3& us, const P3& sb, const P3& sc, const P3& u, const P3& pb, const P3& pc,
-                                          int& crossings, float& half)
+                                          bool mirror, int& crossings, float& half)
 {
     const float ea = edge_fn(sb, sc), eb = edge_fn(sc, us), ec = edge_fn(us, sb);
     const float d = ea * us.z + eb * sb.z + ec * sc.z;
     const bool la = left_of(ea, sb, sc), lb = left_of(eb, sc, us), lc = left_of(ec, us, sb);
     const bool front = d >= 0.0f;
-    crossings = (la & lb & lc) ? (int)front : ((!la & !lb & !lc) ? -(int)!front : 0);
+    const bool left = la & lb & lc, right = !la & !lb & !lc;
+    crossings = mirror ? (left ? -(int)!front : (right ? (int)front : 0)) : (left ? (int)front : (right ? -(int)!front : 0));
     const float nu = __builtin_sqrtf(u.x * u.x + u.y * u.y + u.z * u.z);
     const float nb = __builtin_sqrtf(pb.x * pb.x + pb.y * pb.y + pb.z * pb.z);
     const float nc = __builtin_sqrtf(pc.x * pc.x + pc.y * pc.y + pc.z * pc.z);
@@ -935,7 +1008,7 @@
     half = fast_atan2(front ? num : -num, den);
 }
 
-__device__ __forceinline__ float fan_terms(const float* __restrict__ vb, int v, bool real, int& n,
+__device__ __forceinline__ float fan_terms(const float* __restrict__ vb, int v, bool real, bool mirror, int& n,
                                            const int32_t* __restrict__ ring_off, const int32_t* __restrict__ ring_vidx)
 {
     const float vx = vb[3 * v], vy = vb[3 * v + 1], vz = vb[3 * v + 2];
@@ -963,7 +1036,7 @@
                 const P3 sc = {shear_x(cc[u][0], cc[u][2]) - qx, shear_y(cc[u][1], cc[u][2]) - qy, cc[u][2] - vz};
                 int cr;
                 float hf;
-                cone_term(us, sb, sc, u_dir, pb, pc, cr, hf);
+                cone_term(us, sb, sc, u_dir, pb, pc, mirror, cr, hf);
                 half_sum += hf;
                 n += cr;
                 pb = pc;
@@ -988,7 +1061,7 @@
                     const P3 sc = {shear_x(cc[u][0], cc[u][2]) - qx, shear_y(cc[u][1], cc[u][2]) - qy, cc[u][2] - vz};
                     int cr;
                     float hf;
-                    cone_term(us, sb, sc, u_dir, pb, pc, cr, hf);
+                    cone_term(us, sb, sc, u_dir, pb, pc, mirror, cr, hf);
                     half_sum += hf;
                     n += cr;
                     pb = pc;
@@ -1004,6 +1077,7 @@
         todo &= todo - 1;
         const int llo = __builtin_amdgcn_readlane(lo, src), lcnt = __builtin_amdgcn_readlane(cnt, src);
         const float lvx = __shfl(vx, src), lvy = __shfl(vy, src), lvz = __shfl(vz, src);
+        const bool lmirror = __builtin_amdgcn_readlane((int)mirror, src) != 0;
         float h = 0.0f;
         int cr = 0;
         for (int j = lane; j < lcnt; j += 64) {
@@ -1015,7 +1089,7 @@
             const P3 sb = {shear_x(bx, bz) - lqx, shear_y(by, bz) - lqy, bz - lvz}, sc = {shear_x(cx, cz) - lqx, shear_y(cy, cz) - lqy, cz - lvz};
             int c1;
             float h1;
-            cone_term(us, sb, sc, u_dir, pb, pc, c1, h1);
+            cone_term(us, sb, sc, u_dir, pb, pc, lmirror, c1, h1);
             h += h1;
             cr += c1;
         }
@@ -1025,10 +1099,10 @@
     }
     return half_sum;
 }
-__device__ __forceinline__ float fan_winding(const float* __restrict__ vb, int v, bool real, int n,
+__device__ __forceinline__ float fan_winding(const float* __restrict__ vb, int v, bool real, bool mirror, int n,
                                              const int32_t* __restrict__ ring_off, const int32_t* __restrict__ ring_vidx)
 {
-    const float half_sum = fan_terms(vb, v, real, n, ring_off, ring_vidx);
+    const float half_sum = fan_terms(vb, v, real, mirror, n, ring_off, ring_vidx);
     return (float)n - half_sum * (0.5f / kPi);
 }
 
@@ -1037,24 +1111,26 @@
     const int32_t* __restrict__ ring_off, const int32_t* __restrict__ ring_vidx,
     int V, int stride, float thresh, float* __restrict__ w_out, uint8_t* __restrict__ exterior,
     uint8_t* __restrict__ exterior_copy,
-    const float2* __restrict__ fans)
+    const float2* __restrict__ fans,
+    const int32_t* __restrict__ dir)
 {
     const int b = blockIdx.y;
     const int i = blockIdx.x * kBlock + threadIdx.x;
     const bool real = i < V;
     const int v = qperm[real ? i : V - 1];
     const int n = count[(size_t)b * stride + (real ? i : V - 1)];
+    const bool mirror = dir && dir[(size_t)b * (stride >> 6) + ((real ? i : V - 1) >> 6)] < 0;
     float w;
     if (fans) {
         const float2 f = fans[(size_t)b * stride + (real ? i : V - 1)];
         w = (float)(n + __float_as_int(f.x)) - f.y * (0.5f / kPi);
     } else
-        w = fan_winding(verts + (size_t)b * V * 3, v, real, n, ring_off, ring_vidx);
+        w = fan_winding(verts + (size_t)b * V * 3, v, real, mirror, n, ring_off, ring_vidx);
     const size_t o = (size_t)b * V + v;
     if (real) {
         if (w_out) w_out[o] = w;
         if (exterior) exterior[o] = w <= thresh;
-        if (exterior_copy) exterior_copy[o] = w <= thresh;
+        if (exterior_copy) exterior_copy[o] = (uint8_t)(w <= thresh) | (mirror ? 2 : 0);
     }
 }
 
@@ -1187,7 +1263,7 @@
                         const P3 pc = {__builtin_fmaf(kShearX, c.z, c.x), __builtin_fmaf(kShearY, c.z, c.y), c.z};
                         int c1;
                         float h1;
-                        cone_term(us, bb, c, u_dir, pb, pc, c1, h1);
+                        cone_term(us, bb, c, u_dir, pb, pc, false, c1, h1);
                         crossings += mult * c1;
                         half_sum += (float)mult * h1;
                     }
@@ -1252,7 +1328,7 @@
         const P3 sc = {shear_x(p1[0], p1[2]) - sx, shear_y(p1[1], p1[2]) - sy, p1[2] - az};
         int c1;
         float h1;
-        cone_term(us, sb, sc, u_dir, pb, pc, c1, h1);
+        cone_term(us, sb, sc, u_dir, pb, pc, false, c1, h1);
         h += h1;
         c += c1;
     };
@@ -1307,7 +1383,7 @@
 
 struct RayLayout {
     size_t stream, bounds, lists, list_len, zeroed, zeroed_bytes, leaf_cnt, leaf_fill, count, leaf_off, tiles, body, pairs,
-        stats, fans, qrec, ranges, total;
+        stats, fans, qrec, ranges, records_m, dir, total;
     int T, qblocks, cap, max_tiles, workers, columns;
     size_t seg_count;
 };
@@ -1369,14 +1445,14 @@
     uint8_t* eb = exterior + (size_t)b * V;
     const int q_beg = seg_q_off[sg], nq = seg_q_off[sg + 1] - q_beg;
     SEG_CLOCK(0);
+    const uint8_t* fb = body_flags + (size_t)b * V;
     {
-        const uint8_t* fb = body_flags + (size_t)b * V;
         constexpr int kRounds = kSegFusedMaxQ / kSegOneBlock;
         uint32_t interior = 0;
 #pragma unroll
         for (int r = 0; r < kRounds; ++r) {
             const int q = r * kSegOneBlock + t;
-            if (q < nq && fb[seg_q_vidx[q_beg + q]] == 0) interior |= 1u << r;
+            if (q < nq && (fb[seg_q_vidx[q_beg + q]] & 1) == 0) interior |= 1u << r;
         }
         if (t == 0) s_n = 0;
         __syncthreads();
@@ -1413,7 +1489,9 @@
         const int v0 = seg_q_vidx[q_beg + s_list[min(k, n - 1)]];
         const float qz = vb[3 * (size_t)v0 + 2];
         const float qx = shear_x(vb[3 * (size_t)v0], qz), qy = shear_y(vb[3 * (size_t)v0 + 1], qz);
-        int crossings = 0;
+        const bool mirror = (fb[v0] & 2) != 0;
+        const float sg = mirror ? -1.0f : 1.0f, nqz = -sg * qz;
+        int crossings = 0, face_crossings = 0;
         float half_sum = 0.0f;
         for (int chunk = e_beg; chunk < e_end; chunk += kSegOneChunk) {
             const int cn = min(kSegOneChunk, e_end - chunk);
@@ -1433,7 +1511,8 @@
             for (int f = sl; f < cn; f += slices) {
                 const float* e = sT + f * 9;
                 if (e[7] != kConeMarker) {
-                    const P3 a = {e[0] - qx, e[1] - qy, e[2] - qz}, bb = {e[3] - qx, e[4] - qy, e[5] - qz}, c = {e[6] - qx, e[7] - qy, e[8] - qz};
+                    const P3 a = {e[0] - qx, e[1] - qy, __builtin_fmaf(sg, e[2], nqz)}, bb = {e[3] - qx, e[4] - qy, __builtin_fmaf(sg, e[5], nqz)},
+                             c = {e[6] - qx, e[7] - qy, __builtin_fmaf(sg, e[8], nqz)};
                     const float ea = edge_fn(bb, c), eb2 = edge_fn(c, a), ec = edge_fn(a, bb);
                     const float numz = ea * a.z + eb2 * bb.z + ec * c.z;
                     const float mn = __builtin_fminf(__builtin_fminf(ea, eb2), ec), mx = __builtin_fmaxf(__builtin_fmaxf(ea, eb2), ec);
@@ -1445,7 +1524,7 @@
                             if (tie) n1 = crossing_with_ties<true>(a, bb, c, ea, eb2, ec);
                         }
                     }
-                    crossings += n1;
+                    face_crossings += n1;
                 } else {
                     const P3 bb = {e[0] - qx, e[1] - qy, e[2] - qz}, c = {e[3] - qx, e[4] - qy, e[5] - qz};
                     const bool at_query = ((bb.x == 0.0f) & (bb.y == 0.0f) & (bb.z == 0.0f)) | ((c.x == 0.0f) & (c.y == 0.0f) & (c.z == 0.0f));
@@ -1455,7 +1534,7 @@
                         const P3 pc = {__builtin_fmaf(kShearX, c.z, c.x), __builtin_fmaf(kShearY, c.z, c.y), c.z};
                         int c1;
                         float h1;
-                        cone_term(us, bb, c, u_dir, pb, pc, c1, h1);
+                        cone_term(us, bb, c, u_dir, pb, pc, mirror, c1, h1);
                         crossings += mult * c1;
                         half_sum += (float)mult * h1;
                     }
@@ -1464,7 +1543,7 @@
         }
         if (have) {
             const int at = slices > 1 ? (sl * mine + j) * 64 + lane : j * 64 + lane;
-            s_cnt[at] = crossings;
+            s_cnt[at] = crossings + (mirror ? -face_crossings : face_crossings);
             s_half[at] = half_sum;
         }
         if (slices > 1) break;
@@ -1493,13 +1572,14 @@
         }
         const float vx = vb[3 * (size_t)v], vy = vb[3 * (size_t)v + 1], vz = vb[3 * (size_t)v + 2];
         const float qx = shear_x(vx, vz), qy = shear_y(vy, vz);
-        auto cone = [&](const float (&p0)[3], const float (&p1)[3], float ax, float ay, float az, float sx, float sy, float& h, int& c) {
+        const bool mirror = (fb[v] & 2) != 0;
+        auto cone = [&](const float (&p0)[3], const float (&p1)[3], float ax, float ay, float az, float sx, float sy, bool mir, float& h, int& c) {
             const P3 pb = {p0[0] - ax, p0[1] - ay, p0[2] - az}, pc = {p1[0] - ax, p1[1] - ay, p1[2] - az};
             const P3 sb = {shear_x(p0[0], p0[2]) - sx, shear_y(p0[1], p0[2]) - sy, p0[2] - az};
             const P3 sc = {shear_x(p1[0], p1[2]) - sx, shear_y(p1[1], p1[2]) - sy, p1[2] - az};
             int c1;
             float h1;
-            cone_term(us, sb, sc, u_dir, pb, pc, c1, h1);
+            cone_term(us, sb, sc, u_dir, pb, pc, mir, c1, h1);
             h += h1;
             c += c1;
         };
@@ -1515,7 +1595,7 @@
                 for (int u = 0; u < 4; ++u) pos(id[u], pp[u]);
 #pragma unroll
                 for (int h = 0; h < 2; ++h)
-                    if (e + h < e1) cone(pp[2 * h], pp[2 * h + 1], vx, vy, vz, qx, qy, half_sum, cnt);
+                    if (e + h < e1) cone(pp[2 * h], pp[2 * h + 1], vx, vy, vz, qx, qy, mirror, half_sum, cnt);
             }
         }
         unsigned long long todo = __builtin_amdgcn_ballot_w64(e1 - e0 > kLongLinks);
@@ -1525,13 +1605,14 @@
             const int le0 = __builtin_amdgcn_readlane(e0, src), le1 = __builtin_amdgcn_readlane(e1, src);
             const float lvx = __shfl(vx, src), lvy = __shfl(vy, src), lvz = __shfl(vz, src);
             const float lqx = __shfl(qx, src), lqy = __shfl(qy, src);
+            const bool lmirror = __builtin_amdgcn_readlane((int)mirror, src) != 0;
             float h = 0.0f;
             int cr = 0;
             for (int e = le0 + lane; e < le1; e += 64) {
                 float a0[3], a1[3];
                 pos(link[2 * e], a0);
                 pos(link[2 * e + 1], a1);
-                cone(a0, a1, lvx, lvy, lvz, lqx, lqy, h, cr);
+                cone(a0, a1, lvx, lvy, lvz, lqx, lqy, lmirror, h, cr);
             }
 #pragma unroll
             for (int m2 = 32; m2 >= 1; m2 >>= 1) { h += __shfl_xor(h, m2); cr += __shfl_xor(cr, m2); }
@@ -1606,6 +1687,8 @@
     l.fans = verts ? tuch_ws_take(o, (size_t)B * l.qblocks * kRayQueries * sizeof(float2)) : 0;
     l.qrec = verts ? tuch_ws_take(o, (size_t)B * l.qblocks * kRayQueries * sizeof(QRec)) : 0;
     l.ranges = verts ? tuch_ws_take(o, (size_t)B * l.qblocks * 4 * sizeof(float4)) : 0;
+    l.records_m = tuch_ws_take(o, (size_t)B * L * 2 * sizeof(uint4));
+    l.dir = tuch_ws_take(o, (size_t)B * l.qblocks * sizeof(int32_t));
     l.total = o;
     return l;
 }
@@ -1632,9 +1715,17 @@
     return m->opt.ray_cross != 0 && 2L * m->tree_qblocks * kRayQueries < kNoSlot;
 }
 
+static int ray_dir_mode(const tuch_contact_model* m, bool verts, bool plus_only)
+{
+    if (plus_only || m->opt.ray_dir == 0) return 0;
+    if (verts && (m->opt.ray_cross != 0 || fans_in_bounds_launch(m) || fans_in_near_launch(m))) return 0;
+    return m->opt.ray_dir == 2 ? 2 : 1;
+}
+
 static void launch_ray_boxes(const tuch_contact_model* m, const RayLayout& l, const float* verts, int B, char* ws, hipStream_t s,
-                             bool one_launch, bool query_side = false)
-{
+                             bool one_launch, bool query_side, bool mirrored)
+{
+    uint4* records_m = mirrored ? (uint4*)(ws + l.records_m) : nullptr;
     RayElem* st = (RayElem*)(ws + l.stream);
     float* bounds = (float*)(ws + l.bounds);
     const RayPre pre{query_side ? ceil_div(l.qblocks, kBoundsBlock / 64) : 0, l.qblocks, (QRec*)(ws + l.qrec), (float4*)(ws + l.ranges),
@@ -1649,7 +1740,7 @@
                            (const int32_t*)m->tree_vidx, (const float*)m->tree_sign_word, m->V, m->tree_exact_len, st,
                            (uint4*)(ws + l.zeroed), l.zeroed_bytes / sizeof(uint4), fans ? leaf_blocks : 0,
                            (const int32_t*)m->tree_qperm, (const int32_t*)m->ring_off, (const int32_t*)m->ring_vidx,
-                           (float2*)(ws + l.fans), l.qblocks * kRayQueries, pre);
+                           (float2*)(ws + l.fans), l.qblocks * kRayQueries, pre, records_m);
         return;
     }
     if (query_side)
@@ -1662,15 +1753,16 @@
                        (const RayElem*)st, l.T, (const TreeNode*)m->tree_node, m->tree_nodes,
                        (const int32_t*)m->tree_height_off, (const int32_t*)m->tree_height_nodes, bounds,
                        (const float*)nullptr, (const int32_t*)nullptr, (const float*)nullptr, 0, 0, (RayElem*)nullptr,
-                       (uint4*)nullptr, (size_t)0);
+                       (uint4*)nullptr, (size_t)0, 0, (const int32_t*)nullptr, (const int32_t*)nullptr, (const int32_t*)nullptr,
+                       (float2*)nullptr, 0, RayPre{0, 0, nullptr, nullptr, nullptr}, records_m);
 }
 
 template <bool kVerts>
 static int launch_ray_counts(const tuch_contact_model* m, const RayLayout& l, const float* verts, const float* queries,
-                             const int32_t* counts, int B, int Q, char* ws, hipStream_t s, unsigned long long* stats)
+                             const int32_t* counts, int B, int Q, char* ws, hipStream_t s, unsigned long long* stats, int dir_mode)
 {
     const bool one = kVerts && !stats && cross_in_one_launch(m);
-    launch_ray_boxes(m, l, verts, B, ws, s, kVerts, one);
+    launch_ray_boxes(m, l, verts, B, ws, s, kVerts, one, dir_mode != 0);
     const int L = m->tree_leaves;
     const TreeNode* nodes = (const TreeNode*)m->tree_node;
     if (one) {
@@ -1700,14 +1792,17 @@
     int32_t* pairs = (int32_t*)(ws + l.pairs);
     const bool fans = kVerts && fans_in_near_launch(m);
     float2* fan_out = fans ? (float2*)(ws + l.fans) : nullptr;
+    int32_t* dir = dir_mode ? (int32_t*)(ws + l.dir) : nullptr;
     if ((long)l.qblocks * B <= 2048)
         hipLaunchKernelGGL((ray_near_kernel<kVerts, 4>), dim3(l.qblocks + (fans ? ceil_div(Q, 256) : 0), B), dim3(256), 0, s, queries, nodes,
                            (const float*)(ws + l.bounds), m->tree_nodes, L, qperm, counts, Q, l.qblocks, lists, list_len,
-                           leaf_cnt, stats, (const int32_t*)m->ring_off, (const int32_t*)m->ring_vidx, fan_out);
+                           leaf_cnt, stats, (const int32_t*)m->ring_off, (const int32_t*)m->ring_vidx, fan_out,
+                           (const uint4*)(ws + l.records_m), dir, dir_mode);
     else
         hipLaunchKernelGGL((ray_near_kernel<kVerts, 1>), dim3(l.qblocks + (fans ? ceil_div(Q, 64) : 0), B), dim3(64), 0, s, queries, nodes,
                            (const float*)(ws + l.bounds), m->tree_nodes, L, qperm, counts, Q, l.qblocks, lists, list_len,
-                           leaf_cnt, stats, (const int32_t*)m->ring_off, (const int32_t*)m->ring_vidx, fan_out);
+                           leaf_cnt, stats, (const int32_t*)m->ring_off, (const int32_t*)m->ring_vidx, fan_out,
+                           (const uint4*)(ws + l.records_m), dir, dir_mode);
     const size_t tf_lds = (2 * (size_t)L + l.qblocks + 1) * sizeof(int32_t);
     if (l.qblocks <= kFillMaxBlocks && tf_lds <= 48u * 1024)
         hipLaunchKernelGGL(ray_tiles_fill_kernel, dim3(B, std::min(256, std::max(kFillSplit, 2048 / B))), dim3(kTilesFillBlock), tf_lds, s, (const int32_t*)leaf_cnt,
@@ -1727,7 +1822,7 @@
     hipLaunchKernelGGL((ray_leaf_kernel<kVerts, COUNT, SEG>), grid, dim3(64), 0, s, queries, (const RayElem*)(ws + l.stream),  \
                        (const RayTile*)tiles, (const RayBody*)body, (const int32_t*)pairs, (const RayEntry*)lists,            \
                        (const int32_t*)list_len, nodes, L, qperm, counts, Q, l.T, l.qblocks, B, l.cap, l.max_tiles,           \
-                       (int32_t*)(ws + l.count), stats, vmask, seg_count)
+                       (int32_t*)(ws + l.count), stats, vmask, seg_count, (const int32_t*)dir)
     if (stats) {
         if (seg) TUCH_LAUNCH_RAY_LEAF(true, kVerts); else TUCH_LAUNCH_RAY_LEAF(true, false);
     } else {
@@ -1738,19 +1833,22 @@
 }
 
 int tuch_ray_exterior_verts(const tuch_contact_model* m, const float* verts, int B, float thresh, uint8_t* exterior,
-                            float* w, void* workspace, hipStream_t s, unsigned long long* stats_host, uint8_t* exterior_copy)
+                            float* w, void* workspace, hipStream_t s, unsigned long long* stats_host, uint8_t* exterior_copy,
+                            bool plus_only)
 {
     const RayLayout l = full_layout(m, B, m->V, true);
+    const int dir_mode = ray_dir_mode(m, true, plus_only);
     char* ws = (char*)workspace;
     unsigned long long* stats = stats_host ? (unsigned long long*)(ws + l.stats) : nullptr;
     if (stats && hipMemsetAsync(stats, 0, 4 * sizeof(unsigned long long), s) != hipSuccess) return TUCH_ERR_HIP;
-    const int rc = launch_ray_counts<true>(m, l, verts, verts, nullptr, B, m->V, ws, s, stats);
+    const int rc = launch_ray_counts<true>(m, l, verts, verts, nullptr, B, m->V, ws, s, stats, dir_mode);
     if (rc != TUCH_OK) return rc;
     if (w || exterior)
         hipLaunchKernelGGL(ray_finalize_verts_kernel, dim3(ceil_div(m->V, kBlock), B), dim3(kBlock), 0, s, verts,
                            (const int32_t*)(ws + l.count), (const int32_t*)m->tree_qperm, (const int32_t*)m->ring_off,
                            (const int32_t*)m->ring_vidx, m->V, l.qblocks * kRayQueries, thresh, w, exterior, exterior_copy,
-                           (const float2*)(fans_in_bounds_launch(m) || fans_in_near_launch(m) ? ws + l.fans : nullptr));
+                           (const float2*)(fans_in_bounds_launch(m) || fans_in_near_launch(m) ? ws + l.fans : nullptr),
+                           (const int32_t*)(dir_mode ? ws + l.dir : nullptr));
     if (stats_host) {
         RayBody bodies[8];
         const int nb = B < 8 ? B : 8;
@@ -1760,9 +1858,18 @@
             return TUCH_ERR_HIP;
         unsigned long long tiles = 0;
         for (int b = 0; b < nb; ++b) tiles += bodies[b].tiles;
+        if (hipMemcpy(stats_host + 4, stats + 3, sizeof(unsigned long long), hipMemcpyDeviceToHost) != hipSuccess) return TUCH_ERR_HIP;
         stats_host[3] = tiles * B / nb;
     }
     return tuch_check_launch("tuch_ray_exterior_verts");
+}
+
+int tuch_ray_dir_active(const tuch_contact_model* m) { return tuch_ray_available(m) ? ray_dir_mode(m, true, false) : 0; }
+
+const int32_t* tuch_ray_dir(const tuch_contact_model* m, int B, const void* workspace)
+{
+    if (ray_dir_mode(m, true, false) == 0) return nullptr;
+    return (const int32_t*)((const char*)workspace + full_layout(m, B, m->V, true).dir);
 }
 
 const int32_t* tuch_ray_segment_counts(const tuch_contact_model* m, int B, const void* workspace)
@@ -1776,7 +1883,7 @@
 {
     const RayLayout l = full_layout(m, B, Q, false);
     char* ws = (char*)workspace;
-    const int rc = launch_ray_counts<false>(m, l, verts, points, counts, B, Q, ws, s, nullptr);
+    const int rc = launch_ray_counts<false>(m, l, verts, points, counts, B, Q, ws, s, nullptr, ray_dir_mode(m, false, false));
     if (rc != TUCH_OK) return rc;
     hipLaunchKernelGGL(ray_finalize_points_kernel, dim3(ceil_div(Q, kBlock), B), dim3(kBlock), 0, s,
                        (const int32_t*)(ws + l.count), counts, Q, l.qblocks * kRayQueries, thresh, w, exterior);
diff --git a/tuch_amd/csrc/winding.hip b/tuch_amd/csrc/winding.hip
--- a/tuch_amd/csrc/winding.hip
+++ b/tuch_amd/csrc/winding.hip
@@ -891,7 +891,8 @@
     }
     if (body_by_rays) {
         rc = tuch_ray_exterior_verts(m, verts, B, thresh, exterior, w, ws + l.ray, s, nullptr,
-                                     segments_fused ? (uint8_t*)(ws + l.body_flags) : (uint8_t*)nullptr);
+                                     segments_fused ? (uint8_t*)(ws + l.body_flags) : (uint8_t*)nullptr,
+                                      segments && !segments_fused);
         if (rc != TUCH_OK) return rc;
     } else if (use_strips(m) && use_tree(m)) {
         launch_tree_walk(m, l, verts, B, ws, nullptr, s);
@@ -995,6 +996,32 @@
     return tuch_ray_exterior_verts(m, verts, B, 0.99f, nullptr, nullptr, (char*)workspace + l.ray, (hipStream_t)stream, out_host);
 }
 
+extern "C" int tuch_ray_directions(const tuch_contact_model* m, const float* verts, int B, void* workspace,
+                                   size_t workspace_bytes, int32_t* dir_out, void* stream)
+{
+    TUCH_REQUIRE(m && verts && dir_out, "tuch_ray_directions: null pointer");
+    TUCH_REQUIRE(tuch_ray_available(m), "tuch_ray_directions: the model has no cluster tree / vertex rings");
+    TUCH_REQUIRE(B > 0 && B <= 65535, "tuch_ray_directions: bad batch %d", B);
+    const ExteriorLayout l = exterior_layout(m, B);
+    if (!workspace || workspace_bytes < l.total) {
+        tuch_set_error("tuch_ray_directions: workspace %zu < %zu bytes", workspace_bytes, l.total);
+        return TUCH_ERR_WORKSPACE;
+    }
+    hipStream_t s = (hipStream_t)stream;
+    char* ray_ws = (char*)workspace + l.ray;
+    const int rc = tuch_ray_exterior_verts(m, verts, B, 0.99f, nullptr, nullptr, ray_ws, s, nullptr);
+    if (rc != TUCH_OK) return rc;
+    const size_t n = (size_t)B * 2 * m->tree_qblocks;
+    const int32_t* dir = tuch_ray_dir(m, B, ray_ws);
+    if ((dir ? hipMemcpyAsync(dir_out, dir, n * sizeof(int32_t), hipMemcpyDeviceToDevice, s)
+             : hipMemsetD32Async((hipDeviceptr_t)dir_out, 1, n, s)) != hipSuccess ||
+        hipStreamSynchronize(s) != hipSuccess) {
+        tuch_set_error("tuch_ray_directions: copy failed");
+        return TUCH_ERR_HIP;
+    }
+    return tuch_check_launch("tuch_ray_directions");
+}
+
 struct PointsLayout { size_t stream, bounds, partial, total; int frontier, nsub, qblocks; };
 
 static PointsLayout points_layout(const tuch_contact_model* m, int B, int Q)
diff --git a/tuch_amd/ops.py b/tuch_amd/ops.py
--- a/tuch_amd/ops.py
+++ b/tuch_amd/ops.py
@@ -871,10 +871,21 @@
         L = _C.lib()
         nbytes = L.tuch_exterior_workspace_bytes(self._handle, b)
         ws = _workspace(nbytes, verts.device)
-        out = (ctypes.c_ulonglong * 4)()
+        out = (ctypes.c_ulonglong * 5)()
         _C.check(L.tuch_ray_work(self._handle, _C.ptr(verts), b, _C.ptr(ws), nbytes, out, _C.stream()))
         return dict(elements=int(out[0]), wavefronts=int(out[3]), queries_per_step=64,
-                    lanes_inside_leaf_slabs=int(out[1]) / max(int(out[2]), 1))
+                    lanes_inside_leaf_slabs=int(out[1]) / max(int(out[2]), 1),
+                    blocks_minus=int(out[4]), blocks=-(-self.num_verts // 128) * 2 * b)
+
+    def ray_directions(self, verts: torch.Tensor) -> torch.Tensor:
+        verts = _f32(verts)
+        b = verts.shape[0]
+        L = _C.lib()
+        nbytes = L.tuch_exterior_workspace_bytes(self._handle, b)
+        ws = _workspace(nbytes, verts.device)
+        out = torch.empty(b, -(-self.num_verts // 128) * 2, dtype=torch.int32, device=verts.device)
+        _C.check(L.tuch_ray_directions(self._handle, _C.ptr(verts), b, _C.ptr(ws), nbytes, _C.ptr(out), _C.stream()))
+        return out
 
     def exterior_flags(self, verts: torch.Tensor, apply_segments: bool = True, thresh: float = 0.99,
                        return_details: bool = False):
```

After: 155,600 body-fit iterations/s (median of 6 runs). 2.7% higher.
